# siyi-wind/MDViT

Hardware: AMD Instinct MI355X
Metric: 512x512 images/sec MDViT train step (fwd+bwd, two-sweep, AdamW) (higher is better)
Workload: dtype bf16x3 (fp32 storage; GEMM operands split hi+lo bf16, fp32 accumulate); 1 GPU; MDViT Sup+MLPFM train step, 4 domain(s) x bs=4 per GPU, 512x512, drop_rate=0.1 drop_path=0.1, bf16x3 GEMMs, data-parallel x1

## Files before the change

### include/mdvit_hip.h

```cpp
#ifndef MDVIT_HIP_H
#define MDVIT_HIP_H

#include <stddef.h>
#include <stdint.h>

#ifdef __cplusplus
extern "C" {
#endif

#define MDVIT_ABI_VERSION 1

enum {
    MDVIT_OK = 0,
    MDVIT_E_SHAPE = 1,
    MDVIT_E_DTYPE = 2,
    MDVIT_E_ALIGN = 3,
    MDVIT_E_WORKSPACE = 4,
    MDVIT_E_HIP = 5
};

enum { MDVIT_EPI_NONE = 0, MDVIT_EPI_GELU_DUAL = 1, MDVIT_EPI_DGELU = 2 };
enum { MDVIT_ACT_NONE = 0, MDVIT_ACT_HSWISH = 1, MDVIT_ACT_RELU = 2 };

const char* mdvit_last_error(void);
// ... 75 lines not shown
int mdvit_gemm_ph_prefers(int32_t M, int32_t N, int32_t K, int32_t planes);
int mdvit_gemm_ph_prefers_epi(int32_t M, int32_t N, int32_t K, int32_t planes, int32_t epi_reads);
int mdvit_gemm_ph_config(int32_t mode);
int mdvit_gemm_pm_prefers(int32_t M, int32_t N, int32_t K, int32_t planes, int32_t a_f32);
int mdvit_gemm_pm_config(int32_t mode);
int mdvit_gemm_pm_splits(int32_t M, int32_t N, int32_t K, int32_t planes, int32_t a_f32);
int mdvit_split_planes(const float* in, int64_t ld_in, void* out, int64_t ld_out, int64_t plane_stride, int64_t rows, int32_t cols, int32_t planes, void* stream);
int mdvit_split_planes_t(const float* in, int64_t ld_in, void* out, int64_t ld_out, int64_t plane_stride, int32_t rows, int32_t cols, int32_t transpose,
                         int32_t planes, void* stream);
int mdvit_split_planes_many(const void* items_dev, int32_t n, int32_t blocks_per_item, int32_t planes, void* stream);

int mdvit_mlp_fwd_f32(const float* x, const float* W1, const float* b1, const float* W2, const float* b2, const float* res,
                      const float* rowscale , int32_t rows_per_scale, float* h, float* y, int32_t M, int32_t C, int32_t hidden,
                      float drop_p, uint32_t key1_0, uint32_t key1_1, uint32_t key2_0, uint32_t key2_1, const uint32_t* drop_seed, void* stream);

int mdvit_mlp_config(int32_t wide_min_tokens, int32_t ablate);

int mdvit_mlp_bwd_dgrad_f32(const float* gm, const float* x, const float* W1, const float* b1, const float* W2t, const float* W1t,
                            float* du , float* dx, int32_t M, int32_t C, int32_t hidden, float drop_p,
                            uint32_t key1_0, uint32_t key1_1, const uint32_t* drop_seed, void* stream);

int mdvit_mlp_rc_fwd(const float* x, const void* W1p, const float* b1, const void* W2p, const float* b2, const float* res,
                     const float* rowscale , int32_t rows_per_scale, float* y, int32_t M, int32_t C, int32_t hidden,
                     float drop_p, uint32_t key1_0, uint32_t key1_1, uint32_t key2_0, uint32_t key2_1, const uint32_t* drop_seed, void* stream);
int mdvit_mlp_rc_dgrad(const float* gm, const float* x, const void* W1p, const float* b1, const void* W2tp, const void* W1tp, float* dx,
                       int32_t M, int32_t C, int32_t hidden, float drop_p, uint32_t key1_0, uint32_t key1_1, const uint32_t* drop_seed, void* stream);
int mdvit_linear_rc(const float* x, int64_t lda, const void* Wp, int64_t wplane, const float* bias, float* y, int64_t ldc, int32_t M, int32_t N, int32_t K,
                    float drop_p, uint32_t key0, uint32_t key1, const float* rowscale, int32_t rows_per_scale, const float* residual, int64_t ldr,
                    const uint32_t* drop_seed, void* stream);
int mdvit_linear_rc_ln(const float* x, const float* gamma, const float* beta, int32_t groups, float eps, float* mean, float* rstd, float* ln_out,
                       const void* Wp, int64_t wplane, const float* bias, float* y, int64_t ldc, int32_t M, int32_t N, int32_t K, void* stream);
int mdvit_mlp_rc16_fwd(const float* x, const void* W1p, const float* b1, const void* W2p, const float* b2, const float* res, const float* rowscale,
                       int32_t rows_per_scale, float* h, float* y, int32_t M, int32_t C, int32_t Hd, float drop_p, uint32_t key1_0, uint32_t key1_1,
                       uint32_t key2_0, uint32_t key2_1, const uint32_t* drop_seed, void* stream);
int mdvit_mlp_rc_fwd_ln(const float* x2, const float* gamma, const float* beta, int32_t groups, float eps, float* mean, float* rstd, float* ln_out,
                        const void* W1p, const float* b1, const void* W2p, const float* b2, const float* rowscale, int32_t rows_per_scale, float* h, float* y,
                        int32_t M, int32_t C, int32_t Hd, float drop_p, uint32_t key1_0, uint32_t key1_1, uint32_t key2_0, uint32_t key2_1,
                        const uint32_t* drop_seed, void* stream);
int mdvit_mlp_rc16_dgrad(const float* gm, const float* x, const void* W1p, const float* b1, const void* W2tp, const void* W1tp, float* du, float* dx,
                         int32_t M, int32_t C, int32_t Hd, float drop_p, uint32_t key1_0, uint32_t key1_1, const uint32_t* drop_seed, void* stream);
int mdvit_mlp_rc16_fwd_hbf16(const float* x, const void* W1p, const float* b1, const void* W2p, const float* b2, const float* res, const float* rowscale,
                             int32_t rows_per_scale, float* h, float* y, int32_t M, int32_t C, int32_t Hd, float drop_p, uint32_t key1_0, uint32_t key1_1,
                             uint32_t key2_0, uint32_t key2_1, const uint32_t* drop_seed, void* stream);
int mdvit_mlp_rc_fwd_ln_hbf16(const float* x2, const float* gamma, const float* beta, int32_t groups, float eps, float* mean, float* rstd, float* ln_out,
                              const void* W1p, const float* b1, const void* W2p, const float* b2, const float* rowscale, int32_t rows_per_scale, float* h, float* y,
                              int32_t M, int32_t C, int32_t Hd, float drop_p, uint32_t key1_0, uint32_t key1_1, uint32_t key2_0, uint32_t key2_1,
                              const uint32_t* drop_seed, void* stream);
int mdvit_mlp_rc16_dgrad_hbf16(const float* gm, const float* x, const void* W1p, const float* b1, const void* W2tp, const void* W1tp, float* du, float* dx,
                               int32_t M, int32_t C, int32_t Hd, float drop_p, uint32_t key1_0, uint32_t key1_1, const uint32_t* drop_seed, void* stream);
int mdvit_mlp_rc_bwd(const float* gm, const float* x, const void* W1p, const float* b1, const void* W2tp, const void* W1tp, float* dx_parts, float* dW1, float* db1,
                     float* dW2, void* ws, size_t ws_bytes, int32_t M, int32_t C, int32_t hidden, float drop_p, uint32_t key1_0, uint32_t key1_1,
                     const uint32_t* drop_seed, int32_t accumulate, void* stream);
size_t mdvit_mlp_rc_wgrad_ws_bytes(int32_t M, int32_t C, int32_t hidden);
int mdvit_gemm_ledger(int32_t enable);
int mdvit_gemm_ledger_read(int32_t index, char* name, int32_t cap, int64_t* launches, double* flop, double* bytes);
int mdvit_gemm_sampler(const char* symbol, int32_t stride);
int mdvit_gemm_sampler_read(int32_t index, char* name, int32_t cap, int64_t* seen, int64_t* timed, double* ms);
int mdvit_mlp_rc_config(int32_t fwd_variant);
int mdvit_mlp_rc_planes(int32_t planes);
int mdvit_block_config(int32_t mlp_bwd_fused);
int mdvit_mlp_rc_wgrad(const float* gm, const float* x, const void* W1p, const float* b1, const void* W2tp, float* dW1, float* db1, float* dW2,
                       void* ws, size_t ws_bytes, int32_t M, int32_t C, int32_t hidden, float drop_p, uint32_t key1_0, uint32_t key1_1,
                       const uint32_t* drop_seed, int32_t accumulate, void* stream);

typedef struct MdvitBlockDesc {
    int32_t B, H, W, C, heads, hidden, s3, s5, s7, ln_groups, D, da_hidden, precision;
    float eps, drop_p;
    uint32_t key_proj[2], key_fc1[2], key_fc2[2];
    const uint32_t* drop_seed;
    const float* rowscale1; const float* rowscale2;
    const float* label;
    const float *cpe_w, *cpe_b, *n1_g, *n1_b, *qkv_w, *qkv_b, *w3, *b3, *w5, *b5, *w7, *b7, *da_w1, *da_b1, *da_w2, *da_b2, *proj_w, *proj_b, *n2_g, *n2_b, *fc1_w, *fc1_b,
        *fc2_w, *fc2_b;
    const float *qkv_wt, *proj_wt, *fc1_wt, *fc2_wt;
    const void *fc1_p, *fc2_p, *fc2t_p, *fc1t_p;
    const void *qkv_p, *proj_p, *projt_p, *qkvt_p;
    int32_t store_bf16;
    const float* a_pre;
    int32_t attn_kind;
} MdvitBlockDesc;
typedef struct MdvitBlockGrads {
    float *cpe_w, *cpe_b, *n1_g, *n1_b, *qkv_w, *qkv_b, *w3, *b3, *w5, *b5, *w7, *b7, *da_w1, *da_b1, *da_w2, *da_b2, *proj_w, *proj_b, *n2_g, *n2_b, *fc1_w, *fc1_b, *fc2_w,
        *fc2_b;
    int32_t accumulate, dgrad_only, aux_first;
    int32_t ln_accumulate;
    float* e_out;
} MdvitBlockGrads;
typedef struct MdvitBlockStreams {
    void* main; void* side;
    void** events; int32_t n_events; int32_t* next_event;
} MdvitBlockStreams;
size_t mdvit_block_save_bytes(const MdvitBlockDesc* d);
size_t mdvit_block_fwd_ws_bytes(const MdvitBlockDesc* d);
int mdvit_block_fwd(const MdvitBlockDesc* d, const float* x, float* y, void* save, size_t save_bytes, void* ws, size_t ws_bytes, void* stream);
size_t mdvit_block_bwd_ws_bytes(const MdvitBlockDesc* d, const MdvitBlockGrads* g, int32_t with_side_stream, size_t* side_bytes);
int mdvit_block_bwd(const MdvitBlockDesc* d, const MdvitBlockGrads* g, const MdvitBlockStreams* st, const float* x, const void* save, size_t save_bytes,
                    const float* dy, float* dx , void* ws, size_t ws_bytes, void* ws_side, size_t ws_side_bytes);

int mdvit_rowdot_fwd(const float* x, int64_t ldx, const float* w, const float* b, float* y,
                     int32_t M, int32_t K, int32_t accumulate, void* stream);
int mdvit_rowdot_bwd(const float* x, int64_t ldx, const float* w, const float* dy, float* dx, int64_t lddx,
                     float* dw, float* db, void* ws , size_t ws_bytes, int32_t M, int32_t K, void* stream);

int mdvit_colsum_f32(const float* A, int64_t lda, float* out, float* masked, void* ws , size_t ws_bytes, int32_t M, int32_t N,
                     float drop_p, uint32_t key0, uint32_t key1, const float* rowscale, int32_t rows_per_scale,
                     int32_t accumulate, const uint32_t* drop_seed, void* stream);
// ... 181 lines not shown
```

### mdvit_amd/_lib.py

```python
from __future__ import annotations

import ctypes as C
import os
import re
from typing import List

_HERE = os.path.dirname(os.path.abspath(__file__))
LIB_PATH = os.environ.get("MDVIT_HIP_LIB") or os.path.join(_HERE, "lib", "libmdvit_hip.so")
HEADER_PATH = os.path.join(_HERE, "..", "include", "mdvit_hip.h")

EPI_NONE, EPI_GELU_DUAL, EPI_DGELU = 0, 1, 2
ACT_NONE, ACT_HSWISH, ACT_RELU = 0, 1, 2

f32p = C.c_void_p
vp = C.c_void_p
i32 = C.c_int32
i64 = C.c_int64
u32 = C.c_uint32
f32 = C.c_float


class GemmDesc(C.Structure):
    _fields_ = [
        ("A", vp), ("B", vp), ("C", vp), ("C2", vp),
# ... 71 lines not shown
    _fields_ = [(n, vp) for n in BLOCK_PARAMS] + [("accumulate", i32), ("dgrad_only", i32), ("aux_first", i32), ("ln_accumulate", i32), ("e_out", vp)]


class SeAdapterDesc(C.Structure):
    _fields_ = [("kind", i32), ("B", i32), ("N", i32), ("C", i32), ("r", i32), ("W1", vp), ("b1", vp), ("W2", vp), ("b2", vp), ("Wg", vp), ("bg", vp)]


SE_DASE, SE_USE = 0, 1


class BlockStreams(C.Structure):
    _fields_ = [("main", vp), ("side", vp), ("events", C.POINTER(vp)), ("n_events", i32), ("next_event", C.POINTER(i32))]


_SIGS = {
    "mdvit_block_fwd": [C.POINTER(BlockDesc), vp, vp, vp, C.c_size_t, vp, C.c_size_t, vp],
    "mdvit_block_bwd": [C.POINTER(BlockDesc), C.POINTER(BlockGrads), C.POINTER(BlockStreams), vp, vp, C.c_size_t, vp, vp, vp, C.c_size_t, vp, C.c_size_t],
    "mdvit_gemm_planes": [C.POINTER(PlaneGemmDesc), vp],
    "mdvit_gemm_planes_plan": [C.POINTER(PlaneGemmDesc), C.POINTER(i32), C.POINTER(i32), C.POINTER(i32)],
    "mdvit_gemm_planes_force_plan": [i32, i32],
    "mdvit_gemm_ph_config": [i32],
    "mdvit_gemm_pm_config": [i32],
    "mdvit_da_fwd_many": [C.POINTER(DaMany), vp, i32, i32, vp],
    "mdvit_da_bwd_many": [C.POINTER(DaMany), C.POINTER(DaManyGrads), vp, f32, vp, C.c_size_t, i32, i32, vp],
    "mdvit_gemm_pm_prefers": [i32, i32, i32, i32, i32],
    "mdvit_gemm_pm_splits": [i32, i32, i32, i32, i32],
    "mdvit_gemm_f32_grouped": [C.POINTER(GemmDesc), i32, C.POINTER(vp), C.POINTER(vp), C.POINTER(vp), vp],
    "mdvit_gemm_f32_grouped_bias": [C.POINTER(GemmDesc), i32, C.POINTER(vp), C.POINTER(vp), C.POINTER(vp), C.POINTER(vp), vp],
    "mdvit_transpose_batch": [i32, C.POINTER(vp), C.POINTER(i64), C.POINTER(vp), C.POINTER(i32), C.POINTER(i32), vp],
    "mdvit_compose_bias": [i32, C.POINTER(vp), i64, C.POINTER(vp), C.POINTER(vp), i32, i32, vp],
    "mdvit_compose_bias_bwd": [i32, C.POINTER(vp), i64, C.POINTER(vp), C.POINTER(vp), C.POINTER(vp), i64, C.POINTER(vp), i32, i32, i32, vp],
    "mdvit_gemm_ph_prefers": [i32, i32, i32, i32],
    "mdvit_gemm_ph_prefers_epi": [i32, i32, i32, i32, i32],
    "mdvit_mlp_config": [i32, i32],
    "mdvit_mlp_rc_config": [i32],
    "mdvit_mlp_rc_planes": [i32],
    "mdvit_block_config": [i32],
    "mdvit_gemm_ledger": [i32],
    "mdvit_gemm_ledger_read": [i32, C.c_char_p, i32, C.POINTER(i64), C.POINTER(C.c_double), C.POINTER(C.c_double)],
    "mdvit_gemm_sampler": [C.c_char_p, i32],
    "mdvit_gemm_sampler_read": [i32, C.c_char_p, i32, C.POINTER(i64), C.POINTER(i64), C.POINTER(C.c_double)],
    "mdvit_mlp_rc_fwd": [vp, vp, vp, vp, vp, vp, vp, i32, vp, i32, i32, i32, f32, u32, u32, u32, u32, vp, vp],
    "mdvit_linear_rc": [vp, i64, vp, i64, vp, vp, i64, i32, i32, i32, f32, u32, u32, vp, i32, vp, i64, vp, vp],
    "mdvit_linear_rc_ln": [vp, vp, vp, i32, f32, vp, vp, vp, vp, i64, vp, vp, i64, i32, i32, i32, vp],
    "mdvit_mlp_rc_fwd_ln": [vp, vp, vp, i32, f32, vp, vp, vp, vp, vp, vp, vp, vp, i32, vp, vp, i32, i32, i32, f32, u32, u32, u32, u32, vp, vp],
    "mdvit_mlp_rc16_fwd": [vp, vp, vp, vp, vp, vp, vp, i32, vp, vp, i32, i32, i32, f32, u32, u32, u32, u32, vp, vp],
    "mdvit_mlp_rc_dgrad": [vp, vp, vp, vp, vp, vp, vp, i32, i32, i32, f32, u32, u32, vp, vp],
    "mdvit_mlp_rc16_dgrad": [vp, vp, vp, vp, vp, vp, vp, vp, i32, i32, i32, f32, u32, u32, vp, vp],
    "mdvit_mlp_rc_fwd_ln_hbf16": [vp, vp, vp, i32, f32, vp, vp, vp, vp, vp, vp, vp, vp, i32, vp, vp, i32, i32, i32, f32, u32, u32, u32, u32, vp, vp],
    "mdvit_mlp_rc16_fwd_hbf16": [vp, vp, vp, vp, vp, vp, vp, i32, vp, vp, i32, i32, i32, f32, u32, u32, u32, u32, vp, vp],
    "mdvit_mlp_rc16_dgrad_hbf16": [vp, vp, vp, vp, vp, vp, vp, vp, i32, i32, i32, f32, u32, u32, vp, vp],
    "mdvit_mlp_rc_wgrad": [vp, vp, vp, vp, vp, vp, vp, vp, vp, C.c_size_t, i32, i32, i32, f32, u32, u32, vp, i32, vp],
    "mdvit_mlp_rc_bwd": [vp, vp, vp, vp, vp, vp, vp, vp, vp, vp, vp, C.c_size_t, i32, i32, i32, f32, u32, u32, vp, i32, vp],
    "mdvit_imgconv_fwd": [vp, vp, vp, i32, i32, i32, i32, i32, i32, vp],
    "mdvit_imgconv_wgrad": [vp, vp, vp, vp, C.c_size_t, i32, i32, i32, i32, i32, i32, i32, vp],
    "mdvit_maxpool3x3s2_fwd": [vp, vp, vp, i32, i32, i32, i32, vp],
    "mdvit_maxpool3x3s2_bwd": [vp, vp, vp, i32, i32, i32, i32, vp],
    "mdvit_resize_ac_fwd": [vp, vp, i32, i32, i32, i32, i32, i32, vp],
    "mdvit_resize_ac_bwd": [vp, vp, i32, i32, i32, i32, i32, i32, vp],
    "mdvit_ew": [vp, vp, vp, i64, i32, vp],
    "mdvit_add3": [vp, vp, vp, vp, i64, vp],
    "mdvit_add_parts": [vp, vp, C.POINTER(vp), i32, i64, vp, vp],
    "mdvit_add_bcast": [vp, vp, vp, i32, i64, vp],
    "mdvit_sum_batch": [vp, vp, i32, i64, vp],
    "mdvit_gate_fwd": [vp, vp, vp, i32, i64, i32, i32, vp],
    "mdvit_gate_bwd": [vp, vp, vp, vp, vp, vp, C.c_size_t, i32, i64, i32, i32, vp],
    "mdvit_imgconv_im2col": [vp, vp, i32, i32, i32, i32, i32, i32, vp],
    "mdvit_chanpool_fwd": [vp, vp, vp, i64, i32, vp],
    "mdvit_chanpool_bwd": [vp, vp, vp, i64, i32, vp],
    "mdvit_conv7x7_2to1_fwd": [vp, vp, vp, i32, i32, i32, vp],
    "mdvit_conv7x7_2to1_bwd": [vp, vp, vp, vp, vp, i32, i32, i32, vp],
    "mdvit_bn1_fwd": [vp, vp, vp, vp, vp, vp, vp, vp, i64, i32, i32, f32, f32, vp],
    "mdvit_bn1_bwd": [vp, vp, vp, vp, vp, vp, i64, i32, i32, vp],
    "mdvit_subsample2": [vp, vp, i32, i32, i32, i32, i32, vp],
    "mdvit_patchify": [vp, vp, i32, i32, i32, i32, i32, vp],
    "mdvit_dropout2d": [vp, vp, i32, i64, i32, f32, u32, u32, vp, vp],
    "mdvit_sdpa_fwd": [vp, vp, vp, vp, i32, i32, i32, i32, vp],
    "mdvit_sdpa_bwd": [vp, vp, vp, vp, vp, vp, vp, vp, i32, i32, i32, i32, vp],
    "mdvit_sdpa_mfma_fwd": [vp, vp, vp, vp, i32, i32, i32, i32, vp],
    "mdvit_sdpa_mfma_bwd": [vp, vp, vp, vp, vp, vp, vp, vp, i32, i32, i32, i32, vp],
    "mdvit_structure_weight": [vp, vp, vp, i32, i32, i32, vp],
    "mdvit_structure_loss_fwd": [vp, vp, vp, vp, vp, i32, i64, vp],
    "mdvit_structure_loss_bwd": [vp, vp, vp, vp, vp, vp, i32, i64, vp],
    "mdvit_split_planes": [vp, i64, vp, i64, i64, i64, i32, i32, vp],
    "mdvit_split_planes_many": [vp, i32, i32, i32, vp],
    "mdvit_split_planes_t": [vp, i64, vp, i64, i64, i32, i32, i32, i32, vp],
    "mdvit_event_create": [C.POINTER(vp)],
    "mdvit_event_destroy": [vp],
    "mdvit_event_elapsed_ms": [vp, vp, C.POINTER(f32)],
    "mdvit_timing_arm": [vp, vp],
    "mdvit_gemm_f32": [C.POINTER(GemmDesc), vp],
    "mdvit_gemm_plan": [C.POINTER(GemmDesc), C.POINTER(i32), C.POINTER(i32), C.POINTER(i32)],
    "mdvit_gemm_force_plan": [i32, i32],
    "mdvit_conv_weight_relayout": [vp, vp, i32, i32, i32, vp],
    "mdvit_conv_weight_relayout_many": [vp, i32, i32, vp],
    "mdvit_gemm_kernel_name": [vp, C.c_char_p, i32],
    "mdvit_gemm_tn_config": [i32, i32, i32],
    "mdvit_gemm_tn_grid_order": [i32],
    "mdvit_transpose_f32": [vp, i64, vp, i32, i32, vp],
    "mdvit_mlp_bwd_dgrad_f32": [vp, vp, vp, vp, vp, vp, vp, vp, i32, i32, i32, f32, u32, u32, vp, vp],
    "mdvit_mlp_fwd_f32": [vp, vp, vp, vp, vp, vp, vp, i32, vp, vp, i32, i32, i32, f32, u32, u32, u32, u32, vp, vp],
    "mdvit_transpose_many": [vp, i32, i32, vp],
    "mdvit_rowdot_fwd": [vp, i64, vp, vp, vp, i32, i32, i32, vp],
    "mdvit_rowdot_bwd": [vp, i64, vp, vp, vp, i64, vp, vp, vp, C.c_size_t, i32, i32, vp],
    "mdvit_colsum_f32": [vp, i64, vp, vp, vp, C.c_size_t, i32, i32, f32, u32, u32, vp, i32, i32, vp, vp],
    "mdvit_layernorm_fwd": [vp, vp, vp, vp, vp, vp, i32, i32, i32, f32, vp],
# ... 150 lines not shown
```

### mdvit_amd/csrc/block.hip

```cpp
#include <stdlib.h>
#include "common.h"

namespace {

struct Arena {
    char* base; size_t off, cap; bool dry;
    float* take(size_t floats) {
        const size_t bytes = (floats * sizeof(float) + 255) & ~(size_t)255;
        float* p = dry ? nullptr : reinterpret_cast<float*>(base + off);
        off += bytes;
        return p;
    }
    void* take_bytes(size_t bytes) { return take((bytes + 3) / 4); }
};

enum { MLP_RC = 0, MLP_RECOMP = 1, MLP_STORED = 2 };

inline int mlp_mode(const MdvitBlockDesc& d) {
    if (d.precision == 1 && d.C == 64 && d.hidden % 256 == 0 && d.hidden <= 4096 && d.fc1_p && d.fc2_p && (long)d.B * d.H * d.W * d.hidden < (1L << 32)) return MLP_RC;
    if (d.precision >= 1 && d.C <= 128 && d.C % 32 == 0 && d.hidden % 4 == 0) return MLP_RECOMP;
    return MLP_STORED;
}
inline bool mlp_rc16(const MdvitBlockDesc& d) {
    return mlp_mode(d) == MLP_RECOMP && d.precision == 1 && d.C == 128 && d.hidden % 32 == 0 && d.hidden <= 4096 && d.fc1_p && d.fc2_p && d.fc1_b && d.fc2_b &&
// ... 187 lines not shown
        if (hbf16(d))
            BLK_RUN(mdvit_mlp_rc16_fwd_hbf16(sv.cur2, d.fc1_p, d.fc1_b, d.fc2_p, d.fc2_b, sv.x2, d.rowscale2, N_tok, sv.h, y, M, C, Hd, d.drop_p, d.key_fc1[0],
                                             d.key_fc1[1], d.key_fc2[0], d.key_fc2[1], seed, s));
        else
            BLK_RUN(mdvit_mlp_rc16_fwd(sv.cur2, d.fc1_p, d.fc1_b, d.fc2_p, d.fc2_b, sv.x2, d.rowscale2, N_tok, sv.h, y, M, C, Hd, d.drop_p, d.key_fc1[0], d.key_fc1[1],
                                       d.key_fc2[0], d.key_fc2[1], seed, s));
    } else {
        MdvitGemmDesc g;
        gemm_init(g, d);
        g.A = sv.cur2; g.B = d.fc1_w; g.M = M; g.N = Hd; g.K = C; g.lda = C; g.ldb = C; g.ldc = Hd; g.bias = d.fc1_b; g.epi = MDVIT_EPI_GELU_DUAL;
        g.e_drop_p = d.drop_p; g.e_key0 = d.key_fc1[0]; g.e_key1 = d.key_fc1[1]; g.drop_seed = seed;
        if (mode == MLP_RECOMP) { g.C = sv.h; g.C2 = nullptr; }
        else { g.C = sv.u; g.C2 = sv.h; }
        g.trans_a = 0; g.trans_b = 1; g.allow_split = 0;
        if (ph_takes(d, d.fc1_p, M, Hd, C, 0)) { const int rc = gemm_planes_nt(A, g, d.fc1_p, s); if (rc != MDVIT_OK) return rc; }
        else BLK_RUN(mdvit_gemm_f32(&g, s));
        gemm_init(g, d);
        g.A = sv.h; g.B = d.fc2_w; g.C = y; g.M = M; g.N = C; g.K = Hd; g.lda = Hd; g.ldb = Hd; g.ldc = C; g.bias = d.fc2_b;
        g.e_drop_p = d.drop_p; g.e_key0 = d.key_fc2[0]; g.e_key1 = d.key_fc2[1]; g.e_rowscale = d.rowscale2; g.e_rows_per_scale = N_tok;
        g.residual = sv.x2; g.ldr = C; g.drop_seed = seed;
        g.trans_a = 0; g.trans_b = 1; g.allow_split = 0;
        if (ph_takes(d, d.fc2_p, M, C, Hd, 1)) { const int rc = gemm_planes_nt(A, g, d.fc2_p, s); if (rc != MDVIT_OK) return rc; }
        else BLK_RUN(mdvit_gemm_f32(&g, s));
    }
    return MDVIT_OK;
}

int block_bwd(const MdvitBlockDesc& d, const MdvitBlockGrads& G, const MdvitBlockStreams& st, const float* x, const float* dy, float* dx, Arena& SV, Arena& A, Arena& S) {
    const int B = d.B, H = d.H, W = d.W, C = d.C, Hd = d.hidden;
    const long T = (long)B * H * W;
    const int M = (int)T, N_tok = H * W;
    const int mode = mlp_mode(d);
    const bool dgrad_only = G.dgrad_only != 0, want_w = !dgrad_only;
    const int acc = G.accumulate;
    hipStream_t s = (hipStream_t)st.main, side = s;
    Saved sv;
    layout_saved(d, SV, sv);
    if (sdpa_kind(d)) sv.x1 = const_cast<float*>(x);
    const uint32_t* seed = d.drop_p > 0.f ? d.drop_seed : nullptr;
    const bool fast_ln = C == 64 || C == 128 || C == 320 || C == 512;

    const bool have_side = st.side != nullptr && st.side != st.main;
    const bool defer = want_w && acc != 0 && G.ln_accumulate != 0 && have_side && fast_ln;
    struct Late { const float* part; int batches, nblk, n0; float* out0; int n1; float* out1; };
    Late late[4];
    int n_late = 0;
    if (want_w && acc == 0) {
        const MdvitZeroItem z[4] = {{G.qkv_b, sizeof(float) * 3 * C}, {G.proj_b, sizeof(float) * C}, {mode == MLP_RC ? nullptr : G.fc1_b, sizeof(float) * Hd},
                                    {mode == MLP_RC ? nullptr : G.fc2_b, sizeof(float) * C}};
        BLK_RUN(mdvit_zero_many(z, 4, s));
    }

    const bool masked = d.drop_p > 0.f || d.rowscale2 != nullptr;
    float* gm2 = masked ? S.take(T * C) : const_cast<float*>(dy);
    float* tmp = A.take(T * C);
    float* dcur2 = tmp;
    const float* dcur2_b = nullptr;
    float* du = nullptr;
    if (mode == MLP_RC) {
        if (masked || want_w) {
            const size_t pb = want_w ? mdvit_partials_ws_bytes(C) : 0;
            void* pw = want_w ? (defer ? S.take_bytes(pb) : A.take_bytes(pb)) : nullptr;
            if (want_w && defer) {
                int nb = 0;
                BLK_RUN(mdvit_colsum_parts(dy, C, masked ? gm2 : nullptr, pw, pb, M, C, d.drop_p, d.key_fc2[0], d.key_fc2[1], d.rowscale2, N_tok, seed, s, &nb));
                late[n_late++] = Late{(const float*)pw, 1, nb, C, G.fc2_b, 0, nullptr};
            } else {
                BLK_RUN(mdvit_colsum_f32(dy, C, want_w ? G.fc2_b : nullptr, masked ? gm2 : nullptr, pw, pb, M, C, d.drop_p, d.key_fc2[0], d.key_fc2[1], d.rowscale2, N_tok,
                                         acc, seed, s));
            }
        }
        const bool fuse_bwd = want_w && (Hd == 256 || Hd == 512) && (g_blk_mlp_bwd == 1 || (g_blk_mlp_bwd == 2 && !have_side));
        if (fuse_bwd) {
            const int roles = Hd / 256;
            float* parts = roles == 1 ? dcur2 : A.take((long)roles * T * C);
            const size_t wb = mdvit_mlp_rc_wgrad_ws_bytes(M, C, Hd);
            void* ww = A.take_bytes(wb);
            BLK_RUN(mdvit_mlp_rc_bwd(gm2, sv.cur2, d.fc1_p, d.fc1_b, d.fc2t_p, d.fc1t_p, parts, G.fc1_w, G.fc1_b, G.fc2_w, ww, wb, M, C, Hd, d.drop_p, d.key_fc1[0],
                                     d.key_fc1[1], seed, acc, s));
            dcur2 = parts;
            dcur2_b = roles == 2 ? parts + T * C : nullptr;
        } else {
        BLK_RUN(mdvit_mlp_rc_dgrad(gm2, sv.cur2, d.fc1_p, d.fc1_b, d.fc2t_p, d.fc1t_p, dcur2, M, C, Hd, d.drop_p, d.key_fc1[0], d.key_fc1[1], seed, s));
        if (want_w) {
            const size_t wb = mdvit_mlp_rc_wgrad_ws_bytes(M, C, Hd);
            void* ww = S.take_bytes(wb);
            if (!A.dry) { const int rc = fork_side(d, st, side); if (rc != MDVIT_OK) return rc; }
            BLK_RUN(mdvit_mlp_rc_wgrad(gm2, sv.cur2, d.fc1_p, d.fc1_b, d.fc2t_p, G.fc1_w, G.fc1_b, G.fc2_w, ww, wb, M, C, Hd, d.drop_p, d.key_fc1[0], d.key_fc1[1], seed,
                                       acc, side));
        }
        }
    } else {
        if (masked) BLK_RUN(mdvit_colsum_f32(dy, C, nullptr, gm2, nullptr, 0, M, C, d.drop_p, d.key_fc2[0], d.key_fc2[1], d.rowscale2, N_tok, 0, seed, s));
        MdvitGemmDesc g;
        int rc = MDVIT_OK;
        const bool hb = hbf16(d);
        if (hb && !(d.fc2t_p && d.fc1t_p)) return mdvit_set_error(MDVIT_E_SHAPE, "block_bwd: store_bf16 needs the transposed fc weight planes (the 16-token MLP backward)");
        if (mlp_rc16(d) && d.fc2t_p && d.fc1t_p) {
            du = want_w ? S.take(hb ? (T * Hd + 1) / 2 : T * Hd) : nullptr;
            if (hb) BLK_RUN(mdvit_mlp_rc16_dgrad_hbf16(gm2, sv.cur2, d.fc1_p, d.fc1_b, d.fc2t_p, d.fc1t_p, du, dcur2, M, C, Hd, d.drop_p, d.key_fc1[0], d.key_fc1[1], seed, s));
            else BLK_RUN(mdvit_mlp_rc16_dgrad(gm2, sv.cur2, d.fc1_p, d.fc1_b, d.fc2t_p, d.fc1t_p, du, dcur2, M, C, Hd, d.drop_p, d.key_fc1[0], d.key_fc1[1], seed, s));
        } else {
            du = S.take(T * Hd);
            gemm_init(g, d);
            g.epi = MDVIT_EPI_DGELU; g.e_drop_p = d.drop_p; g.e_key0 = d.key_fc1[0]; g.e_key1 = d.key_fc1[1]; g.drop_seed = seed;
            if (mode == MLP_RECOMP) { g.rc_a = sv.cur2; g.rc_lda = C; g.rc_b = d.fc1_w; g.rc_ldb = C; g.rc_bias = d.fc1_b; g.rc_k = C; }
            else { g.gelu_u = sv.u; g.ldu = Hd; }
            g.allow_split = 0;
            rc = gemm_dgrad(A, d, g, gm2, d.fc2_w, d.fc2_wt, du, M, Hd, C, s, d.fc2t_p);
            if (rc != MDVIT_OK) return rc;
            gemm_init(g, d);
            g.allow_split = 1;
            rc = gemm_dgrad(A, d, g, du, d.fc1_w, d.fc1_wt, dcur2, M, C, Hd, s, d.fc1t_p);
            if (rc != MDVIT_OK) return rc;
        }
        if (want_w) {
            if (!A.dry) { rc = fork_side(d, st, side); if (rc != MDVIT_OK) return rc; }
            rc = gemm_wgrad(S, d, gm2, sv.h, G.fc2_w, G.fc2_b, M, C, Hd, acc, side, 0, hb);
            if (rc == MDVIT_OK) rc = gemm_wgrad(S, d, du, sv.cur2, G.fc1_w, G.fc1_b, M, Hd, C, acc, side, hb, 0);
            if (rc != MDVIT_OK) return rc;
        }
    }
    const bool masked1 = d.drop_p > 0.f || d.rowscale1 != nullptr;
    float* dx2 = masked1 ? A.take(T * C) : S.take(T * C);
    float* gm1 = masked1 ? S.take(T * C) : dx2;
    {
        const bool lnw = want_w || !fast_ln;
        const size_t pb = lnw ? mdvit_partials_ws_bytes(2 * C) : 0;
        void* pw = lnw ? A.take_bytes(pb) : nullptr;
        float* dg = want_w ? G.n2_g : (lnw ? A.take((long)d.ln_groups * C) : nullptr);
        float* db = want_w ? G.n2_b : (lnw ? A.take((long)d.ln_groups * C) : nullptr);
        if (!A.dry) mdvit_layernorm_bwd_next_dy2(dcur2_b);
        if (defer) {
            void* pws = S.take_bytes(pb);
            int nb = 0;
            BLK_RUN(mdvit_layernorm_bwd_parts(dcur2, sv.x2, d.n2_g, sv.mean2, sv.rstd2, dy, dx2, masked1 ? gm1 : nullptr, pws, pb, M, C, d.ln_groups, d.drop_p, d.key_proj[0],
                                              d.key_proj[1], d.rowscale1, N_tok, seed, s, &nb));
            late[n_late++] = Late{(const float*)pws, d.ln_groups, nb, C, dg, C, db};
        } else if (masked1 && fast_ln) {
            BLK_RUN(mdvit_layernorm_bwd_masked(dcur2, sv.x2, d.n2_g, sv.mean2, sv.rstd2, dy, dx2, gm1, dg, db, pw, pb, M, C, d.ln_groups, d.drop_p, d.key_proj[0],
                                               d.key_proj[1], d.rowscale1, N_tok, seed, s));
        } else {
            BLK_RUN(mdvit_layernorm_bwd(dcur2, sv.x2, d.n2_g, sv.mean2, sv.rstd2, dy, dx2, dg, db, pw, pb, M, C, d.ln_groups, s));
            if (masked1) BLK_RUN(mdvit_colsum_f32(dx2, C, nullptr, gm1, nullptr, 0, M, C, d.drop_p, d.key_proj[0], d.key_proj[1], d.rowscale1, N_tok, 0, seed, s));
        }
    }
    float* datt = tmp;
    {
        MdvitGemmDesc g;
        gemm_init(g, d);
        g.allow_split = 1;
        int rc = MDVIT_OK;
        if (d.precision == 1 && (C == 64 || C == 128) && d.projt_p && M >= 1024) {
            BLK_RUN(mdvit_linear_rc(gm1, C, d.projt_p, (long)C * C, nullptr, datt, C, M, C, C, 0.f, 0, 0, nullptr, 1, nullptr, 0, nullptr, s));
// ... 182 lines not shown
```

### mdvit_amd/csrc/common.h

```cpp
#pragma once
#include <hip/hip_runtime.h>
#include <hip/hip_ext.h>
#include <stdint.h>
#include <stdio.h>
#include <string.h>

#include "../../include/mdvit_hip.h"

#define MDVIT_WAVE 64

extern thread_local char g_mdvit_err[512];
int mdvit_set_error(int code, const char* fmt, ...);

#define MDVIT_CHECK_ARG(cond, code, ...)                      \
    do {                                                      \
        if (!(cond)) return mdvit_set_error(code, __VA_ARGS__); \
    } while (0)

extern hipEvent_t g_mdvit_t0, g_mdvit_t1;
#define MDVIT_TIMED_LAUNCH(kernel, grid, block, shmem, s, ...)                                                       \
    do {                                                                                                              \
        if (g_mdvit_t0) {                                                                                             \
            hipExtLaunchKernelGGL(kernel, grid, block, shmem, s, g_mdvit_t0, g_mdvit_t1, 0, __VA_ARGS__);             \
            g_mdvit_t0 = g_mdvit_t1 = nullptr;                                                                        \
        } else {                                                                                                      \
            hipLaunchKernelGGL(kernel, grid, block, shmem, s, __VA_ARGS__);                                           \
        }                                                                                                             \
    } while (0)

#define MDVIT_LAUNCH_CHECK()                                                         \
    do {                                                                             \
        hipError_t e__ = hipGetLastError();                                          \
        if (e__ != hipSuccess)                                                       \
            return mdvit_set_error(MDVIT_E_HIP, "%s:%d launch failed: %s", __FILE__, \
                                   __LINE__, hipGetErrorString(e__));                \
    } while (0)

int mdvit_zero_async(void* ptr, size_t bytes, hipStream_t stream);
struct MdvitZeroItem { void* p; size_t bytes; };
int mdvit_zero_many(const MdvitZeroItem* items, int n, hipStream_t stream);
#define MDVIT_ZERO(ptr, bytes, strm)                                   \
    do {                                                               \
        int rc__ = mdvit_zero_async((ptr), (bytes), (strm));           \
        if (rc__ != MDVIT_OK) return rc__;                             \
    } while (0)

int mdvit_reduce_partials(const float* part, int nblk, long stride, int n0, float* out0, int n1, float* out1, int accumulate, hipStream_t stream);
int mdvit_reduce_partials_batched(const float* part, int batches, int nblk, int n, float* out, hipStream_t stream);
int mdvit_reduce_partials_batched2(const float* part, int batches, int nblk, int n0, float* out0, int n1, float* out1, hipStream_t stream);
int mdvit_reduce_partials_batched2_acc(const float* part, int batches, int nblk, int n0, float* out0, int n1, float* out1, int accumulate, hipStream_t stream);
int mdvit_layernorm_bwd_parts(const float* dy, const float* x, const float* gamma, const float* mean, const float* rstd, const float* add, float* dx,
                              float* dx_masked, void* ws, size_t ws_bytes, int M, int C, int groups, float drop_p, uint32_t key0, uint32_t key1,
                              const float* rowscale, int rows_per_scale, const uint32_t* seed, hipStream_t stream, int* nblk);
int mdvit_colsum_parts(const float* A, long lda, float* masked, void* ws, size_t ws_bytes, int M, int N, float drop_p, uint32_t key0, uint32_t key1,
                       const float* rowscale, int rows_per_scale, const uint32_t* seed, hipStream_t stream, int* nblk);
void mdvit_layernorm_bwd_next_dy2(const float* dy2);
constexpr int MDVIT_MAX_PARTIAL_ROWS = 2048;
#define MDVIT_CHECK_PARTIALS_WS(ws, ws_bytes, nblk, n, what)                                                              \
    MDVIT_CHECK_ARG((ws) != nullptr && (ws_bytes) >= sizeof(float) * (size_t)(nblk) * (size_t)(n), MDVIT_E_WORKSPACE,    \
                    what ": workspace too small: need %zu bytes (mdvit_partials_ws_bytes), got %zu",                      \
                    sizeof(float) * (size_t)(nblk) * (size_t)(n), (size_t)(ws_bytes))

static inline bool aligned16(const void* p) { return (reinterpret_cast<uintptr_t>(p) & 15) == 0; }

static inline int cdiv(long a, long b) { return (int)((a + b - 1) / b); }

__device__ __forceinline__ uint32_t mdvit_hash32(uint32_t x) {
    x ^= x >> 16; x *= 0x7feb352dU; x ^= x >> 15; x *= 0x846ca68bU; x ^= x >> 16;
    return x;
}
__device__ __forceinline__ uint32_t mdvit_drop_bits(uint32_t k0, uint32_t k1, uint32_t idx) {
    return mdvit_hash32(((idx >> 2) ^ k0) + k1);
}
__device__ __forceinline__ uint32_t mdvit_drop_bits_q(uint32_t k0, uint32_t k1, uint32_t quad) { return mdvit_hash32((quad ^ k0) + k1); }
__device__ __forceinline__ float mdvit_drop_scale(uint32_t k0, uint32_t k1, uint32_t idx, uint32_t thresh, float inv_keep) {
    const uint32_t h = __builtin_rotateright32(mdvit_drop_bits(k0, k1, idx), 8u * (idx & 3u));
    return h >= thresh ? inv_keep : 0.0f;
}
static inline uint32_t mdvit_drop_thresh(double p) {
    double t = p * 65536.0 + 0.5;
    if (t < 0.0) t = 0.0;
    if (t > 65535.0) t = 65535.0;
    return (uint32_t)t << 16;
}
__device__ __forceinline__ void mdvit_drop_keep4(uint32_t h, uint32_t thresh16, bool (&keep)[4]) {
    const uint32_t r = __builtin_rotateright32(h, 8);
    keep[0] = (h >> 16) >= thresh16;
    keep[1] = (r >> 16) >= thresh16;
    keep[2] = (h & 0xffffu) >= thresh16;
    keep[3] = (r & 0xffffu) >= thresh16;
}
__device__ __forceinline__ float4 mdvit_drop_scale4(uint32_t k0, uint32_t k1, uint32_t idx4, uint32_t thresh, float inv_keep) {
    const uint32_t h = mdvit_drop_bits(k0, k1, idx4);
    return make_float4(h >= thresh ? inv_keep : 0.0f,
                       __builtin_rotateright32(h, 8) >= thresh ? inv_keep : 0.0f,
                       __builtin_rotateright32(h, 16) >= thresh ? inv_keep : 0.0f,
                       __builtin_rotateright32(h, 24) >= thresh ? inv_keep : 0.0f);
}

__device__ __forceinline__ float mdvit_normalize_level(unsigned char level, int c) {
    const float mean[3] = {0.485f, 0.456f, 0.406f}, stdv[3] = {0.229f, 0.224f, 0.225f};
    const float v = (float)((double)level / 255.0);
    return (v - mean[c]) / stdv[c];
}

__device__ __forceinline__ unsigned mdvit_xcd_logical_block() {
    const unsigned nwg = gridDim.x, q = nwg >> 3, r = nwg & 7, xcd = blockIdx.x & 7, idx = blockIdx.x >> 3;
    return (xcd < r ? xcd * (q + 1) : r * (q + 1) + (xcd - r) * q) + idx;
// ... 84 lines not shown
```

### mdvit_amd/csrc/mlp_rc.hip

```cpp
#include "common.h"
#include <type_traits>
#ifndef RC_ABL
#define RC_ABL 0
#endif

typedef float rc_f32x16 __attribute__((ext_vector_type(16)));
typedef __bf16 rc_bf16x8 __attribute__((ext_vector_type(8)));
typedef unsigned rc_u4 __attribute__((ext_vector_type(4)));
typedef unsigned rc_u2 __attribute__((ext_vector_type(2)));
typedef float rc_f4 __attribute__((ext_vector_type(4)));
typedef short rc_v4i16 __attribute__((ext_vector_type(4)));
typedef short rc_v8i16 __attribute__((ext_vector_type(8)));
typedef __attribute__((address_space(3))) rc_v4i16* rc_lds_v4i16_ptr;

namespace {

template <int ROWB>
__device__ __forceinline__ int rc_swz(int row) {
    if (ROWB == 64) return (row >> 2) & 3;
    if (ROWB == 128) return (((row >> 1) & 1) << 2) | ((row >> 2) & 3);
    return row & 15;
}

template <int ROWB>
__device__ __forceinline__ void rc_glds_piece(const uint16_t* __restrict__ src, long ld, int piece, int lane, char* tile) {
    constexpr int LPR = ROWB / 16, RPP = 1024 / ROWB;
    const int row = piece * RPP + lane / LPR;
    const int lc = (lane % LPR) ^ rc_swz<ROWB>(row);
    __builtin_amdgcn_global_load_lds(src + (long)row * ld + (lc << 3), (__attribute__((address_space(3))) void*)(tile + piece * 1024), 16, 0, 0);
}

template <int ROWB>
__device__ __forceinline__ rc_bf16x8 rc_frag(const char* tile, int row, int chunk) {
    return __builtin_bit_cast(rc_bf16x8, *reinterpret_cast<const rc_u4*>(tile + row * ROWB + ((chunk ^ rc_swz<ROWB>(row)) << 4)));
}

__device__ __forceinline__ rc_bf16x8 rc_frag_perm(const char* tile, int row, int hf, int g) {
    const int f = rc_swz<64>(row);
    typedef __attribute__((address_space(3))) const volatile rc_u2* lds_u2_ptr;
    const rc_u2 a = *(lds_u2_ptr)(tile + row * 64 + (((2 * hf) ^ f) << 4) + 8 * g);
    const rc_u2 b = *(lds_u2_ptr)(tile + row * 64 + (((2 * hf + 1) ^ f) << 4) + 8 * g);
    return __builtin_bit_cast(rc_bf16x8, (rc_u4{a[0], a[1], b[0], b[1]}));
}

#define RC_MFMA3P(P1, acc, ah, al, bh, bl)                                          \
    do {                                                                            \
        if constexpr (!(P1)) {                                                      \
            acc = __builtin_amdgcn_mfma_f32_32x32x16_bf16(al, bh, acc, 0, 0, 0);    \
            acc = __builtin_amdgcn_mfma_f32_32x32x16_bf16(ah, bl, acc, 0, 0, 0);    \
        }                                                                           \
        acc = __builtin_amdgcn_mfma_f32_32x32x16_bf16(ah, bh, acc, 0, 0, 0);        \
    } while (0)
#define RC_MFMA3(acc, ah, al, bh, bl)                                           \
    do {                                                                        \
        acc = __builtin_amdgcn_mfma_f32_32x32x16_bf16(al, bh, acc, 0, 0, 0);    \
        acc = __builtin_amdgcn_mfma_f32_32x32x16_bf16(ah, bl, acc, 0, 0, 0);    \
        acc = __builtin_amdgcn_mfma_f32_32x32x16_bf16(ah, bh, acc, 0, 0, 0);    \
    } while (0)

__device__ __forceinline__ void rc_split8(const float* v, rc_u4& hi, rc_u4& lo) {
    uint2 h0, l0, h1, l1;
    mdvit_split_bf16x3(make_float4(v[0], v[1], v[2], v[3]), h0, l0);
    mdvit_split_bf16x3(make_float4(v[4], v[5], v[6], v[7]), h1, l1);
    hi = rc_u4{h0.x, h0.y, h1.x, h1.y};
    lo = rc_u4{l0.x, l0.y, l1.x, l1.y};
}

__device__ __forceinline__ rc_bf16x8 rc_natural_order(rc_u4 v) {
    const rc_u2 a = __builtin_amdgcn_permlane32_swap(v[0], v[2], false, false);
    const rc_u2 b = __builtin_amdgcn_permlane32_swap(v[1], v[3], false, false);
    return __builtin_bit_cast(rc_bf16x8, (rc_u4{a[0], b[0], a[1], b[1]}));
}

struct LnPro { const float* g; const float* b; float* mean; float* rstd; float* out; float eps; int rows_per_group; };
template <int K>
__device__ __forceinline__ void rc_ln_rows32(float4 (&a)[K / 16], float4 (&b)[K / 16], int row, int rowc, int M, int lhi, const LnPro ln);

template <int C, bool LNP = false>
__device__ __forceinline__ void rc_load_rows(const float* __restrict__ src, int row, int M, int lhi, rc_bf16x8 (&hi)[C / 16], rc_bf16x8 (&lo)[C / 16],
                                             const LnPro* ln = nullptr) {
    const float* p = src + (long)min(row, M - 1) * C + 8 * lhi;
    float4 a[C / 16], b[C / 16];
#pragma unroll
    for (int kb = 0; kb < C / 16; ++kb) {
        a[kb] = *reinterpret_cast<const float4*>(p + 16 * kb);
        b[kb] = *reinterpret_cast<const float4*>(p + 16 * kb + 4);
    }
    if constexpr (LNP) rc_ln_rows32<C>(a, b, row, min(row, M - 1), M, lhi, *ln);
#pragma unroll
    for (int kb = 0; kb < C / 16; ++kb) {
        const float v[8] = {a[kb].x, a[kb].y, a[kb].z, a[kb].w, b[kb].x, b[kb].y, b[kb].z, b[kb].w};
        rc_u4 h, l;
        rc_split8(v, h, l);
        hi[kb] = __builtin_bit_cast(rc_bf16x8, h);
        lo[kb] = __builtin_bit_cast(rc_bf16x8, l);
    }
}

__device__ __forceinline__ void rc_erf_parts(float x, float& e, float& q) {
    e = __builtin_amdgcn_exp2f(x * x * -0.72134752044448170368f);
    const float t = __builtin_amdgcn_rcpf(fmaf(0.3275911f * 0.70710678118654752f, fabsf(x), 1.0f));
    float poly = fmaf(1.061405429f, t, -1.453152027f);
    poly = fmaf(poly, t, 1.421413741f);
    poly = fmaf(poly, t, -0.284496736f);
    poly = fmaf(poly, t, 0.254829592f);
    q = fmaf(-(poly * t), e, 1.0f);
}
__device__ __forceinline__ float rc_gelu_k(float x, float hk) {
    float e, q;
    rc_erf_parts(x, e, q);
    const float hx = x * hk;
    return fmaf(fabsf(hx), q, hx);
}
__device__ __forceinline__ float rc_dgelu_k(float x, float d, float hks, float pks) {
    float e, q;
    rc_erf_parts(x, e, q);
    const float cdf = fmaf(copysignf(q, x), hks, hks);
    return d * fmaf(x * e, pks, cdf);
}
__device__ __forceinline__ void rc_gelu_both_k(float x, float hk, float d, float hks, float pks, float& h, float& du) {
    float e, q;
    rc_erf_parts(x, e, q);
    const float hx = x * hk;
    h = fmaf(fabsf(hx), q, hx);
    const float cdf = fmaf(copysignf(q, x), hks, hks);
    du = d * fmaf(x * e, pks, cdf);
}
typedef float rc_f2 __attribute__((ext_vector_type(2)));
template <bool P1 = false>
__device__ __forceinline__ void rc_split2(float a, float b, uint32_t& hi, uint32_t& lo) {
    hi = __builtin_bit_cast(uint32_t, __builtin_convertvector((rc_f2{a, b}), mdvit_bf16x2));
    if constexpr (P1) { lo = 0u; return; }
    const rc_f2 l = {a - __uint_as_float(hi << 16), b - __uint_as_float(hi & 0xffff0000u)};
    lo = __builtin_bit_cast(uint32_t, __builtin_convertvector(l, mdvit_bf16x2));
}
__device__ __forceinline__ void rc_keep_sel4(uint32_t h, uint32_t thresh16, float on, float off, float (&k)[4]) {
    bool keep[4];
    mdvit_drop_keep4(h, thresh16, keep);
#pragma unroll
    for (int j = 0; j < 4; ++j) k[j] = keep[j] ? on : off;
}
// ... 15 lines not shown
#pragma unroll
    for (int kq = 0; kq < 4; ++kq) {
        float s0 = 0.f, s1 = 0.f;
#pragma unroll
        for (int j = 0; j < VPL; ++j) {
            const float4 va = a[kq + 4 * j], vb = b[kq + 4 * j];
            s0 += (va.x + va.y) + (va.z + va.w);
            s1 += (vb.x + vb.y) + (vb.z + vb.w);
        }
        q[kq][0] = s0; q[kq][1] = s1;
    }
    const float mu = lin_sum16(q) * (1.0f / K);
#pragma unroll
    for (int kb = 0; kb < KB; ++kb) {
        a[kb].x -= mu; a[kb].y -= mu; a[kb].z -= mu; a[kb].w -= mu;
        b[kb].x -= mu; b[kb].y -= mu; b[kb].z -= mu; b[kb].w -= mu;
    }
#pragma unroll
    for (int kq = 0; kq < 4; ++kq) {
        float s0 = 0.f, s1 = 0.f;
#pragma unroll
        for (int j = 0; j < VPL; ++j) {
            s0 += mdvit_ln_sq4(a[kq + 4 * j]);
            s1 += mdvit_ln_sq4(b[kq + 4 * j]);
        }
        q[kq][0] = s0; q[kq][1] = s1;
    }
    const float rs = mdvit_ln_rstd(lin_sum16(q), 1.0f / K, ln.eps);
#pragma unroll
    for (int kb = 0; kb < KB; ++kb) {
        const float4 ga = *reinterpret_cast<const float4*>(gg + 16 * kb), gb4 = *reinterpret_cast<const float4*>(gg + 16 * kb + 4);
        const float4 ba = *reinterpret_cast<const float4*>(gb + 16 * kb), bb4 = *reinterpret_cast<const float4*>(gb + 16 * kb + 4);
        a[kb] = mdvit_ln_affine4(a[kb], rs, ga, ba);
        b[kb] = mdvit_ln_affine4(b[kb], rs, gb4, bb4);
        if (row < M) {
            *reinterpret_cast<float4*>(ln.out + (long)row * K + 8 * lhi + 16 * kb) = a[kb];
            *reinterpret_cast<float4*>(ln.out + (long)row * K + 8 * lhi + 16 * kb + 4) = b[kb];
        }
    }
    if (lhi == 0 && row < M) { ln.mean[row] = mu; ln.rstd[row] = rs; }
}

struct RcArgs {
    const float* x; const float* gm; const float* res; const float* rowscale; const float* b1; const float* b2;
    const uint16_t* W1p;
    const uint16_t* W2p;
    const uint16_t* W2tp;
    const uint16_t* W1tp;
    float* y; float* dx;
    float* du;
    int hbf;
    float* h;
    LnPro ln;
    float* part;
    int M, Hd, rows_per_scale;
    int drop; uint32_t k1a, k1b, k2a, k2b, thresh; float inv_keep;
    const uint32_t* seed;
    int groups, tiles_per_group;
};

template <int NM, int V, int ND, int LEAD>
__device__ __forceinline__ void rc_interleave() {
    __builtin_amdgcn_sched_group_barrier(0x100, LEAD, 0);
#pragma unroll
    for (int i = 0; i < NM; ++i) {
        __builtin_amdgcn_sched_group_barrier(0x008, 1, 0);
        __builtin_amdgcn_sched_group_barrier(0x002, V, 0);
        if (i < ND - LEAD) __builtin_amdgcn_sched_group_barrier(0x100, 1, 0);
    }
}

#define RC_WAIT_VM(n) asm volatile("s_waitcnt vmcnt(%0)" ::"n"(n) : "memory")
#define RC_BARRIER() asm volatile("s_waitcnt lgkmcnt(0)\n\ts_barrier" ::: "memory")

template <int C, int NW, bool DROP>
__global__ __launch_bounds__(NW * 64) __attribute__((amdgpu_waves_per_eu(2, 2))) void mlp_rc_fwd_kernel(RcArgs p) {
    constexpr int KB = C / 16, CB = C / 32;
    constexpr int RB1 = C * 2;
    constexpr int T1 = 32 * RB1, T2 = C * 64;
    constexpr int PIECES = (2 * T1 + 2 * T2) / 1024;
    static_assert(PIECES % NW == 0, "pieces must divide over the waves");
    constexpr int PPW = PIECES / NW;
    extern __shared__ __attribute__((aligned(1024))) char smem[];
    char* sW1 = smem;
    char* sW2 = sW1 + 3 * 2 * T1;
    float* sB1 = reinterpret_cast<float*>(sW2 + 3 * 2 * T2);
    const int tid = threadIdx.x, lane = tid & 63, wave = __builtin_amdgcn_readfirstlane(tid >> 6), l31 = lane & 31, lhi = lane >> 5;
    const int row = blockIdx.x * (NW * 32) + wave * 32 + l31;
    const int n = p.Hd >> 5;
    uint32_t s0 = 0, s1 = 0;
    if (p.seed) { s0 = p.seed[0]; s1 = p.seed[1]; }
    const uint32_t k1a = p.k1a ^ s0, k1b = p.k1b + s1, k2a = p.k2a ^ s0, k2b = p.k2b + s1;
    const long wplane = (long)p.Hd * C;

    auto issue_w1 = [&](int slot_s, int src_s, int pc) __attribute__((always_inline)) {
        constexpr int PP = T1 / 1024;
        const int pl = pc / PP, q = pc % PP;
        rc_glds_piece<RB1>(p.W1p + pl * wplane + (long)(src_s * 32) * C, C, q, lane, sW1 + ((slot_s % 3) * 2 + pl) * T1);
    };
    auto issue_w2 = [&](int s, int pc) __attribute__((always_inline)) {
        constexpr int PP = T2 / 1024;
        const int pl = pc / PP, q = pc % PP;
        rc_glds_piece<64>(p.W2p + pl * wplane + s * 32, p.Hd, q, lane, sW2 + ((s % 3) * 2 + pl) * T2);
    };
    auto issue_group = [&](int g) __attribute__((always_inline)) {
#pragma unroll
// ... 278 lines not shown
    constexpr int PIECES = (4 * T1 + 2 * T3) / 1024;
    static_assert(PIECES % NW == 0, "pieces must divide over the waves");
    constexpr int PPW = PIECES / NW;
    extern __shared__ __attribute__((aligned(1024))) char smem[];
    char* sW1 = smem;
    char* sW2t = sW1 + 3 * 2 * T1;
    char* sW1t = sW2t + 3 * 2 * T1;
    float* sB1 = reinterpret_cast<float*>(sW1t + 3 * 2 * T3);
    const int tid = threadIdx.x, lane = tid & 63, wave = __builtin_amdgcn_readfirstlane(tid >> 6), l31 = lane & 31, lhi = lane >> 5;
    const int row = blockIdx.x * (NW * 32) + wave * 32 + l31;
    const int n = p.Hd >> 5;
    uint32_t s0 = 0, s1 = 0;
    if (p.seed) { s0 = p.seed[0]; s1 = p.seed[1]; }
    const uint32_t k1a = p.k1a ^ s0, k1b = p.k1b + s1;
    const uint32_t dq0 = (uint32_t)((long)row * p.Hd + 4 * lhi) >> 2, thresh16 = p.thresh >> 16;
    const float hks = 0.5f * p.inv_keep, pks = 0.39894228040143268f * p.inv_keep;
    const long wplane = (long)p.Hd * C;

    static_assert(T1 / 1024 == NW && T3 / 1024 == NW, "one 1 KiB piece of each of the six planes per wave and hidden step");
    uint32_t voff1, voff3;
    {
        constexpr int LPR = RB1 / 16, RPP = 1024 / RB1;
        const int r1 = wave * RPP + lane / LPR;
        voff1 = (uint32_t)(r1 * C + (((lane % LPR) ^ rc_swz<RB1>(r1)) << 3)) * 2u;
        const int r3 = wave * 16 + (lane >> 2);
        voff3 = (uint32_t)(r3 * p.Hd + (((lane & 3) ^ rc_swz<64>(r3)) << 3)) * 2u;
    }
    typedef __attribute__((address_space(3))) void* lds_ptr;
    auto issue_a = [&](int slot_s, int src_s) __attribute__((always_inline)) {
        const int sl = slot_s % 3;
        const char* b1p = reinterpret_cast<const char*>(p.W1p) + (long)src_s * (32 * C * 2);
        const char* b2p = reinterpret_cast<const char*>(p.W2tp) + (long)src_s * (32 * C * 2);
        __builtin_amdgcn_global_load_lds(b1p + voff1, (lds_ptr)(sW1 + (sl * 2 + 0) * T1 + wave * 1024), 16, 0, 0);
        __builtin_amdgcn_global_load_lds(b1p + wplane * 2 + voff1, (lds_ptr)(sW1 + (sl * 2 + 1) * T1 + wave * 1024), 16, 0, 0);
        __builtin_amdgcn_global_load_lds(b2p + voff1, (lds_ptr)(sW2t + (sl * 2 + 0) * T1 + wave * 1024), 16, 0, 0);
        __builtin_amdgcn_global_load_lds(b2p + wplane * 2 + voff1, (lds_ptr)(sW2t + (sl * 2 + 1) * T1 + wave * 1024), 16, 0, 0);
    };
    auto issue_b = [&](int s) __attribute__((always_inline)) {
        const int sl = s % 3;
        const char* b3p = reinterpret_cast<const char*>(p.W1tp) + (long)s * (32 * 2);
        __builtin_amdgcn_global_load_lds(b3p + voff3, (lds_ptr)(sW1t + (sl * 2 + 0) * T3 + wave * 1024), 16, 0, 0);
        __builtin_amdgcn_global_load_lds(b3p + wplane * 2 + voff3, (lds_ptr)(sW1t + (sl * 2 + 1) * T3 + wave * 1024), 16, 0, 0);
    };
    auto issue_group = [&](int g) __attribute__((always_inline)) {
        issue_a(g + 2, min(g + 2, n - 1));
        issue_b(g);
    };
    issue_a(0, 0);
    issue_a(1, 1);
    issue_group(0);
    for (int i = tid; i < p.Hd / 4; i += NW * 64) reinterpret_cast<float4*>(sB1)[i] = reinterpret_cast<const float4*>(p.b1)[i];
    rc_bf16x8 xh[KB], xl[KB], gh[KB], gl[KB];
    rc_load_rows<C>(p.x, row, p.M, lhi, xh, xl);
    rc_load_rows<C>(p.gm, row, p.M, lhi, gh, gl);
    rc_f32x16 dxacc[CB];
#pragma unroll
    for (int cb = 0; cb < CB; ++cb)
#pragma unroll
        for (int r = 0; r < 16; ++r) dxacc[cb][r] = 0.f;
    RC_WAIT_VM(0);
    __syncthreads();

    auto prod1 = [&](int s, rc_f32x16& u, rc_f32x16& d) __attribute__((always_inline)) {
        const char* w1h = sW1 + ((s % 3) * 2) * T1; const char* w1l = w1h + T1;
        const char* w2h = sW2t + ((s % 3) * 2) * T1; const char* w2l = w2h + T1;
#pragma unroll
        for (int q = 0; q < 4; ++q) {
            const rc_f4 b4 = *reinterpret_cast<const rc_f4*>(sB1 + s * 32 + 8 * q + 4 * lhi);
            u[4 * q + 0] = b4.x; u[4 * q + 1] = b4.y; u[4 * q + 2] = b4.z; u[4 * q + 3] = b4.w;
        }
#pragma unroll
        for (int r = 0; r < 16; ++r) d[r] = 0.f;
#pragma unroll
        for (int kb = 0; kb < KB; ++kb) {
            const rc_bf16x8 ah = rc_frag<RB1>(w1h, l31, 2 * kb + lhi), al = rc_frag<RB1>(w1l, l31, 2 * kb + lhi);
            RC_MFMA3P(P1, u, ah, al, xh[kb], xl[kb]);
            const rc_bf16x8 ch = rc_frag<RB1>(w2h, l31, 2 * kb + lhi), cl = rc_frag<RB1>(w2l, l31, 2 * kb + lhi);
            RC_MFMA3P(P1, d, ch, cl, gh[kb], gl[kb]);
        }
    };
    auto prod3 = [&](int s, const rc_bf16x8 (&dh)[2], const rc_bf16x8 (&dl)[2]) __attribute__((always_inline)) {
        const char* hi = sW1t + ((s % 3) * 2) * T3; const char* lo = hi + T3;
#pragma unroll
        for (int half = 0; half < 2; ++half)
#pragma unroll
            for (int cb = 0; cb < CB; ++cb) {
                const rc_bf16x8 ah = rc_frag_perm(hi, cb * 32 + l31, half, lhi);
                rc_bf16x8 al = ah;
                if constexpr (!P1) al = rc_frag_perm(lo, cb * 32 + l31, half, lhi);
                RC_MFMA3P(P1, dxacc[cb], ah, al, dh[half], dl[half]);
            }
    };
    auto act = [&](int s, const rc_f32x16& u, const rc_f32x16& d, rc_bf16x8 (&dh)[2], rc_bf16x8 (&dl)[2]) __attribute__((always_inline)) {
        uint32_t ph[8], pl[8];
#pragma unroll
        for (int q = 0; q < 4; ++q) {
            float dm[4] = {d[4 * q + 0], d[4 * q + 1], d[4 * q + 2], d[4 * q + 3]};
            if (DROP) {
                bool keep[4];
                mdvit_drop_keep4(mdvit_drop_bits_q(k1a, k1b, dq0 + s * 8 + 2 * q), thresh16, keep);
#pragma unroll
                for (int j = 0; j < 4; ++j) dm[j] = keep[j] ? dm[j] : 0.f;
            }
            const float g0 = rc_dgelu_k(u[4 * q + 0], dm[0], hks, pks), g1 = rc_dgelu_k(u[4 * q + 1], dm[1], hks, pks);
            const float g2 = rc_dgelu_k(u[4 * q + 2], dm[2], hks, pks), g3 = rc_dgelu_k(u[4 * q + 3], dm[3], hks, pks);
            rc_split2<P1>(g0, g1, ph[2 * q], pl[2 * q]);
            rc_split2<P1>(g2, g3, ph[2 * q + 1], pl[2 * q + 1]);
// ... 94 lines not shown
#define RC16_MFMA3_BWD(acc, ah, al, bh, bl)                                     \
    do {                                                                        \
        acc = __builtin_amdgcn_mfma_f32_16x16x32_bf16(al, bh, acc, 0, 0, 0);    \
        acc = __builtin_amdgcn_mfma_f32_16x16x32_bf16(ah, bl, acc, 0, 0, 0);    \
        acc = __builtin_amdgcn_mfma_f32_16x16x32_bf16(ah, bh, acc, 0, 0, 0);    \
    } while (0)
typedef float rc_acc4 __attribute__((ext_vector_type(4)));
constexpr int RC_WT_ROW = 528;
constexpr int RC_BWD_LDS = 2 * 64 * RC_WT_ROW + 8 * 2 * 2048;

template <int C, bool DROP, bool DX = false, bool P1 = false>
__global__ __launch_bounds__(512) __attribute__((amdgpu_waves_per_eu(2, 2))) void mlp_rc_wgrad_kernel(RcArgs p) {
    constexpr int KB = C / 16, CB = C / 32;
    constexpr int TP = 32 * 128;
    static_assert(C == 64, "token-tile staging below is written for C = 64");
    __shared__ __attribute__((aligned(1024))) char smem[2 * 4 * TP];
    extern __shared__ __attribute__((aligned(1024))) char dsm[];
    char* sWt = dsm;
    char* sDu = dsm + 2 * 64 * RC_WT_ROW;
    const int tid = threadIdx.x, lane = tid & 63, wave = __builtin_amdgcn_readfirstlane(tid >> 6), l31 = lane & 31, lhi = lane >> 5, l15 = lane & 15;
    const int roles = p.Hd >> 8;
    const int xcd = blockIdx.x & 7, idx = blockIdx.x >> 3;
    const int role = idx % roles, group = (idx / roles) * 8 + xcd;
    const int hs = role * 256 + wave * 32;
    const int ntiles = (p.M + 31) >> 5;
    const int t_beg = min(group * p.tiles_per_group, ntiles), t_end = min(t_beg + p.tiles_per_group, ntiles);
    uint32_t s0 = 0, s1 = 0;
    if (p.seed) { s0 = p.seed[0]; s1 = p.seed[1]; }
    const uint32_t k1a = p.k1a ^ s0, k1b = p.k1b + s1;
    const long wplane = (long)p.Hd * C;

    rc_bf16x8 w1h[KB], w1l[KB], w2h[KB], w2l[KB];
#pragma unroll
    for (int kb = 0; kb < KB; ++kb) {
        const long o = (long)(hs + l31) * C + 16 * kb + 8 * lhi;
        w1h[kb] = __builtin_bit_cast(rc_bf16x8, *reinterpret_cast<const rc_u4*>(p.W1p + o));
        w1l[kb] = __builtin_bit_cast(rc_bf16x8, *reinterpret_cast<const rc_u4*>(p.W1p + wplane + o));
        w2h[kb] = __builtin_bit_cast(rc_bf16x8, *reinterpret_cast<const rc_u4*>(p.W2tp + o));
        w2l[kb] = __builtin_bit_cast(rc_bf16x8, *reinterpret_cast<const rc_u4*>(p.W2tp + wplane + o));
    }
    const float bias = p.b1[hs + l31];
    rc_f32x16 aw1[CB], aw2[CB];
#pragma unroll
    for (int cb = 0; cb < CB; ++cb)
#pragma unroll
        for (int r = 0; r < 16; ++r) { aw1[cb][r] = 0.f; aw2[cb][r] = 0.f; }
    float db1 = 0.f;
    const uint32_t drot = 8u * (lane & 3), thresh16 = p.thresh >> 16;
    const float hks = 0.5f * p.inv_keep, pks = 0.39894228040143268f * p.inv_keep;

    const int srow = tid >> 4, sc4 = tid & 15;
    const int soff = srow * 128 + (((sc4 >> 1) ^ rc_swz<128>(srow)) << 4) + (sc4 & 1) * 8;
    float4 rx, rg;
    auto load_tile = [&](int t) __attribute__((always_inline)) {
        const int row = t * 32 + srow, rc = min(row, p.M - 1);
        rx = *reinterpret_cast<const float4*>(p.x + (long)rc * C + sc4 * 4);
        rg = *reinterpret_cast<const float4*>(p.gm + (long)rc * C + sc4 * 4);
        if (row >= p.M) rg = make_float4(0.f, 0.f, 0.f, 0.f);
    };
    auto store_tile = [&](int buf) __attribute__((always_inline)) {
        char* b = smem + buf * 4 * TP;
        uint2 hi, lo;
        mdvit_split_bf16x3(rx, hi, lo);
        *reinterpret_cast<rc_u2*>(b + soff) = rc_u2{hi.x, hi.y};
        *reinterpret_cast<rc_u2*>(b + TP + soff) = rc_u2{lo.x, lo.y};
        mdvit_split_bf16x3(rg, hi, lo);
        *reinterpret_cast<rc_u2*>(b + 2 * TP + soff) = rc_u2{hi.x, hi.y};
        *reinterpret_cast<rc_u2*>(b + 3 * TP + soff) = rc_u2{lo.x, lo.y};
    };

    if (DX) {
        for (int i = tid; i < 2 * 64 * 32; i += 512) {
            const int pl = i >> 11, c = (i >> 5) & 63, ch = i & 31;
            const rc_u4 v = *reinterpret_cast<const rc_u4*>(p.W1tp + pl * wplane + (long)c * p.Hd + role * 256 + ch * 8);
            *reinterpret_cast<rc_u4*>(sWt + (pl * 64 + c) * RC_WT_ROW + ch * 16) = v;
        }
    }
    if (t_beg < t_end) {
        load_tile(t_beg);
        store_tile(0);
    }
    __syncthreads();
    for (int t = t_beg; t < t_end; ++t) {
        const int buf = (t - t_beg) & 1;
        const char* xb = smem + buf * 4 * TP;
        const char* xhi = xb; const char* xlo = xb + TP; const char* ghi = xb + 2 * TP; const char* glo = xb + 3 * TP;
        if (t + 1 < t_end) load_tile(t + 1);
        rc_f32x16 u, d;
#pragma unroll
        for (int r = 0; r < 16; ++r) { u[r] = bias; d[r] = 0.f; }
#pragma unroll
        for (int kb = 0; kb < KB; ++kb) {
            const rc_bf16x8 ah = rc_frag<128>(xhi, l31, 2 * kb + lhi), al = rc_frag<128>(xlo, l31, 2 * kb + lhi);
            RC_MFMA3_ACT_AP(P1, u, ah, al, w1h[kb], w1l[kb]);
            const rc_bf16x8 ch = rc_frag<128>(ghi, l31, 2 * kb + lhi), cl = rc_frag<128>(glo, l31, 2 * kb + lhi);
            RC_MFMA3_ACT_AP(P1, d, ch, cl, w2h[kb], w2l[kb]);
        }
        uint32_t hb[4];
        if (DROP) {
#pragma unroll
            for (int j = 0; j < 4; ++j) {
                const int tok = t * 32 + j + 8 * (lane & 3) + 4 * lhi;
                hb[j] = mdvit_drop_bits(k1a, k1b, (uint32_t)((long)tok * p.Hd + hs + l31));
            }
        }
#pragma unroll
        for (int ks = 0; ks < 2; ++ks) {
            rc_u4 hh, hl, dh, dl;
#pragma unroll
            for (int i = 0; i < 4; ++i) {
                const int r = 8 * ks + 2 * i;
                float hv[2], gv[2];
#pragma unroll
                for (int e = 0; e < 2; ++e) {
                    float hk = 0.5f, dm = d[r + e];
                    if (DROP) {
                        const uint32_t w = rc_quad_bcast(hb[(r + e) & 3], (r + e) >> 2);
                        const bool keep = (__builtin_amdgcn_alignbit(w, w, drot) >> 16) >= thresh16;
                        hk = keep ? hks : 0.f; dm = keep ? dm : 0.f;
                    }
                    rc_gelu_both_k(u[r + e], hk, dm, hks, pks, hv[e], gv[e]);
                    db1 += gv[e];
                }
                uint32_t a0, a1, a2, a3;
                rc_split2<P1>(hv[0], hv[1], a0, a1);
                rc_split2<P1>(gv[0], gv[1], a2, a3);
                hh[i] = a0; hl[i] = a1; dh[i] = a2; dl[i] = a3;
            }
            const rc_bf16x8 hhf = __builtin_bit_cast(rc_bf16x8, hh), hlf = __builtin_bit_cast(rc_bf16x8, hl);
            const rc_bf16x8 dhf = __builtin_bit_cast(rc_bf16x8, dh), dlf = __builtin_bit_cast(rc_bf16x8, dl);
            if (DX) {
                char* base = sDu + wave * 4096 + l31 * 64 + 8 * lhi;
                const int f = (l31 >> 1) & 3;
#pragma unroll
                for (int pc = 0; pc < 2; ++pc) {
                    const int ch = (2 * ks + pc) ^ f;
                    *reinterpret_cast<rc_u2*>(base + (ch << 4)) = rc_u2{dh[2 * pc], dh[2 * pc + 1]};
                    *reinterpret_cast<rc_u2*>(base + 2048 + (ch << 4)) = rc_u2{dl[2 * pc], dl[2 * pc + 1]};
                }
            }
            const int t0 = 16 * ks + 4 * lhi;
#pragma unroll
            for (int cb = 0; cb < CB; ++cb) {
                const int col0 = cb * 32 + 16 * ((lane >> 4) & 1);
                const rc_bf16x8 bxh = rc_tr8(xhi, t0, col0, l15), bxl = rc_tr8(xlo, t0, col0, l15);
                RC_MFMA3_ACT_AP(P1, aw1[cb], dhf, dlf, bxh, bxl);
                const rc_bf16x8 agh = rc_tr8(ghi, t0, col0, l15), agl = rc_tr8(glo, t0, col0, l15);
                RC_MFMA3_ACT_AP(P1, aw2[cb], agh, agl, hhf, hlf);
            }
        }
        if (DX) {
            __syncthreads();
            const int cblk = wave & 3, tblk = wave >> 2, g4 = lane >> 4;
            rc_acc4 acc = {0.f, 0.f, 0.f, 0.f};
            const int pr = l15 >> 2, pcb = 32 * tblk + 8 * (l15 & 3);
#pragma unroll
            for (int k8 = 0; k8 < 8; ++k8) {
                const char* wa = sWt + (cblk * 16 + l15) * RC_WT_ROW + (4 * k8 + g4) * 16;
                const rc_bf16x8 ah = __builtin_bit_cast(rc_bf16x8, *reinterpret_cast<const rc_u4*>(wa));
                const rc_bf16x8 al = __builtin_bit_cast(rc_bf16x8, *reinterpret_cast<const rc_u4*>(wa + 64 * RC_WT_ROW));
                const char* dplane = sDu + k8 * 4096;
                const int ra = 8 * g4 + pr, rb = ra + 4;
                const int oa = ra * 64 + (((pcb >> 4) ^ ((ra >> 1) & 3)) << 4) + (pcb & 15), ob = rb * 64 + (((pcb >> 4) ^ ((rb >> 1) & 3)) << 4) + (pcb & 15);
                const rc_v4i16 h0 = __builtin_amdgcn_ds_read_tr16_b64_v4i16((rc_lds_v4i16_ptr)(dplane + oa)), h1 = __builtin_amdgcn_ds_read_tr16_b64_v4i16((rc_lds_v4i16_ptr)(dplane + ob));
                const rc_v4i16 l0 = __builtin_amdgcn_ds_read_tr16_b64_v4i16((rc_lds_v4i16_ptr)(dplane + 2048 + oa)), l1 = __builtin_amdgcn_ds_read_tr16_b64_v4i16((rc_lds_v4i16_ptr)(dplane + 2048 + ob));
                const rc_bf16x8 bh = __builtin_bit_cast(rc_bf16x8, (rc_v8i16{h0[0], h0[1], h0[2], h0[3], h1[0], h1[1], h1[2], h1[3]}));
                const rc_bf16x8 bl = __builtin_bit_cast(rc_bf16x8, (rc_v8i16{l0[0], l0[1], l0[2], l0[3], l1[0], l1[1], l1[2], l1[3]}));
                RC16_MFMA3_BWDP(P1, acc, ah, al, bh, bl);
            }
            const int tok = t * 32 + tblk * 16 + l15;
            if (tok < p.M) *reinterpret_cast<float4*>(p.dx + ((long)role * p.M + tok) * C + cblk * 16 + 4 * g4) = make_float4(acc[0], acc[1], acc[2], acc[3]);
        }
        if (t + 1 < t_end) store_tile(buf ^ 1);
        __syncthreads();
    }

    float* pg = p.part + (long)group * (2L * p.Hd * C + p.Hd);
#pragma unroll
    for (int cb = 0; cb < CB; ++cb)
#pragma unroll
        for (int r = 0; r < 16; ++r) {
            const int i = (r & 3) + 8 * (r >> 2) + 4 * lhi;
            pg[(long)(hs + i) * C + cb * 32 + l31] = aw1[cb][r];
            pg[(long)p.Hd * C + (long)(cb * 32 + i) * p.Hd + hs + l31] = aw2[cb][r];
        }
    db1 += __shfl_xor(db1, 32, 64);
    if (lhi == 0) pg[2L * p.Hd * C + hs + l31] = db1;
}

typedef float rc_f32x4 __attribute__((ext_vector_type(4)));

template <int ROWB>
__device__ __forceinline__ int rc16_swz(int row) {
    if (ROWB == 64) return (row >> 2) & 3;
    if (ROWB == 128) return (row >> 1) & 7;
    return row & 15;
}
template <int ROWB>
__device__ __forceinline__ void rc16_glds_piece(const uint16_t* __restrict__ src, long ld, int piece, int lane, char* tile) {
    constexpr int LPR = ROWB / 16, RPP = 1024 / ROWB;
    const int row = piece * RPP + lane / LPR;
    const int lc = (lane % LPR) ^ rc16_swz<ROWB>(row);
    __builtin_amdgcn_global_load_lds(src + (long)row * ld + (lc << 3), (__attribute__((address_space(3))) void*)(tile + piece * 1024), 16, 0, 0);
}
template <int ROWB>
__device__ __forceinline__ rc_bf16x8 rc16_frag(const char* tile, int row, int chunk) {
    return __builtin_bit_cast(rc_bf16x8, *reinterpret_cast<const rc_u4*>(tile + row * ROWB + ((chunk ^ rc16_swz<ROWB>(row)) << 4)));
}
__device__ __forceinline__ rc_bf16x8 rc16_frag_perm(const char* tile, int row, int g) {
    const int f = rc16_swz<64>(row);
    const rc_u2 a = *reinterpret_cast<const rc_u2*>(tile + row * 64 + (((g >> 1) ^ f) << 4) + (g & 1) * 8);
    const rc_u2 b = *reinterpret_cast<const rc_u2*>(tile + row * 64 + (((2 + (g >> 1)) ^ f) << 4) + (g & 1) * 8);
    return __builtin_bit_cast(rc_bf16x8, (rc_u4{a[0], a[1], b[0], b[1]}));
}

#define RC16_MFMA3P(P1, acc, ah, al, bh, bl)                                        \
    do {                                                                            \
        if constexpr (!(P1)) {                                                      \
            acc = __builtin_amdgcn_mfma_f32_16x16x32_bf16(al, bh, acc, 0, 0, 0);    \
            acc = __builtin_amdgcn_mfma_f32_16x16x32_bf16(ah, bl, acc, 0, 0, 0);    \
        }                                                                           \
        acc = __builtin_amdgcn_mfma_f32_16x16x32_bf16(ah, bh, acc, 0, 0, 0);        \
    } while (0)
#define RC16_MFMA3(acc, ah, al, bh, bl)                                         \
    do {                                                                        \
        acc = __builtin_amdgcn_mfma_f32_16x16x32_bf16(al, bh, acc, 0, 0, 0);    \
        acc = __builtin_amdgcn_mfma_f32_16x16x32_bf16(ah, bl, acc, 0, 0, 0);    \
        acc = __builtin_amdgcn_mfma_f32_16x16x32_bf16(ah, bh, acc, 0, 0, 0);    \
    } while (0)

__device__ __forceinline__ void rc16_ln_rows128(float4 (&a)[4], float4 (&b)[4], int row, int rowc, int M, int g, const LnPro ln);

template <int C, bool LNP = false>
__device__ __forceinline__ void rc16_load_rows(const float* __restrict__ src, int row, int M, int g, rc_bf16x8 (&hi)[C / 32], rc_bf16x8 (&lo)[C / 32],
                                               const LnPro* ln = nullptr) {
    const float* p = src + (long)min(row, M - 1) * C + 8 * g;
    float4 a[C / 32], b[C / 32];
#pragma unroll
    for (int ks = 0; ks < C / 32; ++ks) {
        a[ks] = *reinterpret_cast<const float4*>(p + 32 * ks);
        b[ks] = *reinterpret_cast<const float4*>(p + 32 * ks + 4);
    }
    if constexpr (LNP && C == 128) rc16_ln_rows128(a, b, row, min(row, M - 1), M, g, *ln);
#pragma unroll
    for (int ks = 0; ks < C / 32; ++ks) {
        const float v[8] = {a[ks].x, a[ks].y, a[ks].z, a[ks].w, b[ks].x, b[ks].y, b[ks].z, b[ks].w};
        rc_u4 h, l;
        rc_split8(v, h, l);
        hi[ks] = __builtin_bit_cast(rc_bf16x8, h);
        lo[ks] = __builtin_bit_cast(rc_bf16x8, l);
    }
}

__device__ __forceinline__ float rc16_sum16(const float (&q)[2][2]) {
    float r0 = q[0][0] + q[1][0], r1 = q[0][1] + q[1][1];
    r0 += __shfl_xor(r0, 32, 64); r1 += __shfl_xor(r1, 32, 64);
    r0 += __shfl_xor(r0, 16, 64); r1 += __shfl_xor(r1, 16, 64);
    return r0 + r1;
}
__device__ __forceinline__ void rc16_ln_rows128(float4 (&a)[4], float4 (&b)[4], int row, int rowc, int M, int g, const LnPro ln) {
    constexpr int K = 128;
    const int grp = rowc / ln.rows_per_group;
    const float* gg = ln.g + (long)grp * K + 8 * g;
    const float* gb = ln.b + (long)grp * K + 8 * g;
    float q[2][2];
#pragma unroll
    for (int kq = 0; kq < 2; ++kq) {
        float s0 = 0.f, s1 = 0.f;
#pragma unroll
        for (int j = 0; j < 2; ++j) {
            const float4 va = a[kq + 2 * j], vb = b[kq + 2 * j];
            s0 += (va.x + va.y) + (va.z + va.w);
            s1 += (vb.x + vb.y) + (vb.z + vb.w);
        }
        q[kq][0] = s0; q[kq][1] = s1;
    }
    const float mu = rc16_sum16(q) * (1.0f / K);
#pragma unroll
    for (int ks = 0; ks < 4; ++ks) {
        a[ks].x -= mu; a[ks].y -= mu; a[ks].z -= mu; a[ks].w -= mu;
        b[ks].x -= mu; b[ks].y -= mu; b[ks].z -= mu; b[ks].w -= mu;
    }
#pragma unroll
    for (int kq = 0; kq < 2; ++kq) {
        float s0 = 0.f, s1 = 0.f;
#pragma unroll
        for (int j = 0; j < 2; ++j) {
            s0 += mdvit_ln_sq4(a[kq + 2 * j]);
            s1 += mdvit_ln_sq4(b[kq + 2 * j]);
        }
        q[kq][0] = s0; q[kq][1] = s1;
    }
    const float rs = mdvit_ln_rstd(rc16_sum16(q), 1.0f / K, ln.eps);
#pragma unroll
    for (int ks = 0; ks < 4; ++ks) {
        const float4 ga = *reinterpret_cast<const float4*>(gg + 32 * ks), gb4 = *reinterpret_cast<const float4*>(gg + 32 * ks + 4);
// ... 119 lines not shown
            v.x *= rsc; v.y *= rsc; v.z *= rsc; v.w *= rsc;
            const float4 r4 = rq[ct];
            v.x += r4.x; v.y += r4.y; v.z += r4.z; v.w += r4.w;
            if (row < p.M) *reinterpret_cast<float4*>(p.y + (long)row * C + col) = v;
        }
    }
}

template <int C, int NW, int OCC, bool DROP, bool STORE, bool P1 = false>
__global__ __launch_bounds__(NW * 64) __attribute__((amdgpu_waves_per_eu(OCC, OCC))) void mlp_rc16_dgrad_kernel(RcArgs p) {
    constexpr int KS = C / 32, CT = C / 16;
    constexpr int RB1 = C * 2;
    constexpr int T1 = 32 * RB1, T3 = C * 64;
    constexpr int PIECES = (4 * T1 + 2 * T3) / 1024;
    static_assert(PIECES % NW == 0, "pieces must divide over the waves");
    constexpr int PPW = PIECES / NW;
    extern __shared__ __attribute__((aligned(1024))) char smem[];
    char* sW1 = smem;
    char* sW2 = sW1 + 3 * 2 * T1;
    char* sW3 = sW2 + 3 * 2 * T1;
    float* sB1 = reinterpret_cast<float*>(sW3 + 3 * 2 * T3);
    const int tid = threadIdx.x, lane = tid & 63, wave = __builtin_amdgcn_readfirstlane(tid >> 6), c16 = lane & 15, g = lane >> 4;
    const int row = blockIdx.x * (NW * 16) + wave * 16 + c16;
    const int n = p.Hd >> 5;
    uint32_t s0 = 0, s1 = 0;
    if (p.seed) { s0 = p.seed[0]; s1 = p.seed[1]; }
    const uint32_t k1a = p.k1a ^ s0, k1b = p.k1b + s1;
    const uint32_t dq0 = (uint32_t)((long)row * p.Hd + 4 * g) >> 2, thresh16 = p.thresh >> 16;
    const float hks = 0.5f * p.inv_keep, pks = 0.39894228040143268f * p.inv_keep;
    const long wplane = (long)p.Hd * C;
    auto issue_group = [&](int gi) __attribute__((always_inline)) {
        const int gs = min(gi, n - 1), slot = gi % 3;
#pragma unroll
        for (int i = 0; i < PPW; ++i) {
            const int pc = wave + i * NW;
            constexpr int PP1 = T1 / 1024, PP3 = T3 / 1024;
            if (pc < 2 * PP1) {
                const int pl = pc / PP1, q = pc % PP1;
                rc16_glds_piece<RB1>(p.W1p + pl * wplane + (long)(gs * 32) * C, C, q, lane, sW1 + (slot * 2 + pl) * T1);
            } else if (pc < 4 * PP1) {
                const int pc2 = pc - 2 * PP1, pl = pc2 / PP1, q = pc2 % PP1;
                rc16_glds_piece<RB1>(p.W2tp + pl * wplane + (long)(gs * 32) * C, C, q, lane, sW2 + (slot * 2 + pl) * T1);
            } else {
                const int pc3 = pc - 4 * PP1, pl = pc3 / PP3, q = pc3 % PP3;
                rc16_glds_piece<64>(p.W1tp + pl * wplane + gs * 32, p.Hd, q, lane, sW3 + (slot * 2 + pl) * T3);
            }
        }
    };
    issue_group(0);
    issue_group(1);
    for (int i = tid; i < p.Hd / 4; i += NW * 64) reinterpret_cast<float4*>(sB1)[i] = reinterpret_cast<const float4*>(p.b1)[i];
    rc_bf16x8 xh[KS], xl[KS], mh[KS], ml[KS];
    rc16_load_rows<C>(p.x, row, p.M, g, xh, xl);
    rc16_load_rows<C>(p.gm, row, p.M, g, mh, ml);
    rc_f32x4 dacc[CT];
#pragma unroll
    for (int ct = 0; ct < CT; ++ct) dacc[ct] = rc_f32x4{0.f, 0.f, 0.f, 0.f};
    __syncthreads();

    for (int t = 0; t < n; ++t) {
        if (STORE && t > 0) RC_WAIT_VM(PPW + 2);
        else RC_WAIT_VM(PPW);
        RC_BARRIER();
        issue_group(t + 2);
        const int slot = t % 3;
        const char* w1h = sW1 + (slot * 2) * T1; const char* w1l = w1h + T1;
        const char* w2h = sW2 + (slot * 2) * T1; const char* w2l = w2h + T1;
        const char* w3h = sW3 + (slot * 2) * T3; const char* w3l = w3h + T3;
        rc_u4 dh4, dl4;
#pragma unroll
        for (int ht = 0; ht < 2; ++ht) {
            const int hd = t * 32 + 16 * ht + 4 * g;
            const rc_f4 b4 = *reinterpret_cast<const rc_f4*>(sB1 + hd);
            rc_f32x4 u = {b4.x, b4.y, b4.z, b4.w}, d = {0.f, 0.f, 0.f, 0.f};
#pragma unroll
            for (int ks = 0; ks < KS; ++ks) {
                const rc_bf16x8 ah = rc16_frag<RB1>(w1h, 16 * ht + c16, 4 * ks + g), al = rc16_frag<RB1>(w1l, 16 * ht + c16, 4 * ks + g);
                RC16_MFMA3P(P1, u, ah, al, xh[ks], xl[ks]);
            }
#pragma unroll
            for (int ks = 0; ks < KS; ++ks) {
                const rc_bf16x8 ah = rc16_frag<RB1>(w2h, 16 * ht + c16, 4 * ks + g), al = rc16_frag<RB1>(w2l, 16 * ht + c16, 4 * ks + g);
                RC16_MFMA3P(P1, d, ah, al, mh[ks], ml[ks]);
            }
            float dm[4] = {d[0], d[1], d[2], d[3]};
            if (DROP) {
                bool keep[4];
                mdvit_drop_keep4(mdvit_drop_bits_q(k1a, k1b, dq0 + t * 8 + 4 * ht), thresh16, keep);
#pragma unroll
                for (int j = 0; j < 4; ++j) dm[j] = keep[j] ? dm[j] : 0.f;
            }
            const float g0 = rc_dgelu_k(u[0], dm[0], hks, pks), g1 = rc_dgelu_k(u[1], dm[1], hks, pks), g2 = rc_dgelu_k(u[2], dm[2], hks, pks), g3 = rc_dgelu_k(u[3], dm[3], hks, pks);
            if (STORE && !p.hbf) { if (row < p.M) *reinterpret_cast<float4*>(p.du + (long)row * p.Hd + hd) = make_float4(g0, g1, g2, g3); }
            uint32_t a0, a1, a2, a3;
            rc_split2<P1>(g0, g1, a0, a1);
            rc_split2<P1>(g2, g3, a2, a3);
            dh4[2 * ht] = a0; dl4[2 * ht] = a1; dh4[2 * ht + 1] = a2; dl4[2 * ht + 1] = a3;
        }
        if (STORE && p.hbf && row < p.M) {
            uint16_t* db = reinterpret_cast<uint16_t*>(p.du) + (long)row * p.Hd + t * 32 + 4 * g;
            *reinterpret_cast<uint2*>(db) = make_uint2(dh4[0], dh4[1]);
            *reinterpret_cast<uint2*>(db + 16) = make_uint2(dh4[2], dh4[3]);
        }
        const rc_bf16x8 dh = __builtin_bit_cast(rc_bf16x8, dh4), dl = __builtin_bit_cast(rc_bf16x8, dl4);
#pragma unroll
        for (int ct = 0; ct < CT; ++ct) {
            const rc_bf16x8 ah = rc16_frag_perm(w3h, 16 * ct + c16, g), al = rc16_frag_perm(w3l, 16 * ct + c16, g);
// ... 98 lines not shown
            }
            if (FULL) {
#pragma clang fp contract(off)
                v.x *= rsc; v.y *= rsc; v.z *= rsc; v.w *= rsc;
                v.x += rq[q].x; v.y += rq[q].y; v.z += rq[q].z; v.w += rq[q].w;
            }
            if (row < p.M) *reinterpret_cast<float4*>(p.y + (long)row * p.ldc + col) = v;
        }
    }
    RC_WAIT_VM(0);
}

__global__ __launch_bounds__(256) void rc_reduce_kernel(const float* __restrict__ part, int groups, long stride, int n0, float* o0, int n1, float* o1, int n2, float* o2,
                                                        int accumulate) {
    const int q = blockIdx.x * 256 + threadIdx.x, n = n0 + n1 + n2;
    if (q * 4 >= n) return;
    float4 s = make_float4(0.f, 0.f, 0.f, 0.f);
    const float* src = part + (long)q * 4;
    int g = 0;
    for (; g + 4 <= groups; g += 4) {
        const float4 a = *reinterpret_cast<const float4*>(src + (long)g * stride), b = *reinterpret_cast<const float4*>(src + (long)(g + 1) * stride);
        const float4 c = *reinterpret_cast<const float4*>(src + (long)(g + 2) * stride), d = *reinterpret_cast<const float4*>(src + (long)(g + 3) * stride);
        s.x += a.x; s.y += a.y; s.z += a.z; s.w += a.w;
        s.x += b.x; s.y += b.y; s.z += b.z; s.w += b.w;
        s.x += c.x; s.y += c.y; s.z += c.z; s.w += c.w;
        s.x += d.x; s.y += d.y; s.z += d.z; s.w += d.w;
    }
    for (; g < groups; ++g) {
        const float4 a = *reinterpret_cast<const float4*>(src + (long)g * stride);
        s.x += a.x; s.y += a.y; s.z += a.z; s.w += a.w;
    }
    const int i = q * 4;
    float* dst = i < n0 ? o0 + i : (i < n0 + n1 ? o1 + (i - n0) : o2 + (i - n0 - n1));
    float4 v = s;
    if (accumulate) { const float4 o = *reinterpret_cast<const float4*>(dst); v.x += o.x; v.y += o.y; v.z += o.z; v.w += o.w; }
    *reinterpret_cast<float4*>(dst) = v;
}

int rc_set_lds(const void* k, int bytes, bool (&flags)[64]) {
    int dev = 0;
    if (hipGetDevice(&dev) != hipSuccess || dev < 0 || dev >= 64) dev = 0;
    if (flags[dev]) return MDVIT_OK;
    const hipError_t e = hipFuncSetAttribute(k, hipFuncAttributeMaxDynamicSharedMemorySize, bytes);
    if (e != hipSuccess) return mdvit_set_error(MDVIT_E_HIP, "mlp_rc: cannot raise the dynamic LDS limit: %s", hipGetErrorString(e));
    flags[dev] = true;
    return MDVIT_OK;
}

void rc_fill(RcArgs& a, int M, int Hd, float drop_p, uint32_t k10, uint32_t k11, uint32_t k20, uint32_t k21, const uint32_t* seed) {
    a.M = M; a.Hd = Hd;
    a.drop = drop_p > 0.f; a.k1a = k10; a.k1b = k11; a.k2a = k20; a.k2b = k21;
    a.thresh = mdvit_drop_thresh(drop_p); a.inv_keep = 1.f / (1.f - drop_p);
    a.seed = seed;
}

}

int g_rc_planes = 2;
extern "C" int mdvit_mlp_rc_planes(int32_t planes) {
    if (planes != 1 && planes != 2) return mdvit_set_error(MDVIT_E_SHAPE, "mlp_rc_planes: 1 or 2");
    g_rc_planes = planes;
    return MDVIT_OK;
}
template <auto KERNEL>
static int rc_launch(int lds_cap, dim3 grid, dim3 block, int smem, hipStream_t s, const RcArgs& a) {
    static bool fl[64] = {false};
    if (lds_cap > 0) {
        const int rc = rc_set_lds(reinterpret_cast<const void*>(KERNEL), lds_cap, fl);
        if (rc != MDVIT_OK) return rc;
    }
    hipLaunchKernelGGL(KERNEL, grid, block, smem, s, a);
    return MDVIT_OK;
}

int g_rc_fwd_variant = 3;
int g_rc_fwd128_variant = 16;
extern "C" int mdvit_mlp_rc_config(int32_t fwd_variant) {
    if (fwd_variant == 16 || fwd_variant == 32) g_rc_fwd128_variant = fwd_variant;
    else g_rc_fwd_variant = fwd_variant;
    return MDVIT_OK;
}

extern "C" int mdvit_mlp_rc_fwd(const float* x, const void* W1p, const float* b1, const void* W2p, const float* b2, const float* res, const float* rowscale,
                                int32_t rows_per_scale, float* y, int32_t M, int32_t C, int32_t Hd, float drop_p, uint32_t key1_0, uint32_t key1_1,
                                uint32_t key2_0, uint32_t key2_1, const uint32_t* drop_seed, void* stream) {
    MDVIT_CHECK_ARG(C == 64, MDVIT_E_SHAPE, "mlp_rc_fwd: built for C = 64 (got %d)", C);
    MDVIT_CHECK_ARG(M > 0 && Hd >= 64 && Hd % 64 == 0 && Hd <= 4096, MDVIT_E_SHAPE, "mlp_rc_fwd: need M > 0, hidden %% 64 == 0, hidden <= 4096 (M=%d hidden=%d)", M, Hd);
    MDVIT_CHECK_ARG(x && W1p && b1 && W2p && b2 && res && y, MDVIT_E_SHAPE, "mlp_rc_fwd: null operand");
    MDVIT_CHECK_ARG(aligned16(x) && aligned16(W1p) && aligned16(b1) && aligned16(W2p) && aligned16(b2) && aligned16(res) && aligned16(y), MDVIT_E_ALIGN,
                    "mlp_rc_fwd: operands must be 16-byte aligned");
    MDVIT_CHECK_ARG(!(drop_p > 0.f) || (long)M * Hd < (1L << 32), MDVIT_E_SHAPE, "mlp_rc_fwd: dropout index space exceeds 2^32");
    RcArgs a;
    memset(&a, 0, sizeof(a));
    a.x = x; a.W1p = (const uint16_t*)W1p; a.b1 = b1; a.W2p = (const uint16_t*)W2p; a.b2 = b2; a.res = res; a.rowscale = rowscale; a.y = y;
    a.rows_per_scale = rows_per_scale > 0 ? rows_per_scale : 1;
    rc_fill(a, M, Hd, drop_p, key1_0, key1_1, key2_0, key2_1, drop_seed);
    constexpr int NW = 4;
    const int smem = 3 * 2 * (32 * 128) + 3 * 2 * (64 * 64) + Hd * 4;
    static bool flags[64] = {false};
    static bool flags2[64] = {false};
    int rc = rc_set_lds(reinterpret_cast<const void*>(&mlp_rc_fwd_kernel<64, NW, false>), 3 * 2 * (32 * 128) + 3 * 2 * (64 * 64) + 4096 * 4, flags);
    if (rc == MDVIT_OK) rc = rc_set_lds(reinterpret_cast<const void*>(&mlp_rc_fwd_kernel<64, NW, true>), 3 * 2 * (32 * 128) + 3 * 2 * (64 * 64) + 4096 * 4, flags2);
    if (rc != MDVIT_OK) return rc;
    if (g_rc_fwd_variant == 3) {
        static bool f3[64] = {false}, f4[64] = {false};
        rc = rc_set_lds(reinterpret_cast<const void*>(&mlp_rc_fwd3_kernel<64, NW, false>), 3 * 2 * (32 * 128) + 3 * 2 * (64 * 64) + 4096 * 4, f3);
        if (rc == MDVIT_OK) rc = rc_set_lds(reinterpret_cast<const void*>(&mlp_rc_fwd3_kernel<64, NW, true>), 3 * 2 * (32 * 128) + 3 * 2 * (64 * 64) + 4096 * 4, f4);
        if (rc != MDVIT_OK) return rc;
        constexpr int CAP = 3 * 2 * (32 * 128) + 3 * 2 * (64 * 64) + 4096 * 4;
        const dim3 grid(cdiv(M, NW * 32)), block(NW * 64);
        hipStream_t s = (hipStream_t)stream;
        if (g_rc_planes == 1) rc = a.drop ? rc_launch<&mlp_rc_fwd3_kernel<64, NW, true, 3, false, false, true>>(CAP, grid, block, smem, s, a)
                                          : rc_launch<&mlp_rc_fwd3_kernel<64, NW, false, 3, false, false, true>>(CAP, grid, block, smem, s, a);
        else rc = a.drop ? rc_launch<&mlp_rc_fwd3_kernel<64, NW, true>>(CAP, grid, block, smem, s, a) : rc_launch<&mlp_rc_fwd3_kernel<64, NW, false>>(CAP, grid, block, smem, s, a);
        if (rc != MDVIT_OK) return rc;
    } else if (a.drop) hipLaunchKernelGGL((mlp_rc_fwd_kernel<64, NW, true>), dim3(cdiv(M, NW * 32)), dim3(NW * 64), smem, (hipStream_t)stream, a);
    else hipLaunchKernelGGL((mlp_rc_fwd_kernel<64, NW, false>), dim3(cdiv(M, NW * 32)), dim3(NW * 64), smem, (hipStream_t)stream, a);
    MDVIT_LAUNCH_CHECK();
    return MDVIT_OK;
}

extern "C" int mdvit_mlp_rc_dgrad(const float* gm, const float* x, const void* W1p, const float* b1, const void* W2tp, const void* W1tp, float* dx,
                                  int32_t M, int32_t C, int32_t Hd, float drop_p, uint32_t key1_0, uint32_t key1_1, const uint32_t* drop_seed, void* stream) {
    MDVIT_CHECK_ARG(C == 64, MDVIT_E_SHAPE, "mlp_rc_dgrad: built for C = 64 (got %d)", C);
    MDVIT_CHECK_ARG(M > 0 && Hd >= 64 && Hd % 64 == 0 && Hd <= 4096, MDVIT_E_SHAPE, "mlp_rc_dgrad: need M > 0, hidden %% 64 == 0, hidden <= 4096 (M=%d hidden=%d)", M, Hd);
    MDVIT_CHECK_ARG(gm && x && W1p && b1 && W2tp && W1tp && dx, MDVIT_E_SHAPE, "mlp_rc_dgrad: null operand");
    MDVIT_CHECK_ARG(aligned16(gm) && aligned16(x) && aligned16(W1p) && aligned16(b1) && aligned16(W2tp) && aligned16(W1tp) && aligned16(dx), MDVIT_E_ALIGN,
                    "mlp_rc_dgrad: operands must be 16-byte aligned");
    MDVIT_CHECK_ARG(!(drop_p > 0.f) || (long)M * Hd < (1L << 32), MDVIT_E_SHAPE, "mlp_rc_dgrad: dropout index space exceeds 2^32");
    RcArgs a;
    memset(&a, 0, sizeof(a));
    a.gm = gm; a.x = x; a.W1p = (const uint16_t*)W1p; a.b1 = b1; a.W2tp = (const uint16_t*)W2tp; a.W1tp = (const uint16_t*)W1tp; a.dx = dx;
    rc_fill(a, M, Hd, drop_p, key1_0, key1_1, 0, 0, drop_seed);
    constexpr int NW = 4;
    const int smem = 3 * 4 * (32 * 128) + 3 * 2 * (64 * 64) + Hd * 4;
    static bool flags[64] = {false};
    static bool flags2[64] = {false};
    int rc = rc_set_lds(reinterpret_cast<const void*>(&mlp_rc_dgrad_kernel<64, NW, false>), 3 * 4 * (32 * 128) + 3 * 2 * (64 * 64) + 4096 * 4, flags);
    if (rc == MDVIT_OK) rc = rc_set_lds(reinterpret_cast<const void*>(&mlp_rc_dgrad_kernel<64, NW, true>), 3 * 4 * (32 * 128) + 3 * 2 * (64 * 64) + 4096 * 4, flags2);
    if (rc != MDVIT_OK) return rc;
    if (g_rc_planes == 1) {
        constexpr int CAP = 3 * 4 * (32 * 128) + 3 * 2 * (64 * 64) + 4096 * 4;
        rc = a.drop ? rc_launch<&mlp_rc_dgrad_kernel<64, NW, true, true>>(CAP, dim3(cdiv(M, NW * 32)), dim3(NW * 64), smem, (hipStream_t)stream, a)
                    : rc_launch<&mlp_rc_dgrad_kernel<64, NW, false, true>>(CAP, dim3(cdiv(M, NW * 32)), dim3(NW * 64), smem, (hipStream_t)stream, a);
        if (rc != MDVIT_OK) return rc;
    } else if (a.drop) hipLaunchKernelGGL((mlp_rc_dgrad_kernel<64, NW, true>), dim3(cdiv(M, NW * 32)), dim3(NW * 64), smem, (hipStream_t)stream, a);
    else hipLaunchKernelGGL((mlp_rc_dgrad_kernel<64, NW, false>), dim3(cdiv(M, NW * 32)), dim3(NW * 64), smem, (hipStream_t)stream, a);
    MDVIT_LAUNCH_CHECK();
    return MDVIT_OK;
}

static int rc_wgrad_groups(int M) {
    const int ntiles = (M + 31) / 32;
    int g = (ntiles + 3) / 4;
    g = ((g + 7) / 8) * 8;
    return g < 8 ? 8 : (g > 128 ? 128 : g);
}

extern "C" int mdvit_linear_rc_ln(const float* x, const float* gamma, const float* beta, int32_t groups, float eps, float* mean, float* rstd, float* ln_out,
                                  const void* Wp, int64_t wplane, const float* bias, float* y, int64_t ldc, int32_t M, int32_t N, int32_t K, void* stream) {
    MDVIT_CHECK_ARG(K == 64 || K == 128, MDVIT_E_SHAPE, "linear_rc_ln: built for K = 64 / 128 (got %d)", K);
    MDVIT_CHECK_ARG(M > 0 && N >= 32 && N % 32 == 0 && N <= 4096 && groups > 0 && M % groups == 0, MDVIT_E_SHAPE, "linear_rc_ln: bad shape M=%d N=%d groups=%d", M, N, groups);
    MDVIT_CHECK_ARG(x && gamma && beta && mean && rstd && ln_out && Wp && y && ldc >= N && ldc % 4 == 0, MDVIT_E_SHAPE, "linear_rc_ln: bad operands");
    MDVIT_CHECK_ARG(aligned16(x) && aligned16(gamma) && aligned16(beta) && aligned16(ln_out) && aligned16(Wp) && aligned16(y) && aligned16(bias), MDVIT_E_ALIGN,
                    "linear_rc_ln: operands must be 16-byte aligned");
    LinArgs a;
    memset(&a, 0, sizeof(a));
    a.x = x; a.lda = K; a.Wp = (const uint16_t*)Wp; a.wplane = wplane; a.bias = bias; a.y = y; a.ldc = ldc; a.M = M; a.N = N; a.rows_per_scale = 1; a.inv_keep = 1.f;
    a.ln_g = gamma; a.ln_b = beta; a.ln_mean = mean; a.ln_rstd = rstd; a.ln_out = ln_out; a.ln_eps = eps; a.ln_rows_per_group = M / groups;
    const int smem = 3 * 2 * (32 * K * 2) + N * 4;
    hipStream_t s = (hipStream_t)stream;
    const int nw = cdiv(M, 128) >= 512 ? 4 : 2;
    const dim3 grid(cdiv(M, nw * 32)), block(nw * 64);
    if (K == 64) {
        if (nw == 4) hipLaunchKernelGGL((lin_rc_kernel<64, 4, false, false, true>), grid, block, smem, s, a);
        else hipLaunchKernelGGL((lin_rc_kernel<64, 2, false, false, true>), grid, block, smem, s, a);
    } else {
        if (nw == 4) hipLaunchKernelGGL((lin_rc_kernel<128, 4, false, false, true>), grid, block, smem, s, a);
        else hipLaunchKernelGGL((lin_rc_kernel<128, 2, false, false, true>), grid, block, smem, s, a);
    }
    MDVIT_LAUNCH_CHECK();
    return MDVIT_OK;
}

static int rc16_fwd_impl(int hbf, const float* x, const void* W1p, const float* b1, const void* W2p, const float* b2, const float* res, const float* rowscale,
                                  int32_t rows_per_scale, float* h, float* y, int32_t M, int32_t C, int32_t Hd, float drop_p, uint32_t key1_0, uint32_t key1_1,
                                  uint32_t key2_0, uint32_t key2_1, const uint32_t* drop_seed, void* stream) {
    MDVIT_CHECK_ARG(C == 64 || C == 128, MDVIT_E_SHAPE, "mlp_rc16_fwd: built for C = 64 / 128 (got %d)", C);
    MDVIT_CHECK_ARG(M > 0 && Hd >= 64 && Hd % 32 == 0 && Hd <= 4096, MDVIT_E_SHAPE, "mlp_rc16_fwd: need M > 0, hidden %% 32 == 0, hidden <= 4096 (M=%d hidden=%d)", M, Hd);
    MDVIT_CHECK_ARG(x && W1p && b1 && W2p && b2 && res && y, MDVIT_E_SHAPE, "mlp_rc16_fwd: null operand");
    MDVIT_CHECK_ARG(aligned16(x) && aligned16(W1p) && aligned16(b1) && aligned16(W2p) && aligned16(b2) && aligned16(res) && aligned16(y) && aligned16(h), MDVIT_E_ALIGN,
                    "mlp_rc16_fwd: operands must be 16-byte aligned");
    MDVIT_CHECK_ARG(!(drop_p > 0.f) || (long)M * Hd < (1L << 32), MDVIT_E_SHAPE, "mlp_rc16_fwd: dropout index space exceeds 2^32");
    RcArgs a;
    memset(&a, 0, sizeof(a));
    a.x = x; a.W1p = (const uint16_t*)W1p; a.b1 = b1; a.W2p = (const uint16_t*)W2p; a.b2 = b2; a.res = res; a.rowscale = rowscale; a.y = y; a.h = h;
    a.hbf = hbf && h;
    a.rows_per_scale = rows_per_scale > 0 ? rows_per_scale : 1;
    rc_fill(a, M, Hd, drop_p, key1_0, key1_1, key2_0, key2_1, drop_seed);
    constexpr int NW = 8;
    const int smem = 3 * 2 * (32 * C * 2) + 3 * 2 * (C * 64) + Hd * 4;
    const dim3 grid(cdiv(M, NW * 16)), block(NW * 64);
// ... 63 lines not shown
    a.ln = LnPro{gamma, beta, mean, rstd, ln_out, eps, M / groups};
    rc_fill(a, M, Hd, drop_p, key1_0, key1_1, key2_0, key2_1, drop_seed);
    hipStream_t s = (hipStream_t)stream;
    if (C == 64) {
        constexpr int NW = 4;
        const int smem = 3 * 2 * (32 * 128) + 3 * 2 * (64 * 64) + Hd * 4;
        static bool f0[64] = {false}, f1[64] = {false};
        int rc = rc_set_lds(reinterpret_cast<const void*>(&mlp_rc_fwd3_kernel<64, NW, false, 3, false, true>), 3 * 2 * (32 * 128) + 3 * 2 * (64 * 64) + 4096 * 4, f0);
        if (rc == MDVIT_OK) rc = rc_set_lds(reinterpret_cast<const void*>(&mlp_rc_fwd3_kernel<64, NW, true, 3, false, true>), 3 * 2 * (32 * 128) + 3 * 2 * (64 * 64) + 4096 * 4, f1);
        if (rc != MDVIT_OK) return rc;
        if (g_rc_planes == 1) {
            constexpr int CAP = 3 * 2 * (32 * 128) + 3 * 2 * (64 * 64) + 4096 * 4;
            rc = a.drop ? rc_launch<&mlp_rc_fwd3_kernel<64, NW, true, 3, false, true, true>>(CAP, dim3(cdiv(M, NW * 32)), dim3(NW * 64), smem, s, a)
                        : rc_launch<&mlp_rc_fwd3_kernel<64, NW, false, 3, false, true, true>>(CAP, dim3(cdiv(M, NW * 32)), dim3(NW * 64), smem, s, a);
            if (rc != MDVIT_OK) return rc;
        } else if (a.drop) hipLaunchKernelGGL((mlp_rc_fwd3_kernel<64, NW, true, 3, false, true>), dim3(cdiv(M, NW * 32)), dim3(NW * 64), smem, s, a);
        else hipLaunchKernelGGL((mlp_rc_fwd3_kernel<64, NW, false, 3, false, true>), dim3(cdiv(M, NW * 32)), dim3(NW * 64), smem, s, a);
    } else {
        constexpr int NW = 8;
        const int smem = 3 * 2 * (32 * 128 * 2) + 3 * 2 * (128 * 64) + Hd * 4;
        const dim3 grid(cdiv(M, NW * 16)), block(NW * 64);
#define RC16_FWD_LN_LAUNCH(DROPV, STOREV)                                                                                            \
    do {                                                                                                                             \
        static bool fl[64] = {false};                                                                                                \
        const int rc = rc_set_lds(reinterpret_cast<const void*>(&mlp_rc16_fwd_kernel<128, NW, 2, DROPV, STOREV, true>),              \
                                  3 * 2 * (32 * 128 * 2) + 3 * 2 * (128 * 64) + 4096 * 4, fl);                                       \
        if (rc != MDVIT_OK) return rc;                                                                                               \
        if (g_rc_planes == 1) {                                                                                                      \
            const int rc1 = rc_launch<&mlp_rc16_fwd_kernel<128, NW, 2, DROPV, STOREV, true, true>>(3 * 2 * (32 * 256) + 3 * 2 * (128 * 64) + 4096 * 4, grid, block, smem, s, a); \
            if (rc1 != MDVIT_OK) return rc1;                                                                                         \
        } else                                                                                                                       \
        hipLaunchKernelGGL((mlp_rc16_fwd_kernel<128, NW, 2, DROPV, STOREV, true>), grid, block, smem, s, a);                         \
    } while (0)
        if (a.drop) { if (h) RC16_FWD_LN_LAUNCH(true, true); else RC16_FWD_LN_LAUNCH(true, false); }
        else { if (h) RC16_FWD_LN_LAUNCH(false, true); else RC16_FWD_LN_LAUNCH(false, false); }
#undef RC16_FWD_LN_LAUNCH
    }
    MDVIT_LAUNCH_CHECK();
    return MDVIT_OK;
}
extern "C" int mdvit_mlp_rc_fwd_ln(const float* x2, const float* gamma, const float* beta, int32_t groups, float eps, float* mean, float* rstd, float* ln_out,
                                   const void* W1p, const float* b1, const void* W2p, const float* b2, const float* rowscale, int32_t rows_per_scale, float* h,
                                   float* y, int32_t M, int32_t C, int32_t Hd, float drop_p, uint32_t key1_0, uint32_t key1_1, uint32_t key2_0, uint32_t key2_1,
                                   const uint32_t* drop_seed, void* stream) {
    return rc_fwd_ln_impl(0, x2, gamma, beta, groups, eps, mean, rstd, ln_out, W1p, b1, W2p, b2, rowscale, rows_per_scale, h, y, M, C, Hd, drop_p, key1_0, key1_1, key2_0, key2_1, drop_seed, stream);
}
extern "C" int mdvit_mlp_rc_fwd_ln_hbf16(const float* x2, const float* gamma, const float* beta, int32_t groups, float eps, float* mean, float* rstd, float* ln_out,
                                   const void* W1p, const float* b1, const void* W2p, const float* b2, const float* rowscale, int32_t rows_per_scale, float* h,
                                   float* y, int32_t M, int32_t C, int32_t Hd, float drop_p, uint32_t key1_0, uint32_t key1_1, uint32_t key2_0, uint32_t key2_1,
                                   const uint32_t* drop_seed, void* stream) {
    return rc_fwd_ln_impl(1, x2, gamma, beta, groups, eps, mean, rstd, ln_out, W1p, b1, W2p, b2, rowscale, rows_per_scale, h, y, M, C, Hd, drop_p, key1_0, key1_1, key2_0, key2_1, drop_seed, stream);
}

static int rc16_dgrad_impl(int hbf, const float* gm, const float* x, const void* W1p, const float* b1, const void* W2tp, const void* W1tp, float* du, float* dx,
                                    int32_t M, int32_t C, int32_t Hd, float drop_p, uint32_t key1_0, uint32_t key1_1, const uint32_t* drop_seed, void* stream) {
    MDVIT_CHECK_ARG(C == 64 || C == 128, MDVIT_E_SHAPE, "mlp_rc16_dgrad: built for C = 64 / 128 (got %d)", C);
    MDVIT_CHECK_ARG(M > 0 && Hd >= 64 && Hd % 32 == 0 && Hd <= 4096, MDVIT_E_SHAPE, "mlp_rc16_dgrad: need M > 0, hidden %% 32 == 0, hidden <= 4096 (M=%d hidden=%d)", M, Hd);
    MDVIT_CHECK_ARG(gm && x && W1p && b1 && W2tp && W1tp && dx, MDVIT_E_SHAPE, "mlp_rc16_dgrad: null operand");
    MDVIT_CHECK_ARG(aligned16(gm) && aligned16(x) && aligned16(W1p) && aligned16(b1) && aligned16(W2tp) && aligned16(W1tp) && aligned16(dx) && aligned16(du), MDVIT_E_ALIGN,
                    "mlp_rc16_dgrad: operands must be 16-byte aligned");
    MDVIT_CHECK_ARG(!(drop_p > 0.f) || (long)M * Hd < (1L << 32), MDVIT_E_SHAPE, "mlp_rc16_dgrad: dropout index space exceeds 2^32");
    RcArgs a;
    memset(&a, 0, sizeof(a));
    a.gm = gm; a.x = x; a.W1p = (const uint16_t*)W1p; a.b1 = b1; a.W2tp = (const uint16_t*)W2tp; a.W1tp = (const uint16_t*)W1tp; a.dx = dx; a.du = du;
    a.hbf = hbf && du;
    rc_fill(a, M, Hd, drop_p, key1_0, key1_1, 0, 0, drop_seed);
    constexpr int NW = 8;
    const int wbytes = 3 * 4 * (32 * C * 2) + 3 * 2 * (C * 64);
    const int smem = wbytes + Hd * 4;
    const dim3 grid(cdiv(M, NW * 16)), block(NW * 64);
    hipStream_t s = (hipStream_t)stream;
#define RC16_DGRAD_LAUNCH(CV, OCCV, DROPV, STOREV)                                                                                   \
    do {                                                                                                                             \
        static bool fl[64] = {false};                                                                                                \
        const int rc = rc_set_lds(reinterpret_cast<const void*>(&mlp_rc16_dgrad_kernel<CV, NW, OCCV, DROPV, STOREV>),                \
                                  3 * 4 * (32 * CV * 2) + 3 * 2 * (CV * 64) + 4096 * 4, fl);                                         \
        if (rc != MDVIT_OK) return rc;                                                                                               \
        if (g_rc_planes == 1) {                                                                                                      \
            const int rc1 = rc_launch<&mlp_rc16_dgrad_kernel<CV, NW, OCCV, DROPV, STOREV, true>>(3 * 4 * (32 * CV * 2) + 3 * 2 * (CV * 64) + 4096 * 4, grid, block, smem, s, a); \
            if (rc1 != MDVIT_OK) return rc1;                                                                                         \
        } else                                                                                                                       \
        hipLaunchKernelGGL((mlp_rc16_dgrad_kernel<CV, NW, OCCV, DROPV, STOREV>), grid, block, smem, s, a);                           \
    } while (0)
    if (C == 128) {
        if (a.drop) { if (du) RC16_DGRAD_LAUNCH(128, 2, true, true); else RC16_DGRAD_LAUNCH(128, 2, true, false); }
        else { if (du) RC16_DGRAD_LAUNCH(128, 2, false, true); else RC16_DGRAD_LAUNCH(128, 2, false, false); }
    } else {
        if (a.drop) { if (du) RC16_DGRAD_LAUNCH(64, 4, true, true); else RC16_DGRAD_LAUNCH(64, 4, true, false); }
        else { if (du) RC16_DGRAD_LAUNCH(64, 4, false, true); else RC16_DGRAD_LAUNCH(64, 4, false, false); }
    }
#undef RC16_DGRAD_LAUNCH
    MDVIT_LAUNCH_CHECK();
    return MDVIT_OK;
}
extern "C" int mdvit_mlp_rc16_dgrad(const float* gm, const float* x, const void* W1p, const float* b1, const void* W2tp, const void* W1tp, float* du, float* dx,
                                    int32_t M, int32_t C, int32_t Hd, float drop_p, uint32_t key1_0, uint32_t key1_1, const uint32_t* drop_seed, void* stream) {
    return rc16_dgrad_impl(0, gm, x, W1p, b1, W2tp, W1tp, du, dx, M, C, Hd, drop_p, key1_0, key1_1, drop_seed, stream);
}
extern "C" int mdvit_mlp_rc16_dgrad_hbf16(const float* gm, const float* x, const void* W1p, const float* b1, const void* W2tp, const void* W1tp, float* du, float* dx,
                                    int32_t M, int32_t C, int32_t Hd, float drop_p, uint32_t key1_0, uint32_t key1_1, const uint32_t* drop_seed, void* stream) {
    return rc16_dgrad_impl(1, gm, x, W1p, b1, W2tp, W1tp, du, dx, M, C, Hd, drop_p, key1_0, key1_1, drop_seed, stream);
}

extern "C" int mdvit_linear_rc(const float* x, int64_t lda, const void* Wp, int64_t wplane, const float* bias, float* y, int64_t ldc, int32_t M, int32_t N, int32_t K,
                               float drop_p, uint32_t key0, uint32_t key1, const float* rowscale, int32_t rows_per_scale, const float* residual, int64_t ldr,
                               const uint32_t* drop_seed, void* stream) {
    MDVIT_CHECK_ARG(K == 64 || K == 128, MDVIT_E_SHAPE, "linear_rc: built for K = 64 / 128 (got %d)", K);
    MDVIT_CHECK_ARG(M > 0 && N >= 32 && N % 32 == 0 && N <= 4096, MDVIT_E_SHAPE, "linear_rc: need M > 0, N %% 32 == 0, N <= 4096 (M=%d N=%d)", M, N);
    MDVIT_CHECK_ARG(x && Wp && y && lda >= K && ldc >= N && lda % 4 == 0 && ldc % 4 == 0 && (!residual || (ldr >= N && ldr % 4 == 0)), MDVIT_E_SHAPE, "linear_rc: bad operands");
    MDVIT_CHECK_ARG(aligned16(x) && aligned16(Wp) && aligned16(y) && aligned16(bias) && aligned16(residual), MDVIT_E_ALIGN, "linear_rc: operands must be 16-byte aligned");
    MDVIT_CHECK_ARG(drop_p >= 0.f && drop_p < 1.f && (!(drop_p > 0.f) || (long)M * N < (1L << 32)), MDVIT_E_SHAPE, "linear_rc: bad dropout arguments");
    MDVIT_CHECK_ARG(residual || (drop_p == 0.f && rowscale == nullptr), MDVIT_E_SHAPE, "linear_rc: dropout / row scale come with the residual epilogue");
    LinArgs a;
    memset(&a, 0, sizeof(a));
    a.x = x; a.lda = lda; a.Wp = (const uint16_t*)Wp; a.wplane = wplane; a.bias = bias; a.y = y; a.ldc = ldc; a.residual = residual; a.ldr = ldr;
    a.rowscale = rowscale; a.rows_per_scale = rows_per_scale > 0 ? rows_per_scale : 1; a.M = M; a.N = N;
    a.k0 = key0; a.k1 = key1; a.thresh = mdvit_drop_thresh(drop_p); a.inv_keep = drop_p > 0.f ? 1.f / (1.f - drop_p) : 1.f; a.seed = drop_seed;
    const int smem = 3 * 2 * (32 * K * 2) + N * 4;
    hipStream_t s = (hipStream_t)stream;
    const bool full = residual != nullptr, drop = drop_p > 0.f;
    const int nw = cdiv(M, 128) >= 512 ? 4 : 2;
    const dim3 grid(cdiv(M, nw * 32)), block(nw * 64);
#define LIN_RC_LAUNCH(KV, FULLV, DROPV)                                                                          \
    do {                                                                                                         \
        if (nw == 4) hipLaunchKernelGGL((lin_rc_kernel<KV, 4, FULLV, DROPV>), grid, block, smem, s, a);          \
        else hipLaunchKernelGGL((lin_rc_kernel<KV, 2, FULLV, DROPV>), grid, block, smem, s, a);                  \
    } while (0)
    if (K == 64) {
        if (full) { if (drop) LIN_RC_LAUNCH(64, true, true); else LIN_RC_LAUNCH(64, true, false); }
        else LIN_RC_LAUNCH(64, false, false);
    } else {
        if (full) { if (drop) LIN_RC_LAUNCH(128, true, true); else LIN_RC_LAUNCH(128, true, false); }
        else LIN_RC_LAUNCH(128, false, false);
    }
#undef LIN_RC_LAUNCH
    MDVIT_LAUNCH_CHECK();
    return MDVIT_OK;
}

extern "C" size_t mdvit_mlp_rc_wgrad_ws_bytes(int32_t M, int32_t C, int32_t Hd) {
    return sizeof(float) * (size_t)rc_wgrad_groups(M) * (2u * (size_t)Hd * C + Hd);
}

extern "C" int mdvit_mlp_rc_wgrad(const float* gm, const float* x, const void* W1p, const float* b1, const void* W2tp, float* dW1, float* db1, float* dW2,
                                  void* ws, size_t ws_bytes, int32_t M, int32_t C, int32_t Hd, float drop_p, uint32_t key1_0, uint32_t key1_1,
                                  const uint32_t* drop_seed, int32_t accumulate, void* stream) {
    MDVIT_CHECK_ARG(C == 64, MDVIT_E_SHAPE, "mlp_rc_wgrad: built for C = 64 (got %d)", C);
    MDVIT_CHECK_ARG(M > 0 && Hd >= 256 && Hd % 256 == 0, MDVIT_E_SHAPE, "mlp_rc_wgrad: need M > 0, hidden %% 256 == 0 (M=%d hidden=%d)", M, Hd);
    MDVIT_CHECK_ARG(gm && x && W1p && b1 && W2tp && dW1 && db1 && dW2, MDVIT_E_SHAPE, "mlp_rc_wgrad: null operand");
    MDVIT_CHECK_ARG(aligned16(gm) && aligned16(x) && aligned16(W1p) && aligned16(W2tp) && aligned16(dW1) && aligned16(db1) && aligned16(dW2) && aligned16(ws),
                    MDVIT_E_ALIGN, "mlp_rc_wgrad: operands must be 16-byte aligned");
    MDVIT_CHECK_ARG(!(drop_p > 0.f) || (long)M * Hd < (1L << 32), MDVIT_E_SHAPE, "mlp_rc_wgrad: dropout index space exceeds 2^32");
    const size_t need = mdvit_mlp_rc_wgrad_ws_bytes(M, C, Hd);
    MDVIT_CHECK_ARG(ws && ws_bytes >= need, MDVIT_E_WORKSPACE, "mlp_rc_wgrad: workspace too small: need %zu bytes (mdvit_mlp_rc_wgrad_ws_bytes), got %zu", need, ws_bytes);
    RcArgs a;
    memset(&a, 0, sizeof(a));
    a.gm = gm; a.x = x; a.W1p = (const uint16_t*)W1p; a.b1 = b1; a.W2tp = (const uint16_t*)W2tp; a.part = (float*)ws;
    rc_fill(a, M, Hd, drop_p, key1_0, key1_1, 0, 0, drop_seed);
    a.groups = rc_wgrad_groups(M);
    a.tiles_per_group = cdiv((M + 31) / 32, a.groups);
    const int roles = Hd / 256;
    if (g_rc_planes == 1) {
        if (a.drop) hipLaunchKernelGGL((mlp_rc_wgrad_kernel<64, true, false, true>), dim3(a.groups * roles), dim3(512), 0, (hipStream_t)stream, a);
        else hipLaunchKernelGGL((mlp_rc_wgrad_kernel<64, false, false, true>), dim3(a.groups * roles), dim3(512), 0, (hipStream_t)stream, a);
    } else if (a.drop) hipLaunchKernelGGL((mlp_rc_wgrad_kernel<64, true>), dim3(a.groups * roles), dim3(512), 0, (hipStream_t)stream, a);
    else hipLaunchKernelGGL((mlp_rc_wgrad_kernel<64, false>), dim3(a.groups * roles), dim3(512), 0, (hipStream_t)stream, a);
    MDVIT_LAUNCH_CHECK();
    const int n0 = Hd * C, n2 = Hd;
    hipLaunchKernelGGL(rc_reduce_kernel, dim3(cdiv((2L * n0 + n2) / 4, 256)), dim3(256), 0, (hipStream_t)stream, (const float*)ws, a.groups, (long)(2L * n0 + n2), n0, dW1,
                       n0, dW2, n2, db1, accumulate);
    MDVIT_LAUNCH_CHECK();
    return MDVIT_OK;
}

extern "C" int mdvit_mlp_rc_bwd(const float* gm, const float* x, const void* W1p, const float* b1, const void* W2tp, const void* W1tp, float* dx_parts,
                                float* dW1, float* db1, float* dW2, void* ws, size_t ws_bytes, int32_t M, int32_t C, int32_t Hd, float drop_p,
                                uint32_t key1_0, uint32_t key1_1, const uint32_t* drop_seed, int32_t accumulate, void* stream) {
    MDVIT_CHECK_ARG(C == 64, MDVIT_E_SHAPE, "mlp_rc_bwd: built for C = 64 (got %d)", C);
    MDVIT_CHECK_ARG(M > 0 && (Hd == 256 || Hd == 512), MDVIT_E_SHAPE, "mlp_rc_bwd: need M > 0, hidden in {256, 512} (M=%d hidden=%d)", M, Hd);
    MDVIT_CHECK_ARG(gm && x && W1p && b1 && W2tp && W1tp && dx_parts && dW1 && db1 && dW2, MDVIT_E_SHAPE, "mlp_rc_bwd: null operand");
    MDVIT_CHECK_ARG(aligned16(gm) && aligned16(x) && aligned16(W1p) && aligned16(W2tp) && aligned16(W1tp) && aligned16(dx_parts) && aligned16(dW1) && aligned16(db1) &&
                    aligned16(dW2) && aligned16(ws), MDVIT_E_ALIGN, "mlp_rc_bwd: operands must be 16-byte aligned");
    MDVIT_CHECK_ARG(!(drop_p > 0.f) || (long)M * Hd < (1L << 32), MDVIT_E_SHAPE, "mlp_rc_bwd: dropout index space exceeds 2^32");
    const size_t need = mdvit_mlp_rc_wgrad_ws_bytes(M, C, Hd);
    MDVIT_CHECK_ARG(ws && ws_bytes >= need, MDVIT_E_WORKSPACE, "mlp_rc_bwd: workspace too small: need %zu bytes (mdvit_mlp_rc_wgrad_ws_bytes), got %zu", need, ws_bytes);
    RcArgs a;
    memset(&a, 0, sizeof(a));
    a.gm = gm; a.x = x; a.W1p = (const uint16_t*)W1p; a.b1 = b1; a.W2tp = (const uint16_t*)W2tp; a.W1tp = (const uint16_t*)W1tp; a.dx = dx_parts; a.part = (float*)ws;
    rc_fill(a, M, Hd, drop_p, key1_0, key1_1, 0, 0, drop_seed);
    a.groups = rc_wgrad_groups(M);
    a.tiles_per_group = cdiv((M + 31) / 32, a.groups);
    const int roles = Hd / 256;
    static bool f0[64] = {false}, f1[64] = {false};
    int rc = rc_set_lds(reinterpret_cast<const void*>(&mlp_rc_wgrad_kernel<64, true, true>), RC_BWD_LDS, f0);
    if (rc == MDVIT_OK) rc = rc_set_lds(reinterpret_cast<const void*>(&mlp_rc_wgrad_kernel<64, false, true>), RC_BWD_LDS, f1);
    if (rc != MDVIT_OK) return rc;
    if (g_rc_planes == 1) {
        rc = a.drop ? rc_launch<&mlp_rc_wgrad_kernel<64, true, true, true>>(RC_BWD_LDS, dim3(a.groups * roles), dim3(512), RC_BWD_LDS, (hipStream_t)stream, a)
                    : rc_launch<&mlp_rc_wgrad_kernel<64, false, true, true>>(RC_BWD_LDS, dim3(a.groups * roles), dim3(512), RC_BWD_LDS, (hipStream_t)stream, a);
        if (rc != MDVIT_OK) return rc;
    } else if (a.drop) hipLaunchKernelGGL((mlp_rc_wgrad_kernel<64, true, true>), dim3(a.groups * roles), dim3(512), RC_BWD_LDS, (hipStream_t)stream, a);
    else hipLaunchKernelGGL((mlp_rc_wgrad_kernel<64, false, true>), dim3(a.groups * roles), dim3(512), RC_BWD_LDS, (hipStream_t)stream, a);
    MDVIT_LAUNCH_CHECK();
    const int n0 = Hd * C, n2 = Hd;
    hipLaunchKernelGGL(rc_reduce_kernel, dim3(cdiv((2L * n0 + n2) / 4, 256)), dim3(256), 0, (hipStream_t)stream, (const float*)ws, a.groups, (long)(2L * n0 + n2), n0, dW1,
                       n0, dW2, n2, db1, accumulate);
    MDVIT_LAUNCH_CHECK();
    return MDVIT_OK;
}
```

### mdvit_amd/ops.py

```python
from __future__ import annotations

import ctypes as C
import itertools
import os
import weakref
from typing import Optional, Tuple

import torch

from . import _lib
from ._lib import GemmDesc, call

_key_counter = itertools.count(1)
_POISON = os.environ.get("MDVIT_POISON", "0") == "1"


def _empty(*a, **k):
    t = torch.empty(*a, **k)
    if _POISON and t.is_floating_point():
        t.fill_(float("nan"))
    return t


def _empty_like(x):
# ... 1030 lines not shown
                dWc[i] = torch.zeros((hid, W[i].numel() // hid), device=dev, dtype=torch.float32)
            if dbc[i] is None:
                dbc[i] = torch.zeros_like(b[i])
        dWf = [_empty((hid, Q * hid), device=dev, dtype=torch.float32) for _ in range(G)]
        sW = [_sink_of(w) for w in W]
        sb = [_sink_of(t) for t in b]
        sunk = all(t is not None for t in sW) and all(t is not None for t in sb)
        dW = list(sW) if sunk else [_empty_like(w) for w in W]
        db = list(sb) if sunk else [_empty_like(t) for t in b]
        items = [(g, q) for g in range(G) for q in range(Q)]
        A_blocks = _vp_array([_p(Wf[g][:, q * hid:]) for g, q in items])
        b_ptrs, dbc_ptrs = _vp_array([_p(b[g * Q + q]) for g, q in items]), _vp_array([_p(dbc[g * Q + q]) for g, q in items])
        for q in range(Q):
            Cq = W[q].numel() // hid
            gemm_grouped([dWc[g * Q + q] for g in range(G)], [W[g * Q + q] for g in range(G)], [dWf[g][:, q * hid:] for g in range(G)],
                         hid, hid, Cq, lda=Cq, ldb=Cq, ldc=Q * hid, trans_b=True)
        call("mdvit_compose_bias_bwd", len(items), A_blocks, ldf, b_ptrs, dbc_ptrs, _vp_array([_p(dWf[g][:, q * hid:]) for g, q in items]), Q * hid,
             None, 0, hid, hid, _stream())

        def param_grads():
            for q in range(Q):
                Cq = W[q].numel() // hid
                gemm_grouped([Wf[g][:, q * hid:] for g in range(G)], [dWc[g * Q + q] for g in range(G)], [dW[g * Q + q] for g in range(G)],
                             hid, Cq, hid, lda=ldf, ldb=Cq, ldc=Cq, trans_a=True, trans_b=False, accumulate=sunk)
            call("mdvit_compose_bias_bwd", len(items), A_blocks, ldf, b_ptrs, dbc_ptrs, None, 0, _vp_array([_p(db[g * Q + q]) for g, q in items]), int(sunk),
                 hid, hid, _stream())

        if sunk:
            with _on_side(*dWc, *dbc, foreign="all"):
                param_grads()
        else:
            param_grads()
        if sunk:
            return (None, None) + tuple(dWf) + (None,) * (2 * G * Q)
        return (None, None) + tuple(dWf) + tuple(dW) + tuple(db)


def compose_heads(Wf_list, W_lists, b_lists):
    G, Q = len(Wf_list), len(W_lists[0])
    flatW = [W_lists[g][q] for g in range(G) for q in range(Q)]
    flatb = [b_lists[g][q] for g in range(G) for q in range(Q)]
    out = _ComposeHeads.apply(G, Q, *Wf_list, *flatW, *flatb)
    Wc, bc = out[:G * Q], out[G * Q:]
    return [[(Wc[g * Q + q], bc[g * Q + q]) for q in range(Q)] for g in range(G)]


_mlp_recompute = os.environ.get("MDVIT_MLP_RECOMPUTE", "1") != "0"
_mlp_fused = os.environ.get("MDVIT_MLP_FUSED", "1") != "0"
_mlp_recompute_maxc = int(os.environ.get("MDVIT_MLP_RECOMPUTE_MAXC", "128"))
_mlp_rc = os.environ.get("MDVIT_MLP_RC", "1") != "0"
_mlp_rc16 = os.environ.get("MDVIT_MLP_RC16", "1") != "0"
_mlp_rc_bwd = os.environ.get("MDVIT_MLP_RC_BWD", "1")
_lib.on_load(lambda lib: lib.mdvit_block_config({"0": 0, "1": 1}.get(_mlp_rc_bwd, 2)))


def _mlp_rc_ok(Cin, Hd, b1, b2, res, W1, W2, M) -> bool:
    return (_mlp_rc and _mlp_recompute and _gemm_precision >= 1 and Cin == 64 and Hd % 256 == 0 and Hd <= 4096 and b1 is not None and b2 is not None and res is not None
            and W1.is_contiguous() and W2.is_contiguous() and M * Hd < (1 << 32))


def _mlp_rc16_ok(Cin, Hd, b1, W1, W2, M) -> bool:
    return (_mlp_rc16 and _gemm_precision >= 1 and Cin == 128 and Hd % 32 == 0 and Hd <= 4096 and b1 is not None and W1.is_contiguous() and W2.is_contiguous()
            and M * Hd < (1 << 32))


class _MlpResidual(torch.autograd.Function):
    @staticmethod
    def forward(ctx, x, res, W1, b1, W2, b2, rowscale, drop_p, rows_per_scale):
        ctx.set_materialize_grads(False)
        _chk(x, res, W1, b1, W2, b2, rowscale)
        M, Cin = x.shape
        Hd = W1.shape[0]
        k1 = _next_key() if drop_p > 0 else (0, 0)
        k2 = _next_key() if drop_p > 0 else (0, 0)
        if _mlp_rc_ok(Cin, Hd, b1, b2, res, W1, W2, M):
            out = _empty((M, Cin), device=x.device, dtype=torch.float32)
            W1p, W2p = _wplanes(W1, False, 2), _wplanes(W2, False, 2)
            call("mdvit_mlp_rc_fwd", _p(x), _p(W1p), _p(b1), _p(W2p), _p(b2), _p(res), _p(rowscale), rows_per_scale, _p(out), M, Cin, Hd,
                 drop_p, k1[0], k1[1], k2[0], k2[1], _seed_ptr() if drop_p > 0 else None, _stream())
            del W1p, W2p
            ctx.save_for_backward(x, None, None, W1, W2, rowscale)
            ctx.meta = (drop_p, k1, k2, rows_per_scale)
            ctx.b1_ref, ctx.b2_ref = b1, b2
            ctx.rc = True
            return out
        ctx.rc = False
        h = _empty((M, Hd), device=x.device, dtype=torch.float32)
        if _mlp_recompute and _mlp_fused and _gemm_precision >= 1 and Cin == 64 and Hd % 64 == 0 and b1 is not None and b2 is not None \
                and res is not None and W1.is_contiguous() and W2.is_contiguous() and M * Hd < (1 << 32):
            out = _empty((M, Cin), device=x.device, dtype=torch.float32)
            call("mdvit_mlp_fwd_f32", _p(x), _p(W1), _p(b1), _p(W2), _p(b2), _p(res), _p(rowscale), rows_per_scale, _p(h), _p(out), M, Cin, Hd,
                 drop_p, k1[0], k1[1], k2[0], k2[1], _seed_ptr() if drop_p > 0 else None, _stream())
            ctx.save_for_backward(x, None, h, W1, W2, rowscale)
            ctx.meta = (drop_p, k1, k2, rows_per_scale)
            ctx.b1_ref, ctx.b2_ref = b1, b2
            return out
        if _mlp_recompute and _mlp_recompute_maxc >= 128 and b2 is not None and res is not None and _mlp_rc16_ok(Cin, Hd, b1, W1, W2, M):
            out = _empty((M, Cin), device=x.device, dtype=torch.float32)
            W1p, W2p = _wplanes(W1, False, 2), _wplanes(W2, False, 2)
            call("mdvit_mlp_rc16_fwd", _p(x), _p(W1p), _p(b1), _p(W2p), _p(b2), _p(res), _p(rowscale), rows_per_scale, _p(h), _p(out), M, Cin, Hd,
                 drop_p, k1[0], k1[1], k2[0], k2[1], _seed_ptr() if drop_p > 0 else None, _stream())
            del W1p, W2p
            ctx.save_for_backward(x, None, h, W1, W2, rowscale)
            ctx.meta = (drop_p, k1, k2, rows_per_scale)
            ctx.b1_ref, ctx.b2_ref = b1, b2
            return out
        plane = _plane_ok(M, Hd, Cin) and W1.is_contiguous()
        plane2 = _plane_ok(M, Cin, Hd, res is not None) and W2.is_contiguous()
        if _mlp_recompute and _gemm_precision >= 1 and Cin <= _mlp_recompute_maxc and Cin % 32 == 0 and Hd % 4 == 0:
            u = None
            if plane:
                gemm_nt(x, W1, h, M, Hd, Cin, bias=b1, epi=_lib.EPI_GELU_DUAL, e_drop=drop_p, e_key=k1)
            else:
                gemm(_p(x), _p(W1), _p(h), M, Hd, Cin, lda=Cin, ldb=Cin, ldc=Hd, bias=_p(b1), epi=_lib.EPI_GELU_DUAL, e_drop=drop_p, e_key=k1)
        else:
            u = _empty_like(h)
            if plane:
                gemm_nt(x, W1, h, M, Hd, Cin, bias=b1, U=u, epi=_lib.EPI_GELU_DUAL, e_drop=drop_p, e_key=k1)
            else:
                gemm(_p(x), _p(W1), _p(u), M, Hd, Cin, lda=Cin, ldb=Cin, ldc=Hd, bias=_p(b1), out2=_p(h),
                     epi=_lib.EPI_GELU_DUAL, e_drop=drop_p, e_key=k1)
        out = _empty((M, Cin), device=x.device, dtype=torch.float32)
        if plane2:
            gemm_nt(h, W2, out, M, Cin, Hd, bias=b2, e_drop=drop_p, e_key=k2, e_rowscale=rowscale, e_rows_per_scale=rows_per_scale, residual=res)
        else:
            gemm(_p(h), _p(W2), _p(out), M, Cin, Hd, lda=Hd, ldb=Hd, ldc=Cin, bias=_p(b2),
                 e_drop=drop_p, e_key=k2, e_rowscale=_p(rowscale), e_rows_per_scale=rows_per_scale, residual=_p(res), ldr=Cin)
        ctx.save_for_backward(x, u, h, W1, W2, rowscale)
        ctx.meta = (drop_p, k1, k2, rows_per_scale)
        ctx.b1_ref, ctx.b2_ref = b1, b2
        return out

    @staticmethod
    def backward(ctx, g):
        if g is None:
            return (None,) * 9
        x, u, h, W1, W2, rowscale = ctx.saved_tensors
        drop_p, k1, k2, rps = ctx.meta
        g = _c(g)
        M, Cin = x.shape
        Hd = W1.shape[0]
        dev = x.device
        dW1 = db1 = dW2 = db2 = None
        sinks = [_sink_of(t) for t in (W1, ctx.b1_ref, W2, ctx.b2_ref)] if not _dgrad_only else [None] * 4
        sunk = not _dgrad_only and all(t is not None for t in sinks)
        if ctx.rc:
            masked = drop_p > 0 or rowscale is not None
            want_w = not _dgrad_only
            gm = _empty_like(g) if masked else g
            if want_w and not sunk:
                db2 = _empty((Cin,), device=dev, dtype=torch.float32)
            if masked or want_w:
                wsp, wsb, _keep = _partials_ws(Cin, dev) if want_w else (None, 0, None)
                call("mdvit_colsum_f32", _p(g), Cin, _p(sinks[3] if sunk else db2) if want_w else None, _p(gm) if masked else None, wsp, wsb, M, Cin,
                     drop_p, k2[0], k2[1], _p(rowscale), rps, int(sunk), _seed_ptr() if drop_p > 0 else None, _stream())
            W1p, W2tp, W1tp = _wplanes(W1, False, 2), _wplanes(W2, True, 2), _wplanes(W1, True, 2)
            fused = want_w and Hd in (256, 512) and (_mlp_rc_bwd == "1" or (_mlp_rc_bwd == "auto" and not (sunk and _side_stream is not None)))
            if fused:
                roles = Hd // 256
                parts = _empty((roles, M, Cin), device=dev, dtype=torch.float32)
                wsb = _lib.load().mdvit_mlp_rc_wgrad_ws_bytes(M, Cin, Hd)
                ws = _empty((wsb // 4,), device=dev, dtype=torch.float32)
                if sunk:
                    tgt, accf = (sinks[0], sinks[1], sinks[2]), 1
                    db2 = None
                else:
                    dW1, db1, dW2 = _empty_like(W1), _empty((Hd,), device=dev, dtype=torch.float32), _empty_like(W2)
                    tgt, accf = (dW1, db1, dW2), 0
                call("mdvit_mlp_rc_bwd", _p(gm), _p(x), _p(W1p), _p(ctx.b1_ref), _p(W2tp), _p(W1tp), _p(parts), _p(tgt[0]), _p(tgt[1]), _p(tgt[2]), _p(ws), wsb,
                     M, Cin, Hd, drop_p, k1[0], k1[1], _seed_ptr() if drop_p > 0 else None, accf, _stream())
                if roles == 1:
                    dx = parts[0]
                else:
                    dx = _empty_like(x)
                    call("mdvit_sum_batch", _p(parts), _p(dx), roles, M * Cin, _stream())
                del W1p, W2tp, W1tp
                return dx, g, dW1, db1, dW2, db2, None, None, None
            dx = _empty_like(x)
            call("mdvit_mlp_rc_dgrad", _p(gm), _p(x), _p(W1p), _p(ctx.b1_ref), _p(W2tp), _p(W1tp), _p(dx), M, Cin, Hd,
                 drop_p, k1[0], k1[1], _seed_ptr() if drop_p > 0 else None, _stream())
            if want_w:
                wsb = _lib.load().mdvit_mlp_rc_wgrad_ws_bytes(M, Cin, Hd)
                if sunk:
                    with _on_side(gm, x, W1p, W2tp):
                        ws = _empty((wsb // 4,), device=dev, dtype=torch.float32)
                        call("mdvit_mlp_rc_wgrad", _p(gm), _p(x), _p(W1p), _p(ctx.b1_ref), _p(W2tp), _p(sinks[0]), _p(sinks[1]), _p(sinks[2]), _p(ws), wsb,
                             M, Cin, Hd, drop_p, k1[0], k1[1], _seed_ptr() if drop_p > 0 else None, 1, _stream())
                    db2 = None
                else:
                    dW1, db1, dW2 = _empty_like(W1), _empty((Hd,), device=dev, dtype=torch.float32), _empty_like(W2)
                    ws = _empty((wsb // 4,), device=dev, dtype=torch.float32)
                    call("mdvit_mlp_rc_wgrad", _p(gm), _p(x), _p(W1p), _p(ctx.b1_ref), _p(W2tp), _p(dW1), _p(db1), _p(dW2), _p(ws), wsb,
                         M, Cin, Hd, drop_p, k1[0], k1[1], _seed_ptr() if drop_p > 0 else None, 0, _stream())
            del W1p, W2tp, W1tp
            return dx, g, dW1, db1, dW2, db2, None, None, None
        if not _dgrad_only and not sunk:
            db2 = torch.zeros((Cin,), device=dev, dtype=torch.float32)
        masked = drop_p > 0 or rowscale is not None
        gm = _empty_like(g) if masked else g
        if masked:
            call("mdvit_colsum_f32", _p(g), Cin, None, _p(gm), None, 0, M, Cin,
                 drop_p, k2[0], k2[1], _p(rowscale), rps, 0, _seed_ptr() if drop_p > 0 else None, _stream())
        dx = _empty_like(x)
        if u is None and _mlp_fused and _gemm_precision >= 1 and Cin == 64 and Hd % 64 == 0 and W1.is_contiguous() and W2.is_contiguous():
            du = None if _dgrad_only else _empty_like(h)
            W2t, W1t = wt(W2), wt(W1)
            call("mdvit_mlp_bwd_dgrad_f32", _p(gm), _p(x), _p(W1), _p(ctx.b1_ref), _p(W2t), _p(W1t), _p(du), _p(dx), M, Cin, Hd,
                 drop_p, k1[0], k1[1], _seed_ptr() if drop_p > 0 else None, _stream())
            del W2t, W1t
        elif u is None and _mlp_rc16_ok(Cin, Hd, ctx.b1_ref, W1, W2, M):
            du = None if _dgrad_only else _empty_like(h)
            W1p, W2tp, W1tp = _wplanes(W1, False, 2), _wplanes(W2, True, 2), _wplanes(W1, True, 2)
            call("mdvit_mlp_rc16_dgrad", _p(gm), _p(x), _p(W1p), _p(ctx.b1_ref), _p(W2tp), _p(W1tp), _p(du), _p(dx), M, Cin, Hd,
                 drop_p, k1[0], k1[1], _seed_ptr() if drop_p > 0 else None, _stream())
            del W1p, W2tp, W1tp
        else:
            du = _empty_like(h)
            if u is None and (_plane_rc or _gemm_precision == 2) and _use_plane_gemm and Cin % 32 == 0 and W1.is_contiguous() and W2.is_contiguous():
                gemm_nt(to_planes(gm), W2, du, M, Hd, Cin, w_transposed=True, epi=_lib.EPI_DGELU, rc=(to_planes(x), W1, ctx.b1_ref, Cin),
                        e_drop=drop_p, e_key=k1)
            elif u is None:
                _dgrad(gm, W2, du, M, Hd, Cin, Hd, epi=_lib.EPI_DGELU, rc=(_p(x), Cin, _p(W1), Cin, _p(ctx.b1_ref), Cin), e_drop=drop_p, e_key=k1)
            else:
                _dgrad(gm, W2, du, M, Hd, Cin, Hd, epi=_lib.EPI_DGELU, gelu_u=_p(u), ldu=Hd, e_drop=drop_p, e_key=k1)
            _dgrad(du, W1, dx, M, Cin, Hd, Cin, allow_split=True)
        if not _dgrad_only:
            if sunk:
                dW1_, db1_, dW2_, _ = sinks
                with _on_side(gm, h, du, x):
                    gemm(_p(gm), _p(h), _p(dW2_), Cin, Hd, M, lda=Cin, ldb=Hd, ldc=Hd, trans_a=True, trans_b=False, allow_split=True, accumulate=True,
                         colsum_a=_p(sinks[3]))
                    gemm(_p(du), _p(x), _p(dW1_), Hd, Cin, M, lda=Hd, ldb=Cin, ldc=Cin, trans_a=True, trans_b=False, allow_split=True, accumulate=True,
                         colsum_a=_p(db1_))
                db2 = None
            else:
                dW2 = _empty_like(W2)
                gemm(_p(gm), _p(h), _p(dW2), Cin, Hd, M, lda=Cin, ldb=Hd, ldc=Hd, trans_a=True, trans_b=False, allow_split=True, colsum_a=_p(db2))
                dW1 = _empty_like(W1)
                db1 = torch.zeros((Hd,), device=dev, dtype=torch.float32)
                gemm(_p(du), _p(x), _p(dW1), Hd, Cin, M, lda=Hd, ldb=Cin, ldc=Cin, trans_a=True, trans_b=False, allow_split=True, colsum_a=_p(db1))
        return dx, g, dW1, db1, dW2, db2, None, None, None


def mlp_residual(x, res, W1, b1, W2, b2, rowscale=None, drop_p=0.0, rows_per_scale=1):
    shp = res.shape
    out = _MlpResidual.apply(_c(x).view(-1, shp[-1]), _c(res).view(-1, shp[-1]), W1, b1, W2, b2, rowscale,
                             float(drop_p), int(rows_per_scale))
    return out.view(shp)


class _LayerNorm(torch.autograd.Function):

    @staticmethod
    def forward(ctx, x, gamma, beta, eps, fork):
        ctx.set_materialize_grads(False)
        _chk(x, gamma, beta)
        M, Cn = x.shape
        groups = gamma.shape[0] if gamma.dim() == 2 else 1
        if M % groups:
            raise ValueError(f"layer_norm: {M} rows are not {groups} equal groups")
        y = _empty_like(x)
        mean = _empty((M,), device=x.device, dtype=torch.float32)
        rstd = _empty_like(mean)
        call("mdvit_layernorm_fwd", _p(x), _p(gamma), _p(beta), _p(y), _p(mean), _p(rstd), M, Cn, groups, eps, _stream())
        ctx.save_for_backward(x, gamma, mean, rstd)
        if fork:
            return y, x.view_as(x)
# ... 1597 lines not shown
```

Before: 533.4 images/s.

## Fold fc2 dropout/rowscale mask into MLP backward kernels' gradient load

Adds masked variants of the recompute MLP dgrad, wgrad and fused bwd kernels that apply the fc2 dropout and drop-path rowscale to the incoming gradient as it is loaded. This removes the separate colsum/mask pass and its full-size masked-gradient buffer in the block and autograd backward paths, enabled by default. The mask is recomputed inside the kernels, so the kernels doing the recompute do extra RNG and scaling work. The 16-token path with weight gradients still writes the masked gradient out as a side output for the later weight-gradient GEMMs.

```diff
diff --git a/include/mdvit_hip.h b/include/mdvit_hip.h
--- a/include/mdvit_hip.h
+++ b/include/mdvit_hip.h
@@ -151,6 +151,25 @@
                      float* dW2, void* ws, size_t ws_bytes, int32_t M, int32_t C, int32_t hidden, float drop_p, uint32_t key1_0, uint32_t key1_1,
                      const uint32_t* drop_seed, int32_t accumulate, void* stream);
 size_t mdvit_mlp_rc_wgrad_ws_bytes(int32_t M, int32_t C, int32_t hidden);
+int mdvit_mlp_rc_dgrad_masked(const float* g, const float* x, const void* W1p, const float* b1, const void* W2tp, const void* W1tp, float* dx, int32_t M, int32_t C,
+                              int32_t hidden, float drop_p, uint32_t key1_0, uint32_t key1_1, const uint32_t* drop_seed, float mask_drop_p, uint32_t mask_key0,
+                              uint32_t mask_key1, const uint32_t* mask_seed, const float* rowscale, int32_t rows_per_scale, void* stream);
+int mdvit_mlp_rc16_dgrad_masked(const float* g, const float* x, const void* W1p, const float* b1, const void* W2tp, const void* W1tp, float* du, float* dx, float* gm_out,
+                                int32_t M, int32_t C, int32_t hidden, float drop_p, uint32_t key1_0, uint32_t key1_1, const uint32_t* drop_seed, float mask_drop_p,
+                                uint32_t mask_key0, uint32_t mask_key1, const uint32_t* mask_seed, const float* rowscale, int32_t rows_per_scale, void* stream);
+int mdvit_mlp_rc16_dgrad_masked_hbf16(const float* g, const float* x, const void* W1p, const float* b1, const void* W2tp, const void* W1tp, float* du, float* dx,
+                                      float* gm_out, int32_t M, int32_t C, int32_t hidden, float drop_p, uint32_t key1_0, uint32_t key1_1, const uint32_t* drop_seed,
+                                      float mask_drop_p, uint32_t mask_key0, uint32_t mask_key1, const uint32_t* mask_seed, const float* rowscale,
+                                      int32_t rows_per_scale, void* stream);
+int mdvit_mlp_rc_wgrad_masked(const float* g, const float* x, const void* W1p, const float* b1, const void* W2tp, float* dW1, float* db1, float* dW2, void* ws,
+                              size_t ws_bytes, int32_t M, int32_t C, int32_t hidden, float drop_p, uint32_t key1_0, uint32_t key1_1, const uint32_t* drop_seed,
+                              float mask_drop_p, uint32_t mask_key0, uint32_t mask_key1, const uint32_t* mask_seed, const float* rowscale, int32_t rows_per_scale,
+                              int32_t accumulate, void* stream);
+int mdvit_mlp_rc_bwd_masked(const float* g, const float* x, const void* W1p, const float* b1, const void* W2tp, const void* W1tp, float* dx_parts, float* dW1, float* db1,
+                            float* dW2, void* ws, size_t ws_bytes, int32_t M, int32_t C, int32_t hidden, float drop_p, uint32_t key1_0, uint32_t key1_1,
+                            const uint32_t* drop_seed, float mask_drop_p, uint32_t mask_key0, uint32_t mask_key1, const uint32_t* mask_seed, const float* rowscale,
+                            int32_t rows_per_scale, int32_t accumulate, void* stream);
+int mdvit_mlp_mask_config(int32_t fold);
 int mdvit_gemm_ledger(int32_t enable);
 int mdvit_gemm_ledger_read(int32_t index, char* name, int32_t cap, int64_t* launches, double* flop, double* bytes);
 int mdvit_gemm_sampler(const char* symbol, int32_t stride);
diff --git a/mdvit_amd/_lib.py b/mdvit_amd/_lib.py
--- a/mdvit_amd/_lib.py
+++ b/mdvit_amd/_lib.py
@@ -147,6 +147,12 @@
     "mdvit_mlp_rc16_dgrad_hbf16": [vp, vp, vp, vp, vp, vp, vp, vp, i32, i32, i32, f32, u32, u32, vp, vp],
     "mdvit_mlp_rc_wgrad": [vp, vp, vp, vp, vp, vp, vp, vp, vp, C.c_size_t, i32, i32, i32, f32, u32, u32, vp, i32, vp],
     "mdvit_mlp_rc_bwd": [vp, vp, vp, vp, vp, vp, vp, vp, vp, vp, vp, C.c_size_t, i32, i32, i32, f32, u32, u32, vp, i32, vp],
+    "mdvit_mlp_rc_dgrad_masked": [vp, vp, vp, vp, vp, vp, vp, i32, i32, i32, f32, u32, u32, vp, f32, u32, u32, vp, vp, i32, vp],
+    "mdvit_mlp_rc16_dgrad_masked": [vp, vp, vp, vp, vp, vp, vp, vp, vp, i32, i32, i32, f32, u32, u32, vp, f32, u32, u32, vp, vp, i32, vp],
+    "mdvit_mlp_rc16_dgrad_masked_hbf16": [vp, vp, vp, vp, vp, vp, vp, vp, vp, i32, i32, i32, f32, u32, u32, vp, f32, u32, u32, vp, vp, i32, vp],
+    "mdvit_mlp_rc_wgrad_masked": [vp, vp, vp, vp, vp, vp, vp, vp, vp, C.c_size_t, i32, i32, i32, f32, u32, u32, vp, f32, u32, u32, vp, vp, i32, i32, vp],
+    "mdvit_mlp_rc_bwd_masked": [vp, vp, vp, vp, vp, vp, vp, vp, vp, vp, vp, C.c_size_t, i32, i32, i32, f32, u32, u32, vp, f32, u32, u32, vp, vp, i32, i32, vp],
+    "mdvit_mlp_mask_config": [i32],
     "mdvit_imgconv_fwd": [vp, vp, vp, i32, i32, i32, i32, i32, i32, vp],
     "mdvit_imgconv_wgrad": [vp, vp, vp, vp, C.c_size_t, i32, i32, i32, i32, i32, i32, i32, vp],
     "mdvit_maxpool3x3s2_fwd": [vp, vp, vp, i32, i32, i32, i32, vp],
diff --git a/mdvit_amd/csrc/block.hip b/mdvit_amd/csrc/block.hip
--- a/mdvit_amd/csrc/block.hip
+++ b/mdvit_amd/csrc/block.hip
@@ -263,21 +263,28 @@
     }
 
     const bool masked = d.drop_p > 0.f || d.rowscale2 != nullptr;
-    float* gm2 = masked ? S.take(T * C) : const_cast<float*>(dy);
+    const bool rc16_path = mode != MLP_RC && mlp_rc16(d) && d.fc2t_p && d.fc1t_p;
+    const int fold_case = !want_w ? MDVIT_MASK_FOLD_AUX : (mode == MLP_RC ? MDVIT_MASK_FOLD_FULL64 : MDVIT_MASK_FOLD_FULL128);
+    const bool fold = masked && (mode == MLP_RC || rc16_path) && (g_rc_mask_fold & fold_case) != 0;
+    const float m_p = fold ? d.drop_p : 0.f;
+    const float* m_rs = fold ? d.rowscale2 : nullptr;
+    const bool need_gm2 = masked && (!fold || (want_w && rc16_path));
+    float* gm2 = need_gm2 ? S.take(T * C) : const_cast<float*>(dy);
+    float* gm2_w = fold ? nullptr : gm2;
     float* tmp = A.take(T * C);
     float* dcur2 = tmp;
     const float* dcur2_b = nullptr;
     float* du = nullptr;
     if (mode == MLP_RC) {
-        if (masked || want_w) {
+        if ((masked && !fold) || want_w) {
             const size_t pb = want_w ? mdvit_partials_ws_bytes(C) : 0;
             void* pw = want_w ? (defer ? S.take_bytes(pb) : A.take_bytes(pb)) : nullptr;
             if (want_w && defer) {
                 int nb = 0;
-                BLK_RUN(mdvit_colsum_parts(dy, C, masked ? gm2 : nullptr, pw, pb, M, C, d.drop_p, d.key_fc2[0], d.key_fc2[1], d.rowscale2, N_tok, seed, s, &nb));
+                BLK_RUN(mdvit_colsum_parts(dy, C, masked ? gm2_w : nullptr, pw, pb, M, C, d.drop_p, d.key_fc2[0], d.key_fc2[1], d.rowscale2, N_tok, seed, s, &nb));
                 late[n_late++] = Late{(const float*)pw, 1, nb, C, G.fc2_b, 0, nullptr};
             } else {
-                BLK_RUN(mdvit_colsum_f32(dy, C, want_w ? G.fc2_b : nullptr, masked ? gm2 : nullptr, pw, pb, M, C, d.drop_p, d.key_fc2[0], d.key_fc2[1], d.rowscale2, N_tok,
+                BLK_RUN(mdvit_colsum_f32(dy, C, want_w ? G.fc2_b : nullptr, masked ? gm2_w : nullptr, pw, pb, M, C, d.drop_p, d.key_fc2[0], d.key_fc2[1], d.rowscale2, N_tok,
                                          acc, seed, s));
             }
         }
@@ -287,30 +294,35 @@
             float* parts = roles == 1 ? dcur2 : A.take((long)roles * T * C);
             const size_t wb = mdvit_mlp_rc_wgrad_ws_bytes(M, C, Hd);
             void* ww = A.take_bytes(wb);
-            BLK_RUN(mdvit_mlp_rc_bwd(gm2, sv.cur2, d.fc1_p, d.fc1_b, d.fc2t_p, d.fc1t_p, parts, G.fc1_w, G.fc1_b, G.fc2_w, ww, wb, M, C, Hd, d.drop_p, d.key_fc1[0],
-                                     d.key_fc1[1], seed, acc, s));
+            BLK_RUN(mdvit_mlp_rc_bwd_masked(gm2, sv.cur2, d.fc1_p, d.fc1_b, d.fc2t_p, d.fc1t_p, parts, G.fc1_w, G.fc1_b, G.fc2_w, ww, wb, M, C, Hd, d.drop_p, d.key_fc1[0],
+                                            d.key_fc1[1], seed, m_p, d.key_fc2[0], d.key_fc2[1], seed, m_rs, N_tok, acc, s));
             dcur2 = parts;
             dcur2_b = roles == 2 ? parts + T * C : nullptr;
         } else {
-        BLK_RUN(mdvit_mlp_rc_dgrad(gm2, sv.cur2, d.fc1_p, d.fc1_b, d.fc2t_p, d.fc1t_p, dcur2, M, C, Hd, d.drop_p, d.key_fc1[0], d.key_fc1[1], seed, s));
+        BLK_RUN(mdvit_mlp_rc_dgrad_masked(gm2, sv.cur2, d.fc1_p, d.fc1_b, d.fc2t_p, d.fc1t_p, dcur2, M, C, Hd, d.drop_p, d.key_fc1[0], d.key_fc1[1], seed, m_p, d.key_fc2[0],
+                                          d.key_fc2[1], seed, m_rs, N_tok, s));
         if (want_w) {
             const size_t wb = mdvit_mlp_rc_wgrad_ws_bytes(M, C, Hd);
             void* ww = S.take_bytes(wb);
             if (!A.dry) { const int rc = fork_side(d, st, side); if (rc != MDVIT_OK) return rc; }
-            BLK_RUN(mdvit_mlp_rc_wgrad(gm2, sv.cur2, d.fc1_p, d.fc1_b, d.fc2t_p, G.fc1_w, G.fc1_b, G.fc2_w, ww, wb, M, C, Hd, d.drop_p, d.key_fc1[0], d.key_fc1[1], seed,
-                                       acc, side));
+            BLK_RUN(mdvit_mlp_rc_wgrad_masked(gm2, sv.cur2, d.fc1_p, d.fc1_b, d.fc2t_p, G.fc1_w, G.fc1_b, G.fc2_w, ww, wb, M, C, Hd, d.drop_p, d.key_fc1[0], d.key_fc1[1],
+                                              seed, m_p, d.key_fc2[0], d.key_fc2[1], seed, m_rs, N_tok, acc, side));
         }
         }
     } else {
-        if (masked) BLK_RUN(mdvit_colsum_f32(dy, C, nullptr, gm2, nullptr, 0, M, C, d.drop_p, d.key_fc2[0], d.key_fc2[1], d.rowscale2, N_tok, 0, seed, s));
+        if (masked && !fold) BLK_RUN(mdvit_colsum_f32(dy, C, nullptr, gm2, nullptr, 0, M, C, d.drop_p, d.key_fc2[0], d.key_fc2[1], d.rowscale2, N_tok, 0, seed, s));
         MdvitGemmDesc g;
         int rc = MDVIT_OK;
         const bool hb = hbf16(d);
         if (hb && !(d.fc2t_p && d.fc1t_p)) return mdvit_set_error(MDVIT_E_SHAPE, "block_bwd: store_bf16 needs the transposed fc weight planes (the 16-token MLP backward)");
         if (mlp_rc16(d) && d.fc2t_p && d.fc1t_p) {
             du = want_w ? S.take(hb ? (T * Hd + 1) / 2 : T * Hd) : nullptr;
-            if (hb) BLK_RUN(mdvit_mlp_rc16_dgrad_hbf16(gm2, sv.cur2, d.fc1_p, d.fc1_b, d.fc2t_p, d.fc1t_p, du, dcur2, M, C, Hd, d.drop_p, d.key_fc1[0], d.key_fc1[1], seed, s));
-            else BLK_RUN(mdvit_mlp_rc16_dgrad(gm2, sv.cur2, d.fc1_p, d.fc1_b, d.fc2t_p, d.fc1t_p, du, dcur2, M, C, Hd, d.drop_p, d.key_fc1[0], d.key_fc1[1], seed, s));
+            const float* g_in = fold ? dy : gm2;
+            float* g_out = fold && want_w ? gm2 : nullptr;
+            if (hb) BLK_RUN(mdvit_mlp_rc16_dgrad_masked_hbf16(g_in, sv.cur2, d.fc1_p, d.fc1_b, d.fc2t_p, d.fc1t_p, du, dcur2, g_out, M, C, Hd, d.drop_p, d.key_fc1[0],
+                                                              d.key_fc1[1], seed, m_p, d.key_fc2[0], d.key_fc2[1], seed, m_rs, N_tok, s));
+            else BLK_RUN(mdvit_mlp_rc16_dgrad_masked(g_in, sv.cur2, d.fc1_p, d.fc1_b, d.fc2t_p, d.fc1t_p, du, dcur2, g_out, M, C, Hd, d.drop_p, d.key_fc1[0], d.key_fc1[1],
+                                                     seed, m_p, d.key_fc2[0], d.key_fc2[1], seed, m_rs, N_tok, s));
         } else {
             du = S.take(T * Hd);
             gemm_init(g, d);
diff --git a/mdvit_amd/csrc/common.h b/mdvit_amd/csrc/common.h
--- a/mdvit_amd/csrc/common.h
+++ b/mdvit_amd/csrc/common.h
@@ -54,6 +54,9 @@
                               const float* rowscale, int rows_per_scale, const uint32_t* seed, hipStream_t stream, int* nblk);
 int mdvit_colsum_parts(const float* A, long lda, float* masked, void* ws, size_t ws_bytes, int M, int N, float drop_p, uint32_t key0, uint32_t key1,
                        const float* rowscale, int rows_per_scale, const uint32_t* seed, hipStream_t stream, int* nblk);
+constexpr int MDVIT_MASK_FOLD_AUX = 2, MDVIT_MASK_FOLD_FULL128 = 4, MDVIT_MASK_FOLD_FULL64 = 8;
+constexpr int MDVIT_MASK_FOLD_DEFAULT = MDVIT_MASK_FOLD_AUX | MDVIT_MASK_FOLD_FULL128 | MDVIT_MASK_FOLD_FULL64;
+extern int g_rc_mask_fold;
 void mdvit_layernorm_bwd_next_dy2(const float* dy2);
 constexpr int MDVIT_MAX_PARTIAL_ROWS = 2048;
 #define MDVIT_CHECK_PARTIALS_WS(ws, ws_bytes, nblk, n, what)                                                              \
diff --git a/mdvit_amd/csrc/mlp_rc.hip b/mdvit_amd/csrc/mlp_rc.hip
--- a/mdvit_amd/csrc/mlp_rc.hip
+++ b/mdvit_amd/csrc/mlp_rc.hip
@@ -76,9 +76,35 @@
 template <int K>
 __device__ __forceinline__ void rc_ln_rows32(float4 (&a)[K / 16], float4 (&b)[K / 16], int row, int rowc, int M, int lhi, const LnPro ln);
 
+struct RcMask {
+    const float* rowscale; float* gm_out; const uint32_t* seed;
+    int on, drop, rows_per_scale; uint32_t k0, k1, thresh; float inv_keep;
+};
+__device__ __forceinline__ float4 rc_mask4(float4 a, float rsc, bool drop, uint32_t k0, uint32_t k1, uint32_t idx4, uint32_t thresh, float inv_keep) {
+    float ds[4] = {rsc, rsc, rsc, rsc};
+    if (drop) {
+        const float4 d4 = mdvit_drop_scale4(k0, k1, idx4, thresh, inv_keep);
+        ds[0] *= d4.x; ds[1] *= d4.y; ds[2] *= d4.z; ds[3] *= d4.w;
+    }
+    return make_float4(a.x * ds[0], a.y * ds[1], a.z * ds[2], a.w * ds[3]);
+}
+template <int C, int STEP>
+__device__ __forceinline__ void rc_mask_rows(float4 (&a)[C / STEP], float4 (&b)[C / STEP], int rowc, int sub, const RcMask& mk) {
+    const float rsc = mk.rowscale ? mk.rowscale[rowc / mk.rows_per_scale] : 1.f;
+    uint32_t s0 = 0, s1 = 0;
+    if (mk.seed) { s0 = mk.seed[0]; s1 = mk.seed[1]; }
+    const uint32_t k0 = mk.k0 ^ s0, k1 = mk.k1 + s1;
+    const uint32_t i0 = (uint32_t)((long)rowc * C + 8 * sub);
+#pragma unroll
+    for (int i = 0; i < C / STEP; ++i) {
+        a[i] = rc_mask4(a[i], rsc, mk.drop != 0, k0, k1, i0 + STEP * i, mk.thresh, mk.inv_keep);
+        b[i] = rc_mask4(b[i], rsc, mk.drop != 0, k0, k1, i0 + STEP * i + 4, mk.thresh, mk.inv_keep);
+    }
+}
+
 template <int C, bool LNP = false>
 __device__ __forceinline__ void rc_load_rows(const float* __restrict__ src, int row, int M, int lhi, rc_bf16x8 (&hi)[C / 16], rc_bf16x8 (&lo)[C / 16],
-                                             const LnPro* ln = nullptr) {
+                                             const LnPro* ln = nullptr, const RcMask* mk = nullptr) {
     const float* p = src + (long)min(row, M - 1) * C + 8 * lhi;
     float4 a[C / 16], b[C / 16];
 #pragma unroll
@@ -87,6 +113,7 @@
         b[kb] = *reinterpret_cast<const float4*>(p + 16 * kb + 4);
     }
     if constexpr (LNP) rc_ln_rows32<C>(a, b, row, min(row, M - 1), M, lhi, *ln);
+    if (mk && mk->on) rc_mask_rows<C, 16>(a, b, min(row, M - 1), lhi, *mk);
 #pragma unroll
     for (int kb = 0; kb < C / 16; ++kb) {
         const float v[8] = {a[kb].x, a[kb].y, a[kb].z, a[kb].w, b[kb].x, b[kb].y, b[kb].z, b[kb].w};
@@ -208,6 +235,7 @@
     int hbf;
     float* h;
     LnPro ln;
+    RcMask mk;
     float* part;
     int M, Hd, rows_per_scale;
     int drop; uint32_t k1a, k1b, k2a, k2b, thresh; float inv_keep;
@@ -592,7 +620,7 @@
     for (int i = tid; i < p.Hd / 4; i += NW * 64) reinterpret_cast<float4*>(sB1)[i] = reinterpret_cast<const float4*>(p.b1)[i];
     rc_bf16x8 xh[KB], xl[KB], gh[KB], gl[KB];
     rc_load_rows<C>(p.x, row, p.M, lhi, xh, xl);
-    rc_load_rows<C>(p.gm, row, p.M, lhi, gh, gl);
+    rc_load_rows<C>(p.gm, row, p.M, lhi, gh, gl, nullptr, &p.mk);
     rc_f32x16 dxacc[CB];
 #pragma unroll
     for (int cb = 0; cb < CB; ++cb)
@@ -793,18 +821,29 @@
     const int srow = tid >> 4, sc4 = tid & 15;
     const int soff = srow * 128 + (((sc4 >> 1) ^ rc_swz<128>(srow)) << 4) + (sc4 & 1) * 8;
     float4 rx, rg;
+    float rsc = 1.f;
+    uint32_t mk0 = p.mk.k0, mk1 = p.mk.k1;
+    if (p.mk.on && p.mk.seed) { mk0 ^= p.mk.seed[0]; mk1 += p.mk.seed[1]; }
     auto load_tile = [&](int t) __attribute__((always_inline)) {
         const int row = t * 32 + srow, rc = min(row, p.M - 1);
         rx = *reinterpret_cast<const float4*>(p.x + (long)rc * C + sc4 * 4);
         rg = *reinterpret_cast<const float4*>(p.gm + (long)rc * C + sc4 * 4);
+        if (p.mk.on) {
+            if (p.mk.rowscale) {
+                const int r0 = min(t * 32, p.M - 1), q0 = r0 / p.mk.rows_per_scale, e0 = (q0 + 1) * p.mk.rows_per_scale;
+                const int q = p.mk.rows_per_scale >= 32 ? q0 + (rc >= e0 ? 1 : 0) : rc / p.mk.rows_per_scale;
+                rsc = p.mk.rowscale[q];
+            }
+        }
         if (row >= p.M) rg = make_float4(0.f, 0.f, 0.f, 0.f);
     };
-    auto store_tile = [&](int buf) __attribute__((always_inline)) {
+    auto store_tile = [&](int buf, int t) __attribute__((always_inline)) {
         char* b = smem + buf * 4 * TP;
         uint2 hi, lo;
         mdvit_split_bf16x3(rx, hi, lo);
         *reinterpret_cast<rc_u2*>(b + soff) = rc_u2{hi.x, hi.y};
         *reinterpret_cast<rc_u2*>(b + TP + soff) = rc_u2{lo.x, lo.y};
+        if (p.mk.on) rg = rc_mask4(rg, rsc, p.mk.drop != 0, mk0, mk1, (uint32_t)((long)min(t * 32 + srow, p.M - 1) * C + sc4 * 4), p.mk.thresh, p.mk.inv_keep);
         mdvit_split_bf16x3(rg, hi, lo);
         *reinterpret_cast<rc_u2*>(b + 2 * TP + soff) = rc_u2{hi.x, hi.y};
         *reinterpret_cast<rc_u2*>(b + 3 * TP + soff) = rc_u2{lo.x, lo.y};
@@ -819,7 +858,7 @@
     }
     if (t_beg < t_end) {
         load_tile(t_beg);
-        store_tile(0);
+        store_tile(0, t_beg);
     }
     __syncthreads();
     for (int t = t_beg; t < t_end; ++t) {
@@ -912,7 +951,7 @@
             const int tok = t * 32 + tblk * 16 + l15;
             if (tok < p.M) *reinterpret_cast<float4*>(p.dx + ((long)role * p.M + tok) * C + cblk * 16 + 4 * g4) = make_float4(acc[0], acc[1], acc[2], acc[3]);
         }
-        if (t + 1 < t_end) store_tile(buf ^ 1);
+        if (t + 1 < t_end) store_tile(buf ^ 1, t + 1);
         __syncthreads();
     }
 
@@ -974,7 +1013,7 @@
 
 template <int C, bool LNP = false>
 __device__ __forceinline__ void rc16_load_rows(const float* __restrict__ src, int row, int M, int g, rc_bf16x8 (&hi)[C / 32], rc_bf16x8 (&lo)[C / 32],
-                                               const LnPro* ln = nullptr) {
+                                               const LnPro* ln = nullptr, const RcMask* mk = nullptr) {
     const float* p = src + (long)min(row, M - 1) * C + 8 * g;
     float4 a[C / 32], b[C / 32];
 #pragma unroll
@@ -983,6 +1022,16 @@
         b[ks] = *reinterpret_cast<const float4*>(p + 32 * ks + 4);
     }
     if constexpr (LNP && C == 128) rc16_ln_rows128(a, b, row, min(row, M - 1), M, g, *ln);
+    if (mk && mk->on) {
+        rc_mask_rows<C, 32>(a, b, min(row, M - 1), g, *mk);
+        if (mk->gm_out && row < M) {
+#pragma unroll
+            for (int ks = 0; ks < C / 32; ++ks) {
+                *reinterpret_cast<float4*>(mk->gm_out + (long)row * C + 8 * g + 32 * ks) = a[ks];
+                *reinterpret_cast<float4*>(mk->gm_out + (long)row * C + 8 * g + 32 * ks + 4) = b[ks];
+            }
+        }
+    }
 #pragma unroll
     for (int ks = 0; ks < C / 32; ++ks) {
         const float v[8] = {a[ks].x, a[ks].y, a[ks].z, a[ks].w, b[ks].x, b[ks].y, b[ks].z, b[ks].w};
@@ -1208,7 +1257,7 @@
     for (int i = tid; i < p.Hd / 4; i += NW * 64) reinterpret_cast<float4*>(sB1)[i] = reinterpret_cast<const float4*>(p.b1)[i];
     rc_bf16x8 xh[KS], xl[KS], mh[KS], ml[KS];
     rc16_load_rows<C>(p.x, row, p.M, g, xh, xl);
-    rc16_load_rows<C>(p.gm, row, p.M, g, mh, ml);
+    rc16_load_rows<C>(p.gm, row, p.M, g, mh, ml, nullptr, &p.mk);
     rc_f32x4 dacc[CT];
 #pragma unroll
     for (int ct = 0; ct < CT; ++ct) dacc[ct] = rc_f32x4{0.f, 0.f, 0.f, 0.f};
@@ -1413,6 +1462,20 @@
     a.drop = drop_p > 0.f; a.k1a = k10; a.k1b = k11; a.k2a = k20; a.k2b = k21;
     a.thresh = mdvit_drop_thresh(drop_p); a.inv_keep = 1.f / (1.f - drop_p);
     a.seed = seed;
+}
+
+int rc_mask_fill(RcMask& m, const char* who, int M, int C, float drop_p, uint32_t key0, uint32_t key1, const uint32_t* seed, const float* rowscale, int rows_per_scale,
+                 float* gm_out) {
+    MDVIT_CHECK_ARG(drop_p >= 0.f && drop_p < 1.f, MDVIT_E_SHAPE, "%s: mask drop_p must lie in [0, 1)", who);
+    MDVIT_CHECK_ARG(!(drop_p > 0.f) || (long)M * C < (1L << 32), MDVIT_E_SHAPE, "%s: mask index space exceeds 2^32", who);
+    MDVIT_CHECK_ARG(aligned16(gm_out), MDVIT_E_ALIGN, "%s: gm_out must be 16-byte aligned", who);
+    memset(&m, 0, sizeof(m));
+    m.on = drop_p > 0.f || rowscale != nullptr;
+    if (!m.on) return MDVIT_OK;
+    m.drop = drop_p > 0.f; m.k0 = key0; m.k1 = key1; m.seed = m.drop ? seed : nullptr;
+    m.thresh = mdvit_drop_thresh(drop_p); m.inv_keep = 1.f / (1.f - drop_p);
+    m.rowscale = rowscale; m.rows_per_scale = rows_per_scale > 0 ? rows_per_scale : 1; m.gm_out = gm_out;
+    return MDVIT_OK;
 }
 
 }
@@ -1481,8 +1544,8 @@
     return MDVIT_OK;
 }
 
-extern "C" int mdvit_mlp_rc_dgrad(const float* gm, const float* x, const void* W1p, const float* b1, const void* W2tp, const void* W1tp, float* dx,
-                                  int32_t M, int32_t C, int32_t Hd, float drop_p, uint32_t key1_0, uint32_t key1_1, const uint32_t* drop_seed, void* stream) {
+static int rc_dgrad_impl(const RcMask* mk, const float* gm, const float* x, const void* W1p, const float* b1, const void* W2tp, const void* W1tp, float* dx,
+                         int32_t M, int32_t C, int32_t Hd, float drop_p, uint32_t key1_0, uint32_t key1_1, const uint32_t* drop_seed, void* stream) {
     MDVIT_CHECK_ARG(C == 64, MDVIT_E_SHAPE, "mlp_rc_dgrad: built for C = 64 (got %d)", C);
     MDVIT_CHECK_ARG(M > 0 && Hd >= 64 && Hd % 64 == 0 && Hd <= 4096, MDVIT_E_SHAPE, "mlp_rc_dgrad: need M > 0, hidden %% 64 == 0, hidden <= 4096 (M=%d hidden=%d)", M, Hd);
     MDVIT_CHECK_ARG(gm && x && W1p && b1 && W2tp && W1tp && dx, MDVIT_E_SHAPE, "mlp_rc_dgrad: null operand");
@@ -1493,6 +1556,7 @@
     memset(&a, 0, sizeof(a));
     a.gm = gm; a.x = x; a.W1p = (const uint16_t*)W1p; a.b1 = b1; a.W2tp = (const uint16_t*)W2tp; a.W1tp = (const uint16_t*)W1tp; a.dx = dx;
     rc_fill(a, M, Hd, drop_p, key1_0, key1_1, 0, 0, drop_seed);
+    if (mk) a.mk = *mk;
     constexpr int NW = 4;
     const int smem = 3 * 4 * (32 * 128) + 3 * 2 * (64 * 64) + Hd * 4;
     static bool flags[64] = {false};
@@ -1509,6 +1573,20 @@
     else hipLaunchKernelGGL((mlp_rc_dgrad_kernel<64, NW, false>), dim3(cdiv(M, NW * 32)), dim3(NW * 64), smem, (hipStream_t)stream, a);
     MDVIT_LAUNCH_CHECK();
     return MDVIT_OK;
+}
+
+extern "C" int mdvit_mlp_rc_dgrad(const float* gm, const float* x, const void* W1p, const float* b1, const void* W2tp, const void* W1tp, float* dx,
+                                  int32_t M, int32_t C, int32_t Hd, float drop_p, uint32_t key1_0, uint32_t key1_1, const uint32_t* drop_seed, void* stream) {
+    return rc_dgrad_impl(nullptr, gm, x, W1p, b1, W2tp, W1tp, dx, M, C, Hd, drop_p, key1_0, key1_1, drop_seed, stream);
+}
+extern "C" int mdvit_mlp_rc_dgrad_masked(const float* g, const float* x, const void* W1p, const float* b1, const void* W2tp, const void* W1tp, float* dx,
+                                         int32_t M, int32_t C, int32_t Hd, float drop_p, uint32_t key1_0, uint32_t key1_1, const uint32_t* drop_seed,
+                                         float mask_drop_p, uint32_t mask_key0, uint32_t mask_key1, const uint32_t* mask_seed, const float* rowscale,
+                                         int32_t rows_per_scale, void* stream) {
+    RcMask mk;
+    const int rc = rc_mask_fill(mk, "mlp_rc_dgrad_masked", M, C, mask_drop_p, mask_key0, mask_key1, mask_seed, rowscale, rows_per_scale, nullptr);
+    if (rc != MDVIT_OK) return rc;
+    return rc_dgrad_impl(&mk, g, x, W1p, b1, W2tp, W1tp, dx, M, C, Hd, drop_p, key1_0, key1_1, drop_seed, stream);
 }
 
 static int rc_wgrad_groups(int M) {
@@ -1678,7 +1756,7 @@
     return rc_fwd_ln_impl(1, x2, gamma, beta, groups, eps, mean, rstd, ln_out, W1p, b1, W2p, b2, rowscale, rows_per_scale, h, y, M, C, Hd, drop_p, key1_0, key1_1, key2_0, key2_1, drop_seed, stream);
 }
 
-static int rc16_dgrad_impl(int hbf, const float* gm, const float* x, const void* W1p, const float* b1, const void* W2tp, const void* W1tp, float* du, float* dx,
+static int rc16_dgrad_impl(const RcMask* mk, int hbf, const float* gm, const float* x, const void* W1p, const float* b1, const void* W2tp, const void* W1tp, float* du, float* dx,
                                     int32_t M, int32_t C, int32_t Hd, float drop_p, uint32_t key1_0, uint32_t key1_1, const uint32_t* drop_seed, void* stream) {
     MDVIT_CHECK_ARG(C == 64 || C == 128, MDVIT_E_SHAPE, "mlp_rc16_dgrad: built for C = 64 / 128 (got %d)", C);
     MDVIT_CHECK_ARG(M > 0 && Hd >= 64 && Hd % 32 == 0 && Hd <= 4096, MDVIT_E_SHAPE, "mlp_rc16_dgrad: need M > 0, hidden %% 32 == 0, hidden <= 4096 (M=%d hidden=%d)", M, Hd);
@@ -1691,6 +1769,7 @@
     a.gm = gm; a.x = x; a.W1p = (const uint16_t*)W1p; a.b1 = b1; a.W2tp = (const uint16_t*)W2tp; a.W1tp = (const uint16_t*)W1tp; a.dx = dx; a.du = du;
     a.hbf = hbf && du;
     rc_fill(a, M, Hd, drop_p, key1_0, key1_1, 0, 0, drop_seed);
+    if (mk) a.mk = *mk;
     constexpr int NW = 8;
     const int wbytes = 3 * 4 * (32 * C * 2) + 3 * 2 * (C * 64);
     const int smem = wbytes + Hd * 4;
@@ -1721,11 +1800,29 @@
 }
 extern "C" int mdvit_mlp_rc16_dgrad(const float* gm, const float* x, const void* W1p, const float* b1, const void* W2tp, const void* W1tp, float* du, float* dx,
                                     int32_t M, int32_t C, int32_t Hd, float drop_p, uint32_t key1_0, uint32_t key1_1, const uint32_t* drop_seed, void* stream) {
-    return rc16_dgrad_impl(0, gm, x, W1p, b1, W2tp, W1tp, du, dx, M, C, Hd, drop_p, key1_0, key1_1, drop_seed, stream);
+    return rc16_dgrad_impl(nullptr, 0, gm, x, W1p, b1, W2tp, W1tp, du, dx, M, C, Hd, drop_p, key1_0, key1_1, drop_seed, stream);
 }
 extern "C" int mdvit_mlp_rc16_dgrad_hbf16(const float* gm, const float* x, const void* W1p, const float* b1, const void* W2tp, const void* W1tp, float* du, float* dx,
                                     int32_t M, int32_t C, int32_t Hd, float drop_p, uint32_t key1_0, uint32_t key1_1, const uint32_t* drop_seed, void* stream) {
-    return rc16_dgrad_impl(1, gm, x, W1p, b1, W2tp, W1tp, du, dx, M, C, Hd, drop_p, key1_0, key1_1, drop_seed, stream);
+    return rc16_dgrad_impl(nullptr, 1, gm, x, W1p, b1, W2tp, W1tp, du, dx, M, C, Hd, drop_p, key1_0, key1_1, drop_seed, stream);
+}
+extern "C" int mdvit_mlp_rc16_dgrad_masked(const float* g, const float* x, const void* W1p, const float* b1, const void* W2tp, const void* W1tp, float* du, float* dx,
+                                           float* gm_out, int32_t M, int32_t C, int32_t Hd, float drop_p, uint32_t key1_0, uint32_t key1_1, const uint32_t* drop_seed,
+                                           float mask_drop_p, uint32_t mask_key0, uint32_t mask_key1, const uint32_t* mask_seed, const float* rowscale,
+                                           int32_t rows_per_scale, void* stream) {
+    RcMask mk;
+    const int rc = rc_mask_fill(mk, "mlp_rc16_dgrad_masked", M, C, mask_drop_p, mask_key0, mask_key1, mask_seed, rowscale, rows_per_scale, gm_out);
+    if (rc != MDVIT_OK) return rc;
+    return rc16_dgrad_impl(&mk, 0, g, x, W1p, b1, W2tp, W1tp, du, dx, M, C, Hd, drop_p, key1_0, key1_1, drop_seed, stream);
+}
+extern "C" int mdvit_mlp_rc16_dgrad_masked_hbf16(const float* g, const float* x, const void* W1p, const float* b1, const void* W2tp, const void* W1tp, float* du, float* dx,
+                                                 float* gm_out, int32_t M, int32_t C, int32_t Hd, float drop_p, uint32_t key1_0, uint32_t key1_1,
+                                                 const uint32_t* drop_seed, float mask_drop_p, uint32_t mask_key0, uint32_t mask_key1, const uint32_t* mask_seed,
+                                                 const float* rowscale, int32_t rows_per_scale, void* stream) {
+    RcMask mk;
+    const int rc = rc_mask_fill(mk, "mlp_rc16_dgrad_masked_hbf16", M, C, mask_drop_p, mask_key0, mask_key1, mask_seed, rowscale, rows_per_scale, gm_out);
+    if (rc != MDVIT_OK) return rc;
+    return rc16_dgrad_impl(&mk, 1, g, x, W1p, b1, W2tp, W1tp, du, dx, M, C, Hd, drop_p, key1_0, key1_1, drop_seed, stream);
 }
 
 extern "C" int mdvit_linear_rc(const float* x, int64_t lda, const void* Wp, int64_t wplane, const float* bias, float* y, int64_t ldc, int32_t M, int32_t N, int32_t K,
@@ -1768,9 +1865,9 @@
     return sizeof(float) * (size_t)rc_wgrad_groups(M) * (2u * (size_t)Hd * C + Hd);
 }
 
-extern "C" int mdvit_mlp_rc_wgrad(const float* gm, const float* x, const void* W1p, const float* b1, const void* W2tp, float* dW1, float* db1, float* dW2,
-                                  void* ws, size_t ws_bytes, int32_t M, int32_t C, int32_t Hd, float drop_p, uint32_t key1_0, uint32_t key1_1,
-                                  const uint32_t* drop_seed, int32_t accumulate, void* stream) {
+static int rc_wgrad_impl(const RcMask* mk, const float* gm, const float* x, const void* W1p, const float* b1, const void* W2tp, float* dW1, float* db1, float* dW2,
+                         void* ws, size_t ws_bytes, int32_t M, int32_t C, int32_t Hd, float drop_p, uint32_t key1_0, uint32_t key1_1,
+                         const uint32_t* drop_seed, int32_t accumulate, void* stream) {
     MDVIT_CHECK_ARG(C == 64, MDVIT_E_SHAPE, "mlp_rc_wgrad: built for C = 64 (got %d)", C);
     MDVIT_CHECK_ARG(M > 0 && Hd >= 256 && Hd % 256 == 0, MDVIT_E_SHAPE, "mlp_rc_wgrad: need M > 0, hidden %% 256 == 0 (M=%d hidden=%d)", M, Hd);
     MDVIT_CHECK_ARG(gm && x && W1p && b1 && W2tp && dW1 && db1 && dW2, MDVIT_E_SHAPE, "mlp_rc_wgrad: null operand");
@@ -1783,6 +1880,7 @@
     memset(&a, 0, sizeof(a));
     a.gm = gm; a.x = x; a.W1p = (const uint16_t*)W1p; a.b1 = b1; a.W2tp = (const uint16_t*)W2tp; a.part = (float*)ws;
     rc_fill(a, M, Hd, drop_p, key1_0, key1_1, 0, 0, drop_seed);
+    if (mk) a.mk = *mk;
     a.groups = rc_wgrad_groups(M);
     a.tiles_per_group = cdiv((M + 31) / 32, a.groups);
     const int roles = Hd / 256;
@@ -1799,9 +1897,24 @@
     return MDVIT_OK;
 }
 
-extern "C" int mdvit_mlp_rc_bwd(const float* gm, const float* x, const void* W1p, const float* b1, const void* W2tp, const void* W1tp, float* dx_parts,
-                                float* dW1, float* db1, float* dW2, void* ws, size_t ws_bytes, int32_t M, int32_t C, int32_t Hd, float drop_p,
-                                uint32_t key1_0, uint32_t key1_1, const uint32_t* drop_seed, int32_t accumulate, void* stream) {
+extern "C" int mdvit_mlp_rc_wgrad(const float* gm, const float* x, const void* W1p, const float* b1, const void* W2tp, float* dW1, float* db1, float* dW2,
+                                  void* ws, size_t ws_bytes, int32_t M, int32_t C, int32_t Hd, float drop_p, uint32_t key1_0, uint32_t key1_1,
+                                  const uint32_t* drop_seed, int32_t accumulate, void* stream) {
+    return rc_wgrad_impl(nullptr, gm, x, W1p, b1, W2tp, dW1, db1, dW2, ws, ws_bytes, M, C, Hd, drop_p, key1_0, key1_1, drop_seed, accumulate, stream);
+}
+extern "C" int mdvit_mlp_rc_wgrad_masked(const float* g, const float* x, const void* W1p, const float* b1, const void* W2tp, float* dW1, float* db1, float* dW2,
+                                         void* ws, size_t ws_bytes, int32_t M, int32_t C, int32_t Hd, float drop_p, uint32_t key1_0, uint32_t key1_1,
+                                         const uint32_t* drop_seed, float mask_drop_p, uint32_t mask_key0, uint32_t mask_key1, const uint32_t* mask_seed,
+                                         const float* rowscale, int32_t rows_per_scale, int32_t accumulate, void* stream) {
+    RcMask mk;
+    const int rc = rc_mask_fill(mk, "mlp_rc_wgrad_masked", M, C, mask_drop_p, mask_key0, mask_key1, mask_seed, rowscale, rows_per_scale, nullptr);
+    if (rc != MDVIT_OK) return rc;
+    return rc_wgrad_impl(&mk, g, x, W1p, b1, W2tp, dW1, db1, dW2, ws, ws_bytes, M, C, Hd, drop_p, key1_0, key1_1, drop_seed, accumulate, stream);
+}
+
+static int rc_bwd_impl(const RcMask* mk, const float* gm, const float* x, const void* W1p, const float* b1, const void* W2tp, const void* W1tp, float* dx_parts,
+                       float* dW1, float* db1, float* dW2, void* ws, size_t ws_bytes, int32_t M, int32_t C, int32_t Hd, float drop_p,
+                       uint32_t key1_0, uint32_t key1_1, const uint32_t* drop_seed, int32_t accumulate, void* stream) {
     MDVIT_CHECK_ARG(C == 64, MDVIT_E_SHAPE, "mlp_rc_bwd: built for C = 64 (got %d)", C);
     MDVIT_CHECK_ARG(M > 0 && (Hd == 256 || Hd == 512), MDVIT_E_SHAPE, "mlp_rc_bwd: need M > 0, hidden in {256, 512} (M=%d hidden=%d)", M, Hd);
     MDVIT_CHECK_ARG(gm && x && W1p && b1 && W2tp && W1tp && dx_parts && dW1 && db1 && dW2, MDVIT_E_SHAPE, "mlp_rc_bwd: null operand");
@@ -1814,6 +1927,7 @@
     memset(&a, 0, sizeof(a));
     a.gm = gm; a.x = x; a.W1p = (const uint16_t*)W1p; a.b1 = b1; a.W2tp = (const uint16_t*)W2tp; a.W1tp = (const uint16_t*)W1tp; a.dx = dx_parts; a.part = (float*)ws;
     rc_fill(a, M, Hd, drop_p, key1_0, key1_1, 0, 0, drop_seed);
+    if (mk) a.mk = *mk;
     a.groups = rc_wgrad_groups(M);
     a.tiles_per_group = cdiv((M + 31) / 32, a.groups);
     const int roles = Hd / 256;
@@ -1834,3 +1948,24 @@
     MDVIT_LAUNCH_CHECK();
     return MDVIT_OK;
 }
+
+extern "C" int mdvit_mlp_rc_bwd(const float* gm, const float* x, const void* W1p, const float* b1, const void* W2tp, const void* W1tp, float* dx_parts,
+                                float* dW1, float* db1, float* dW2, void* ws, size_t ws_bytes, int32_t M, int32_t C, int32_t Hd, float drop_p,
+                                uint32_t key1_0, uint32_t key1_1, const uint32_t* drop_seed, int32_t accumulate, void* stream) {
+    return rc_bwd_impl(nullptr, gm, x, W1p, b1, W2tp, W1tp, dx_parts, dW1, db1, dW2, ws, ws_bytes, M, C, Hd, drop_p, key1_0, key1_1, drop_seed, accumulate, stream);
+}
+extern "C" int mdvit_mlp_rc_bwd_masked(const float* g, const float* x, const void* W1p, const float* b1, const void* W2tp, const void* W1tp, float* dx_parts,
+                                       float* dW1, float* db1, float* dW2, void* ws, size_t ws_bytes, int32_t M, int32_t C, int32_t Hd, float drop_p,
+                                       uint32_t key1_0, uint32_t key1_1, const uint32_t* drop_seed, float mask_drop_p, uint32_t mask_key0, uint32_t mask_key1,
+                                       const uint32_t* mask_seed, const float* rowscale, int32_t rows_per_scale, int32_t accumulate, void* stream) {
+    RcMask mk;
+    const int rc = rc_mask_fill(mk, "mlp_rc_bwd_masked", M, C, mask_drop_p, mask_key0, mask_key1, mask_seed, rowscale, rows_per_scale, nullptr);
+    if (rc != MDVIT_OK) return rc;
+    return rc_bwd_impl(&mk, g, x, W1p, b1, W2tp, W1tp, dx_parts, dW1, db1, dW2, ws, ws_bytes, M, C, Hd, drop_p, key1_0, key1_1, drop_seed, accumulate, stream);
+}
+
+int g_rc_mask_fold = MDVIT_MASK_FOLD_DEFAULT;
+extern "C" int mdvit_mlp_mask_config(int32_t fold) {
+    g_rc_mask_fold = fold == 1 ? MDVIT_MASK_FOLD_DEFAULT : (fold & (MDVIT_MASK_FOLD_AUX | MDVIT_MASK_FOLD_FULL128 | MDVIT_MASK_FOLD_FULL64));
+    return MDVIT_OK;
+}
diff --git a/mdvit_amd/ops.py b/mdvit_amd/ops.py
--- a/mdvit_amd/ops.py
+++ b/mdvit_amd/ops.py
@@ -1106,6 +1106,21 @@
 _mlp_rc16 = os.environ.get("MDVIT_MLP_RC16", "1") != "0"
 _mlp_rc_bwd = os.environ.get("MDVIT_MLP_RC_BWD", "1")
 _lib.on_load(lambda lib: lib.mdvit_block_config({"0": 0, "1": 1}.get(_mlp_rc_bwd, 2)))
+_MASK_FOLD_AUX, _MASK_FOLD_FULL128, _MASK_FOLD_FULL64 = 2, 4, 8
+_MASK_FOLD_DEFAULT = _MASK_FOLD_AUX | _MASK_FOLD_FULL128 | _MASK_FOLD_FULL64
+_mlp_mask_fold = _MASK_FOLD_DEFAULT
+
+
+def set_mlp_mask_fold(v: int) -> None:
+    global _mlp_mask_fold
+    v = int(v)
+    _mlp_mask_fold = _MASK_FOLD_DEFAULT if v == 1 else v & (_MASK_FOLD_AUX | _MASK_FOLD_FULL128 | _MASK_FOLD_FULL64)
+    _lib.on_load(lambda lib, v=v: lib.mdvit_mlp_mask_config(v))
+
+
+_mlp_mask_fold_env = os.environ.get("MDVIT_MLP_MASK_FOLD", "1")
+if _mlp_mask_fold_env != "1":
+    set_mlp_mask_fold(int(_mlp_mask_fold_env))
 
 
 def _mlp_rc_ok(Cin, Hd, b1, b2, res, W1, W2, M) -> bool:
@@ -1201,12 +1216,14 @@
         if ctx.rc:
             masked = drop_p > 0 or rowscale is not None
             want_w = not _dgrad_only
-            gm = _empty_like(g) if masked else g
+            fold = masked and bool(_mlp_mask_fold & (_MASK_FOLD_FULL64 if want_w else _MASK_FOLD_AUX))
+            gm = _empty_like(g) if masked and not fold else g
+            mk = (drop_p, k2[0], k2[1], _seed_ptr() if drop_p > 0 else None, _p(rowscale), rps) if fold else (0.0, 0, 0, None, None, 1)
             if want_w and not sunk:
                 db2 = _empty((Cin,), device=dev, dtype=torch.float32)
-            if masked or want_w:
+            if (masked and not fold) or want_w:
                 wsp, wsb, _keep = _partials_ws(Cin, dev) if want_w else (None, 0, None)
-                call("mdvit_colsum_f32", _p(g), Cin, _p(sinks[3] if sunk else db2) if want_w else None, _p(gm) if masked else None, wsp, wsb, M, Cin,
+                call("mdvit_colsum_f32", _p(g), Cin, _p(sinks[3] if sunk else db2) if want_w else None, _p(gm) if masked and not fold else None, wsp, wsb, M, Cin,
                      drop_p, k2[0], k2[1], _p(rowscale), rps, int(sunk), _seed_ptr() if drop_p > 0 else None, _stream())
             W1p, W2tp, W1tp = _wplanes(W1, False, 2), _wplanes(W2, True, 2), _wplanes(W1, True, 2)
             fused = want_w and Hd in (256, 512) and (_mlp_rc_bwd == "1" or (_mlp_rc_bwd == "auto" and not (sunk and _side_stream is not None)))
@@ -1221,8 +1238,8 @@
                 else:
                     dW1, db1, dW2 = _empty_like(W1), _empty((Hd,), device=dev, dtype=torch.float32), _empty_like(W2)
                     tgt, accf = (dW1, db1, dW2), 0
-                call("mdvit_mlp_rc_bwd", _p(gm), _p(x), _p(W1p), _p(ctx.b1_ref), _p(W2tp), _p(W1tp), _p(parts), _p(tgt[0]), _p(tgt[1]), _p(tgt[2]), _p(ws), wsb,
-                     M, Cin, Hd, drop_p, k1[0], k1[1], _seed_ptr() if drop_p > 0 else None, accf, _stream())
+                call("mdvit_mlp_rc_bwd_masked", _p(gm), _p(x), _p(W1p), _p(ctx.b1_ref), _p(W2tp), _p(W1tp), _p(parts), _p(tgt[0]), _p(tgt[1]), _p(tgt[2]), _p(ws), wsb,
+                     M, Cin, Hd, drop_p, k1[0], k1[1], _seed_ptr() if drop_p > 0 else None, *mk, accf, _stream())
                 if roles == 1:
                     dx = parts[0]
                 else:
@@ -1231,28 +1248,30 @@
                 del W1p, W2tp, W1tp
                 return dx, g, dW1, db1, dW2, db2, None, None, None
             dx = _empty_like(x)
-            call("mdvit_mlp_rc_dgrad", _p(gm), _p(x), _p(W1p), _p(ctx.b1_ref), _p(W2tp), _p(W1tp), _p(dx), M, Cin, Hd,
-                 drop_p, k1[0], k1[1], _seed_ptr() if drop_p > 0 else None, _stream())
+            call("mdvit_mlp_rc_dgrad_masked", _p(gm), _p(x), _p(W1p), _p(ctx.b1_ref), _p(W2tp), _p(W1tp), _p(dx), M, Cin, Hd,
+                 drop_p, k1[0], k1[1], _seed_ptr() if drop_p > 0 else None, *mk, _stream())
             if want_w:
                 wsb = _lib.load().mdvit_mlp_rc_wgrad_ws_bytes(M, Cin, Hd)
                 if sunk:
                     with _on_side(gm, x, W1p, W2tp):
                         ws = _empty((wsb // 4,), device=dev, dtype=torch.float32)
-                        call("mdvit_mlp_rc_wgrad", _p(gm), _p(x), _p(W1p), _p(ctx.b1_ref), _p(W2tp), _p(sinks[0]), _p(sinks[1]), _p(sinks[2]), _p(ws), wsb,
-                             M, Cin, Hd, drop_p, k1[0], k1[1], _seed_ptr() if drop_p > 0 else None, 1, _stream())
+                        call("mdvit_mlp_rc_wgrad_masked", _p(gm), _p(x), _p(W1p), _p(ctx.b1_ref), _p(W2tp), _p(sinks[0]), _p(sinks[1]), _p(sinks[2]), _p(ws), wsb,
+                             M, Cin, Hd, drop_p, k1[0], k1[1], _seed_ptr() if drop_p > 0 else None, *mk, 1, _stream())
                     db2 = None
                 else:
                     dW1, db1, dW2 = _empty_like(W1), _empty((Hd,), device=dev, dtype=torch.float32), _empty_like(W2)
                     ws = _empty((wsb // 4,), device=dev, dtype=torch.float32)
-                    call("mdvit_mlp_rc_wgrad", _p(gm), _p(x), _p(W1p), _p(ctx.b1_ref), _p(W2tp), _p(dW1), _p(db1), _p(dW2), _p(ws), wsb,
-                         M, Cin, Hd, drop_p, k1[0], k1[1], _seed_ptr() if drop_p > 0 else None, 0, _stream())
+                    call("mdvit_mlp_rc_wgrad_masked", _p(gm), _p(x), _p(W1p), _p(ctx.b1_ref), _p(W2tp), _p(dW1), _p(db1), _p(dW2), _p(ws), wsb,
+                         M, Cin, Hd, drop_p, k1[0], k1[1], _seed_ptr() if drop_p > 0 else None, *mk, 0, _stream())
             del W1p, W2tp, W1tp
             return dx, g, dW1, db1, dW2, db2, None, None, None
         if not _dgrad_only and not sunk:
             db2 = torch.zeros((Cin,), device=dev, dtype=torch.float32)
         masked = drop_p > 0 or rowscale is not None
-        gm = _empty_like(g) if masked else g
-        if masked:
+        fold = (masked and u is None and _mlp_rc16_ok(Cin, Hd, ctx.b1_ref, W1, W2, M)
+                and not (_mlp_fused and _gemm_precision >= 1 and Cin == 64) and bool(_mlp_mask_fold & (_MASK_FOLD_AUX if _dgrad_only else _MASK_FOLD_FULL128)))
+        gm = _empty_like(g) if masked and not (fold and _dgrad_only) else g
+        if masked and not fold:
             call("mdvit_colsum_f32", _p(g), Cin, None, _p(gm), None, 0, M, Cin,
                  drop_p, k2[0], k2[1], _p(rowscale), rps, 0, _seed_ptr() if drop_p > 0 else None, _stream())
         dx = _empty_like(x)
@@ -1265,8 +1284,9 @@
         elif u is None and _mlp_rc16_ok(Cin, Hd, ctx.b1_ref, W1, W2, M):
             du = None if _dgrad_only else _empty_like(h)
             W1p, W2tp, W1tp = _wplanes(W1, False, 2), _wplanes(W2, True, 2), _wplanes(W1, True, 2)
-            call("mdvit_mlp_rc16_dgrad", _p(gm), _p(x), _p(W1p), _p(ctx.b1_ref), _p(W2tp), _p(W1tp), _p(du), _p(dx), M, Cin, Hd,
-                 drop_p, k1[0], k1[1], _seed_ptr() if drop_p > 0 else None, _stream())
+            mk = (drop_p, k2[0], k2[1], _seed_ptr() if drop_p > 0 else None, _p(rowscale), rps) if fold else (0.0, 0, 0, None, None, 1)
+            call("mdvit_mlp_rc16_dgrad_masked", _p(g if fold else gm), _p(x), _p(W1p), _p(ctx.b1_ref), _p(W2tp), _p(W1tp), _p(du), _p(dx),
+                 _p(gm) if fold and not _dgrad_only else None, M, Cin, Hd, drop_p, k1[0], k1[1], _seed_ptr() if drop_p > 0 else None, *mk, _stream())
             del W1p, W2tp, W1tp
         else:
             du = _empty_like(h)
```

Result: faster. 540.9 images/s (median of 6 runs) (+1.4%).
